# GT-STAR-Lab/MARBLER

Hardware: AMD Instinct MI355X
Metric: env agent-steps/sec (higher is better)
Workload: dtype f32

## Files before the change

include/robogym.h:

```cpp
#ifndef ROBOGYM_H
#define ROBOGYM_H

#include <stdint.h>

#ifdef __cplusplus
extern "C" {
#endif

#define RG_ABI_VERSION 7
#define RG_MAX_AGENTS 16
#define RG_MAX_PREY 64

enum {
    RG_SCN_PREDATOR_CAPTURE_PREY = 0,
    RG_SCN_WAREHOUSE = 1,
    RG_SCN_MATERIAL_TRANSPORT = 2,
    RG_SCN_SIMPLE = 3,
    RG_SCN_ARCTIC_TRANSPORT = 4
};
#define RG_ARCTIC_ROWS 8
#define RG_ARCTIC_COLS 12
enum { RG_COLLISION_CENTER = 0, RG_COLLISION_OFFSET = 1 };
enum { RG_VIOL_NONE = 0, RG_VIOL_COLLISION = 1, RG_VIOL_BOUNDARY = 2, RG_VIOL_COLLISION_BOUNDARY = 3 };
enum { RG_QP_EXACT = 0, RG_QP_CVXOPT = 1 };
#define RG_QP_CVXOPT_MAX_AGENTS 8

typedef struct rg_grid {
    int32_t nx, ny;
    float spacing, w2, h2, ox1, ox2, oy1, oy2;
} rg_grid;

typedef struct rg_scenario_params {
    int32_t scenario;
    int32_t n_agents;
    int32_t obs_dim;
    int32_t update_frequency;
    int32_t controller_period;
    int32_t max_episode_steps;
    int32_t penalize_violations;
    int32_t barrier_has_unsafe_gain;
    int32_t collision_variant;
    int32_t capability_aware;
    int32_t num_prey;
    int32_t num_neighbors;
    int32_t torque[RG_MAX_AGENTS];
    float time_step, bound_x0, bound_y0, bound_w, bound_h;
    float robot_diameter, wheel_radius, max_linear_velocity;
    float collision_offset, collision_diameter;
    float projection_distance, angular_velocity_limit, position_velocity_limit;
    float barrier_gain, unsafe_barrier_gain, safety_radius, barrier_magnitude_limit;
    float qp_rtol;
    int32_t qp_max_sweeps;
    float left, right, up, down;
    float agent_step[RG_MAX_AGENTS];
    float sensing_radius[RG_MAX_AGENTS];
    float capture_radius[RG_MAX_AGENTS];
    float time_penalty, sense_reward, capture_reward, violation_reward;
    float load_reward, unload_reward, goal_width;
    float unload_multiplier, load_multiplier, end_goal_width, zone1_radius;
    float reward_scaler;
    float arctic_normal_step, arctic_slow_step, arctic_fast_step;
    float not_reached_penalty, dist_multiplier;
    rg_grid agent_grid, prey_grid;
    int32_t keep_theta;
    int32_t shared_reward;
    float zone1_mean, zone1_std, zone2_mean, zone2_std;
    int32_t qp_mode;
    float ipm_abstol, ipm_reltol, ipm_feastol;
    int32_t ipm_maxiters;
} rg_scenario_params;

typedef struct rg_state {
    float *poses;
    float *carry_dist;
    int32_t *episode_steps;
    int32_t *reset_count;
    float *prey_loc;
    uint8_t *prey_sensed;
    uint8_t *prey_captured;
    uint8_t *loaded;
    int32_t *load;
    int32_t *zone_load;
    int32_t *messages;
    uint8_t *grid;
    int32_t *goal_col;
    uint8_t *pixel_type;
    uint8_t *reached_goal;
    float *ep_return;
    float *done_return_sum;
    int32_t *done_count;
    int32_t *done_steps_sum;
    float *next_init;
    int32_t *next_episode;
} rg_state;

typedef struct rg_step_io {
    float *obs;
    float *reward;
    uint8_t *done;
    float *dist_travelled;
    uint8_t *violation;
    int32_t *remaining;
    int32_t *qp_sweeps;
    int32_t *elapsed;
    uint8_t *truncated;
    uint8_t *ended;
    float *reward_sum;
    int32_t time_limit;
    int32_t zero_obs_on_end;
} rg_step_io;

typedef struct rg_handle rg_handle;

int rg_abi_version(void);
const char *rg_last_error(void);
int rg_sizeof_params(void);
int rg_sizeof_state(void);
int rg_sizeof_step_io(void);
int rg_next_init_stride(const rg_scenario_params *params);

rg_handle *rg_create(const rg_scenario_params *params, int32_t num_envs, int64_t env_offset, int32_t device,
                     void *hip_stream);
int rg_destroy(rg_handle *h);

int rg_bind_state(rg_handle *h, const rg_state *state);

#define RG_RESET_BOOK_EPISODE 1
int rg_reset(rg_handle *h, const uint8_t *mask, uint64_t seed, int32_t flags);

int rg_step(rg_handle *h, const int32_t *actions, const rg_step_io *io, int32_t auto_reset, uint64_t seed);

int rg_rollout(rg_handle *h, const int32_t *actions, int32_t num_steps, const rg_step_io *io, int32_t auto_reset,
               uint64_t seed);

int rg_set_stream(rg_handle *h, void *hip_stream);

int rg_get_obs(rg_handle *h, float *obs);

int rg_step_kernel(const rg_handle *h);

#define RG_LIDAR_MAX_RAYS 32
typedef struct rg_lidar_params {
    int32_t rays;
    int32_t offset;
    float range;
    float inv_range;
    float dir[RG_LIDAR_MAX_RAYS][2];
} rg_lidar_params;
int rg_sizeof_lidar_params(void);
int rg_set_lidar(rg_handle *h, const rg_lidar_params *lp);

#define RG_TEAM_MAX_SETS 64
#define RG_TEAM_EPISODE 0
#define RG_TEAM_FIXED 1
typedef struct rg_team_params {
    int32_t n_sets;
    int32_t mode;
    const float *agent_step;
    const float *sensing_radius;
    const float *capture_radius;
    const int32_t *torque;
    int32_t *team_index;
} rg_team_params;
int rg_sizeof_team_params(void);
int rg_set_teams(rg_handle *h, const rg_team_params *tp);

#define RG_DISTURB_MAX_SIGMA_XY 0.1f
#define RG_DISTURB_MAX_SIGMA_THETA 0.5f
typedef struct rg_disturbance_params {
    float sigma_xy;
    float sigma_theta;
    float reserved[2];
} rg_disturbance_params;
int rg_sizeof_disturbance_params(void);
int rg_set_disturbance(rg_handle *h, const rg_disturbance_params *dp);

typedef struct {
    const float *w1, *b1;
    const float *wih, *bih;
    const float *whh, *bhh;
    const float *w2, *b2;
    int32_t n_sets, input_dim, hidden_dim, n_actions, use_rnn;
    int32_t gru_packed;
} rg_actor_weights;

int rg_actor_forward(const rg_actor_weights *w, int32_t num_envs, int32_t n_agents, const float *obs,
                     int32_t obs_dim, int32_t append_agent_id, const uint8_t *restart, float *hidden, float *q,
                     int32_t *actions, void *hip_stream);
int rg_actor_forward_explore(const rg_actor_weights *w, int32_t num_envs, int32_t n_agents, const float *obs,
                             int32_t obs_dim, int32_t append_agent_id, const uint8_t *restart, float *hidden, float *q,
                             int32_t *actions, const float *explore_u, float epsilon, void *hip_stream);
int rg_actor_forward_sample(const rg_actor_weights *w, int32_t num_envs, int32_t n_agents, const float *obs,
                            int32_t obs_dim, int32_t append_agent_id, const uint8_t *restart, float *hidden, float *q,
                            int32_t *actions, const float *sample_u, float *prob, void *hip_stream);
int rg_actor_pack_gru(const float *src, int32_t n_sets, int32_t hidden_dim, float *dst, void *hip_stream);
int rg_actor_pack_gru_bf16x3(const float *src, int32_t n_sets, int32_t hidden_dim, void *dst, void *hip_stream);
int rg_actor_pack_gru_f16x2(const float *src, int32_t n_sets, int32_t hidden_dim, void *dst, void *hip_stream);
const char *rg_actor_last_error(void);

typedef struct rg_policy_io {
    float *hidden;
    const uint8_t *restart;
    int32_t append_agent_id;
    int32_t restart_on_done;
    const float *explore_u;
    float epsilon;
    int32_t *actions;
    float *obs;
    float *reward_sum;
    uint8_t *ended;
    float *dist_sum;
} rg_policy_io;
int rg_sizeof_policy_io(void);
int rg_policy_rollout(rg_handle *h, const rg_actor_weights *w, int32_t num_steps, const rg_policy_io *pio, const rg_step_io *io,
                      int32_t auto_reset, uint64_t seed);

typedef struct rg_policy_sample {
    const float *sample_u;
    float *prob;
} rg_policy_sample;
int rg_sizeof_policy_sample(void);
int rg_policy_rollout_sample(rg_handle *h, const rg_actor_weights *w, int32_t num_steps, const rg_policy_io *pio,
                             const rg_policy_sample *sample, const rg_step_io *io, int32_t auto_reset, uint64_t seed);

#ifdef __cplusplus
}
#endif
#endif
```

marbler_amd/_lib.py:

```python
import ctypes as C
import os

MAX_AGENTS, MAX_PREY = 16, 64
ABI_VERSION = 7
RESET_BOOK_EPISODE = 1

_HERE = os.path.dirname(os.path.abspath(__file__))
LIB_PATH = os.environ.get("ROBOGYM_LIB") or os.path.join(_HERE, "librobogym_hip.so")


class RgGrid(C.Structure):
    _fields_ = [("nx", C.c_int32), ("ny", C.c_int32), ("spacing", C.c_float), ("w2", C.c_float),
                ("h2", C.c_float), ("ox1", C.c_float), ("ox2", C.c_float), ("oy1", C.c_float),
                ("oy2", C.c_float)]


class RgScenarioParams(C.Structure):
    _fields_ = [
        ("scenario", C.c_int32), ("n_agents", C.c_int32), ("obs_dim", C.c_int32),
        ("update_frequency", C.c_int32), ("controller_period", C.c_int32),
        ("max_episode_steps", C.c_int32), ("penalize_violations", C.c_int32),
        ("barrier_has_unsafe_gain", C.c_int32), ("collision_variant", C.c_int32),
        ("capability_aware", C.c_int32), ("num_prey", C.c_int32), ("num_neighbors", C.c_int32),
        ("torque", C.c_int32 * MAX_AGENTS),
        ("time_step", C.c_float), ("bound_x0", C.c_float), ("bound_y0", C.c_float),
        ("bound_w", C.c_float), ("bound_h", C.c_float),
        ("robot_diameter", C.c_float), ("wheel_radius", C.c_float), ("max_linear_velocity", C.c_float),
        ("collision_offset", C.c_float), ("collision_diameter", C.c_float),
        ("projection_distance", C.c_float), ("angular_velocity_limit", C.c_float),
        ("position_velocity_limit", C.c_float),
        ("barrier_gain", C.c_float), ("unsafe_barrier_gain", C.c_float), ("safety_radius", C.c_float),
        ("barrier_magnitude_limit", C.c_float), ("qp_rtol", C.c_float), ("qp_max_sweeps", C.c_int32),
        ("left", C.c_float), ("right", C.c_float), ("up", C.c_float), ("down", C.c_float),
        ("agent_step", C.c_float * MAX_AGENTS), ("sensing_radius", C.c_float * MAX_AGENTS),
        ("capture_radius", C.c_float * MAX_AGENTS),
        ("time_penalty", C.c_float), ("sense_reward", C.c_float), ("capture_reward", C.c_float),
        ("violation_reward", C.c_float),
        ("load_reward", C.c_float), ("unload_reward", C.c_float), ("goal_width", C.c_float),
        ("unload_multiplier", C.c_float), ("load_multiplier", C.c_float), ("end_goal_width", C.c_float),
        ("zone1_radius", C.c_float), ("reward_scaler", C.c_float),
        ("arctic_normal_step", C.c_float), ("arctic_slow_step", C.c_float), ("arctic_fast_step", C.c_float),
        ("not_reached_penalty", C.c_float), ("dist_multiplier", C.c_float),
        ("agent_grid", RgGrid), ("prey_grid", RgGrid), ("keep_theta", C.c_int32), ("shared_reward", C.c_int32),
        ("zone1_mean", C.c_float), ("zone1_std", C.c_float), ("zone2_mean", C.c_float),
        ("zone2_std", C.c_float),
        ("qp_mode", C.c_int32), ("ipm_abstol", C.c_float), ("ipm_reltol", C.c_float), ("ipm_feastol", C.c_float), ("ipm_maxiters", C.c_int32),
    ]


class RgState(C.Structure):
    _fields_ = [("poses", C.c_void_p), ("carry_dist", C.c_void_p), ("episode_steps", C.c_void_p),
                ("reset_count", C.c_void_p), ("prey_loc", C.c_void_p), ("prey_sensed", C.c_void_p),
                ("prey_captured", C.c_void_p), ("loaded", C.c_void_p), ("load", C.c_void_p),
                ("zone_load", C.c_void_p), ("messages", C.c_void_p), ("grid", C.c_void_p),
                ("goal_col", C.c_void_p), ("pixel_type", C.c_void_p), ("reached_goal", C.c_void_p),
                ("ep_return", C.c_void_p),
                ("done_return_sum", C.c_void_p), ("done_count", C.c_void_p), ("done_steps_sum", C.c_void_p),
                ("next_init", C.c_void_p), ("next_episode", C.c_void_p)]


class RgStepIO(C.Structure):
    _fields_ = [("obs", C.c_void_p), ("reward", C.c_void_p), ("done", C.c_void_p),
                ("dist_travelled", C.c_void_p), ("violation", C.c_void_p), ("remaining", C.c_void_p),
                ("qp_sweeps", C.c_void_p),
                ("elapsed", C.c_void_p), ("truncated", C.c_void_p), ("ended", C.c_void_p), ("reward_sum", C.c_void_p),
                ("time_limit", C.c_int32), ("zero_obs_on_end", C.c_int32)]


class RgActorWeights(C.Structure):
    _fields_ = [("w1", C.c_void_p), ("b1", C.c_void_p), ("wih", C.c_void_p), ("bih", C.c_void_p),
                ("whh", C.c_void_p), ("bhh", C.c_void_p), ("w2", C.c_void_p), ("b2", C.c_void_p),
                ("n_sets", C.c_int32), ("input_dim", C.c_int32), ("hidden_dim", C.c_int32),
                ("n_actions", C.c_int32), ("use_rnn", C.c_int32), ("gru_packed", C.c_int32)]


class RgPolicyIO(C.Structure):
    _fields_ = [("hidden", C.c_void_p), ("restart", C.c_void_p), ("append_agent_id", C.c_int32), ("restart_on_done", C.c_int32),
                ("explore_u", C.c_void_p), ("epsilon", C.c_float), ("actions", C.c_void_p), ("obs", C.c_void_p),
                ("reward_sum", C.c_void_p), ("ended", C.c_void_p), ("dist_sum", C.c_void_p)]


class RgPolicySample(C.Structure):
    _fields_ = [("sample_u", C.c_void_p), ("prob", C.c_void_p)]


LIDAR_MAX_RAYS = 32


class RgLidarParams(C.Structure):
    _fields_ = [("rays", C.c_int32), ("offset", C.c_int32), ("range", C.c_float), ("inv_range", C.c_float),
                ("dir", (C.c_float * 2) * LIDAR_MAX_RAYS)]


TEAM_MAX_SETS = 64
TEAM_EPISODE, TEAM_FIXED = 0, 1


class RgTeamParams(C.Structure):
    _fields_ = [("n_sets", C.c_int32), ("mode", C.c_int32), ("agent_step", C.c_void_p), ("sensing_radius", C.c_void_p),
                ("capture_radius", C.c_void_p), ("torque", C.c_void_p), ("team_index", C.c_void_p)]


DISTURB_MAX_SIGMA_XY, DISTURB_MAX_SIGMA_THETA = 0.1, 0.5


class RgDisturbanceParams(C.Structure):
    _fields_ = [("sigma_xy", C.c_float), ("sigma_theta", C.c_float), ("reserved", C.c_float * 2)]


EXPORTS = ("rg_abi_version", "rg_last_error", "rg_sizeof_params", "rg_sizeof_state", "rg_sizeof_step_io", "rg_next_init_stride",
           "rg_create", "rg_destroy", "rg_bind_state", "rg_set_stream", "rg_reset", "rg_step", "rg_rollout", "rg_get_obs", "rg_step_kernel",
           "rg_actor_forward", "rg_actor_forward_explore", "rg_actor_pack_gru", "rg_actor_pack_gru_bf16x3", "rg_actor_pack_gru_f16x2", "rg_actor_last_error",
           "rg_sizeof_policy_io", "rg_policy_rollout", "rg_sizeof_lidar_params", "rg_set_lidar",
           "rg_sizeof_team_params", "rg_set_teams",
           "rg_actor_forward_sample", "rg_sizeof_policy_sample", "rg_policy_rollout_sample",
           "rg_sizeof_disturbance_params", "rg_set_disturbance")

_lib = None


class RobogymError(RuntimeError):
    pass


def load():
    global _lib
    if _lib is not None:
        return _lib
    if not os.path.exists(LIB_PATH):
        raise RobogymError(
            f"{LIB_PATH} not found: build it with `python -m marbler_amd.build` (hipcc, gfx950). "
            "marbler_amd has no CPU fallback.")
    lib = C.CDLL(LIB_PATH)
    for name in EXPORTS:
        if not hasattr(lib, name):
            raise RobogymError(f"{LIB_PATH} does not export {name}")
    lib.rg_abi_version.restype = C.c_int
    lib.rg_last_error.restype = C.c_char_p
    lib.rg_create.restype = C.c_void_p
    lib.rg_create.argtypes = [C.POINTER(RgScenarioParams), C.c_int32, C.c_int64, C.c_int32, C.c_void_p]
    lib.rg_next_init_stride.argtypes = [C.POINTER(RgScenarioParams)]
    lib.rg_next_init_stride.restype = C.c_int
    lib.rg_destroy.argtypes = [C.c_void_p]
    lib.rg_bind_state.argtypes = [C.c_void_p, C.POINTER(RgState)]
    lib.rg_set_stream.argtypes = [C.c_void_p, C.c_void_p]
    lib.rg_reset.argtypes = [C.c_void_p, C.c_void_p, C.c_uint64, C.c_int32]
    lib.rg_step.argtypes = [C.c_void_p, C.c_void_p, C.POINTER(RgStepIO), C.c_int32, C.c_uint64]
    lib.rg_rollout.argtypes = [C.c_void_p, C.c_void_p, C.c_int32, C.POINTER(RgStepIO), C.c_int32, C.c_uint64]
    lib.rg_get_obs.argtypes = [C.c_void_p, C.c_void_p]
    lib.rg_step_kernel.argtypes = [C.c_void_p]
    lib.rg_step_kernel.restype = C.c_int
    lib.rg_actor_forward.argtypes = [C.POINTER(RgActorWeights), C.c_int32, C.c_int32, C.c_void_p, C.c_int32, C.c_int32,
                                     C.c_void_p, C.c_void_p, C.c_void_p, C.c_void_p, C.c_void_p]
    lib.rg_actor_forward.restype = C.c_int
    lib.rg_actor_forward_explore.argtypes = [C.POINTER(RgActorWeights), C.c_int32, C.c_int32, C.c_void_p, C.c_int32, C.c_int32,
                                             C.c_void_p, C.c_void_p, C.c_void_p, C.c_void_p, C.c_void_p, C.c_float, C.c_void_p]
    lib.rg_actor_forward_explore.restype = C.c_int
    lib.rg_actor_forward_sample.argtypes = [C.POINTER(RgActorWeights), C.c_int32, C.c_int32, C.c_void_p, C.c_int32, C.c_int32,
                                            C.c_void_p, C.c_void_p, C.c_void_p, C.c_void_p, C.c_void_p, C.c_void_p, C.c_void_p]
    lib.rg_actor_forward_sample.restype = C.c_int
    lib.rg_actor_pack_gru.argtypes = [C.c_void_p, C.c_int32, C.c_int32, C.c_void_p, C.c_void_p]
    lib.rg_actor_pack_gru.restype = C.c_int
    lib.rg_actor_pack_gru_bf16x3.argtypes = [C.c_void_p, C.c_int32, C.c_int32, C.c_void_p, C.c_void_p]
    lib.rg_actor_pack_gru_bf16x3.restype = C.c_int
    lib.rg_actor_pack_gru_f16x2.argtypes = [C.c_void_p, C.c_int32, C.c_int32, C.c_void_p, C.c_void_p]
    lib.rg_actor_pack_gru_f16x2.restype = C.c_int
    lib.rg_actor_last_error.restype = C.c_char_p
    lib.rg_policy_rollout.argtypes = [C.c_void_p, C.POINTER(RgActorWeights), C.c_int32, C.POINTER(RgPolicyIO), C.POINTER(RgStepIO),
                                      C.c_int32, C.c_uint64]
    lib.rg_policy_rollout.restype = C.c_int
    lib.rg_sizeof_policy_io.restype = C.c_int
    lib.rg_policy_rollout_sample.argtypes = [C.c_void_p, C.POINTER(RgActorWeights), C.c_int32, C.POINTER(RgPolicyIO),
                                             C.POINTER(RgPolicySample), C.POINTER(RgStepIO), C.c_int32, C.c_uint64]
    lib.rg_policy_rollout_sample.restype = C.c_int
    lib.rg_sizeof_policy_sample.restype = C.c_int
    lib.rg_set_lidar.argtypes = [C.c_void_p, C.POINTER(RgLidarParams)]
    lib.rg_set_lidar.restype = C.c_int
    lib.rg_sizeof_lidar_params.restype = C.c_int
    lib.rg_set_teams.argtypes = [C.c_void_p, C.POINTER(RgTeamParams)]
    lib.rg_set_teams.restype = C.c_int
    lib.rg_sizeof_team_params.restype = C.c_int
    lib.rg_set_disturbance.argtypes = [C.c_void_p, C.POINTER(RgDisturbanceParams)]
    lib.rg_set_disturbance.restype = C.c_int
    lib.rg_sizeof_disturbance_params.restype = C.c_int
    for f in (lib.rg_destroy, lib.rg_bind_state, lib.rg_set_stream, lib.rg_reset, lib.rg_step, lib.rg_rollout, lib.rg_get_obs,
              lib.rg_sizeof_params, lib.rg_sizeof_state, lib.rg_sizeof_step_io):
        f.restype = C.c_int
    if lib.rg_abi_version() != ABI_VERSION:
        raise RobogymError(f"ABI version {lib.rg_abi_version()} != {ABI_VERSION}; rebuild the library")
    if (lib.rg_sizeof_params() != C.sizeof(RgScenarioParams) or lib.rg_sizeof_state() != C.sizeof(RgState)
            or lib.rg_sizeof_step_io() != C.sizeof(RgStepIO) or lib.rg_sizeof_policy_io() != C.sizeof(RgPolicyIO)
            or lib.rg_sizeof_policy_sample() != C.sizeof(RgPolicySample)
            or lib.rg_sizeof_lidar_params() != C.sizeof(RgLidarParams) or lib.rg_sizeof_team_params() != C.sizeof(RgTeamParams)
            or lib.rg_sizeof_disturbance_params() != C.sizeof(RgDisturbanceParams)):
        raise RobogymError("struct layout of the binding differs from the compiled library; rebuild")
    _lib = lib
    return lib


def check(rc, what):
    if rc != 0:
        raise RobogymError(f"{what} failed ({rc}): {load().rg_last_error().decode()}")
```

marbler_amd/build.py:

```python
import glob
import os
import shutil
import subprocess
import sys

HERE = os.path.dirname(os.path.abspath(__file__))
CSRC = os.path.join(HERE, "csrc")
LIB = os.path.join(HERE, "librobogym_hip.so")
SOURCES = ["robogym_kernels.hip", "robogym_resident.hip", "robogym_rollout_group.hip", "robogym_kernels_ipm.hip", "robogym_rollout_group_ipm.hip",
           "robogym_tpe.hip", "robogym_rollout_tpe.hip", "robogym_capi.hip", "actor_mfma.hip", "robogym_policy_h64.hip",
           "robogym_policy_h128.hip", "robogym_policy_sample_h64.hip", "robogym_policy_sample_h128.hip", "robogym_lidar.hip", "robogym_lidar_rollout.hip", "robogym_lidar_ipm.hip",
           "robogym_lidar_rollout_ipm.hip", "robogym_team.hip", "robogym_team_rollout.hip", "robogym_team_ipm.hip",
           "robogym_team_rollout_ipm.hip", "robogym_disturb.hip", "robogym_disturb_rollout.hip", "robogym_disturb_ipm.hip",
           "robogym_disturb_rollout_ipm.hip"]
HEADERS = sorted(glob.glob(os.path.join(CSRC, "*.h")) + glob.glob(os.path.join(CSRC, "*.inc")) + glob.glob(os.path.join(CSRC, "probes", "*.h"))) + \
          [os.path.join(HERE, "..", "include", "robogym.h")]
ARCH = "gfx950"
GROUP_SLP = ["-mllvm", "-slp-threshold=-60"]
IPM_SCHED = ["-mllvm", "-amdgpu-sched-strategy=max-ilp"]
RESIDENT_PRELOAD = ["-mllvm", "-amdgpu-kernarg-preload-count=16"]
FILE_FLAGS = {"robogym_tpe.hip": ["-fno-slp-vectorize"], "robogym_rollout_tpe.hip": ["-fno-slp-vectorize"],
              "robogym_kernels.hip": GROUP_SLP, "robogym_rollout_group.hip": GROUP_SLP,
              "robogym_resident.hip": GROUP_SLP + RESIDENT_PRELOAD,
              "robogym_kernels_ipm.hip": GROUP_SLP + IPM_SCHED, "robogym_rollout_group_ipm.hip": GROUP_SLP + IPM_SCHED,
              "robogym_policy_h64.hip": GROUP_SLP, "robogym_policy_h128.hip": GROUP_SLP,
              "robogym_policy_sample_h64.hip": GROUP_SLP, "robogym_policy_sample_h128.hip": GROUP_SLP,
              "robogym_lidar.hip": GROUP_SLP, "robogym_lidar_rollout.hip": GROUP_SLP,
              "robogym_lidar_ipm.hip": GROUP_SLP + IPM_SCHED, "robogym_lidar_rollout_ipm.hip": GROUP_SLP + IPM_SCHED,
              "robogym_team.hip": GROUP_SLP, "robogym_team_rollout.hip": GROUP_SLP,
              "robogym_team_ipm.hip": GROUP_SLP + IPM_SCHED, "robogym_team_rollout_ipm.hip": GROUP_SLP + IPM_SCHED,
              "robogym_disturb.hip": GROUP_SLP, "robogym_disturb_rollout.hip": GROUP_SLP,
              "robogym_disturb_ipm.hip": GROUP_SLP + IPM_SCHED, "robogym_disturb_rollout_ipm.hip": GROUP_SLP + IPM_SCHED}
BASE_FLAGS = [f"--offload-arch={ARCH}", "-O3", "-fPIC", "-std=c++17", "-ffp-contract=off", "-Wall", "-Wno-unused-function"]
STAMP = LIB + ".flags"


def hipcc_path():
    for c in (os.environ.get("HIPCC"), "/opt/rocm/bin/hipcc", shutil.which("hipcc")):
        if c and os.path.exists(c):
            return c
    raise RuntimeError("hipcc not found (ROCm 7.x expected under /opt/rocm)")


def flags_stamp(defines=(), extra=(), file_flags=True):
    per_file = sorted(FILE_FLAGS.items()) if file_flags else []
    return repr((BASE_FLAGS, sorted(defines), list(extra), per_file, SOURCES))


def needs_build():
    if not os.path.exists(LIB):
        return True
    t = os.path.getmtime(LIB)
    deps = [os.path.join(CSRC, s) for s in SOURCES] + HEADERS + [os.path.abspath(__file__)]
    if any(os.path.getmtime(d) > t for d in deps):
        return True
    try:
        with open(STAMP) as f:
            return f.read() != flags_stamp()
    except OSError:
        return True


def build(force=False, verbose=False, defines=(), out=None):
    extra = os.environ.get("RG_EXTRA_HIPCC_FLAGS", "").split()
    no_file_flags = bool(os.environ.get("RG_NO_FILE_FLAGS"))
    if out is None:
        if not force and not needs_build():
            return LIB
        if extra or no_file_flags:
            import warnings
            warnings.warn("RG_EXTRA_HIPCC_FLAGS / RG_NO_FILE_FLAGS are for diagnostic variants (build(out=...)) and are IGNORED for the "
                          "shipped library, whose flags are fixed in marbler_amd/build.py")
            extra, no_file_flags = [], False
    shipped = out is None
    out = out or LIB
    objdir = os.path.join(HERE, "build", os.path.splitext(os.path.basename(out))[0])
    os.makedirs(objdir, exist_ok=True)
    flags = BASE_FLAGS + [f"-D{d}" for d in defines] + extra
    objs, procs = [], []
    for src in SOURCES:
        obj = os.path.join(objdir, os.path.splitext(src)[0] + ".o")
        per_file = [] if no_file_flags else FILE_FLAGS.get(src, [])
        cmd = [hipcc_path()] + flags + per_file + ["-c", os.path.join(CSRC, src), "-o", obj]
        if verbose:
            print(" ".join(cmd))
        procs.append((cmd, subprocess.Popen(cmd)))
        objs.append(obj)
    for cmd, pr in procs:
        if pr.wait() != 0:
            raise subprocess.CalledProcessError(pr.returncode, cmd)
    link = [hipcc_path(), f"--offload-arch={ARCH}", "-shared", "-fPIC", "-o", out] + objs
    if verbose:
        print(" ".join(link))
    subprocess.check_call(link)
    with open(out + ".flags", "w") as f:
        f.write(flags_stamp(defines, extra, not no_file_flags) if not shipped else flags_stamp())
    return out


def build_host_sanitized(out=None):
    out = out or os.path.join(HERE, "build", "librobogym_capi_asan.so")
    os.makedirs(os.path.dirname(out), exist_ok=True)
    stubs = os.path.join(HERE, "..", "tests", "sanitize", "launch_stubs.cpp")
    stubs_sample = os.path.join(HERE, "..", "tests", "sanitize", "launch_stubs_sample.cpp")
    cmd = [hipcc_path(), "-x", "hip", "--offload-host-only", "-O1", "-g", "-fno-omit-frame-pointer",
           "-fsanitize=address,undefined", "-fno-sanitize-recover=undefined", "-fPIC", "-shared", "-std=c++17",
           "-I", CSRC, os.path.join(CSRC, "robogym_capi.hip"), stubs, stubs_sample, "-o", out]
    subprocess.check_call(cmd)
    return out


def asan_runtime():
    return subprocess.check_output([hipcc_path(), "-print-file-name=libclang_rt.asan-x86_64.so"], text=True).strip()


if __name__ == "__main__":
    print(build(force="--force" in sys.argv, verbose=True))
```

marbler_amd/csrc/kernel_args.h:

```cpp
#pragma once
#include <hip/hip_runtime.h>
#include <math.h>
#include <stddef.h>
#include <stdint.h>

#include <type_traits>

#include "../../include/robogym.h"

namespace rg {

struct Consts {
    float dt, pd, inv_pd, r2, wlim, vmax, wmax, pvl, bml;
    float xmin, xmax, ymin, ymax, coll_off, coll_lim2;
    float thr_pre;
    float lin_pre;
    float xc, xh, yc, yh;
};

constexpr float PRE_SLACK = 2e-6f;
inline float pre_margin(float max_abs_coordinate) {
    float spacing = 0.0009765625f;
    for (float lim = 2.0f; lim <= max_abs_coordinate && lim < 1024.0f; lim *= 2.0f) spacing *= 2.0f;
    return 1.05f * 1.41421356f * (2.0f * spacing + 6.103515625e-05f);
}

inline Consts make_consts(const rg_scenario_params &p) {
    Consts k;
    k.dt = p.time_step;
    k.pd = p.projection_distance;
    k.inv_pd = 1.0f / p.projection_distance;
    k.r2 = p.safety_radius * p.safety_radius;
    k.wlim = p.angular_velocity_limit;
    k.vmax = p.max_linear_velocity;
    k.wmax = 2.0f * (p.wheel_radius / p.robot_diameter) * (p.max_linear_velocity / p.wheel_radius);
    k.pvl = p.position_velocity_limit;
    k.bml = p.barrier_magnitude_limit;
    k.xmin = p.bound_x0;
    k.ymin = p.bound_y0;
    k.xmax = p.bound_x0 + p.bound_w;
    k.ymax = p.bound_y0 + p.bound_h;
    const bool off = p.collision_variant == RG_COLLISION_OFFSET;
    k.coll_off = off ? p.collision_offset : 0.0f;
    const float lim = off ? p.collision_diameter : p.robot_diameter;
    k.coll_lim2 = lim * lim;
    const float ax = fmaxf(fabsf(k.xmin), fabsf(k.xmax)), ay = fmaxf(fabsf(k.ymin), fabsf(k.ymax));
    const float lp = lim + pre_margin(fmaxf(ax, ay) + 0.25f);
    k.thr_pre = lp * lp * 1.00001f;
    k.lin_pre = lp;
    k.xc = 0.5f * (k.xmin + k.xmax);
    k.xh = 0.5f * (k.xmax - k.xmin);
    k.yc = 0.5f * (k.ymin + k.ymax);
    k.yh = 0.5f * (k.ymax - k.ymin);
    return k;
}

struct KernelArgs {
    rg_scenario_params p;
    Consts k;
    rg_state st;
    rg_step_io io;
    const int32_t *actions;
    const uint8_t *reset_mask;
    int32_t E;
    int32_t envs_per_wave;
    int32_t num_steps;
    int32_t auto_reset;
    int32_t reset_flags;
    int32_t next_stride;
    int64_t env_offset;
    uint64_t seed;
};

inline int next_init_stride(const rg_scenario_params &p) {
    int w = 3 * p.n_agents;
    if (p.scenario == RG_SCN_PREDATOR_CAPTURE_PREY || p.scenario == RG_SCN_SIMPLE) w += 2 * p.num_prey;
    else if (p.scenario == RG_SCN_MATERIAL_TRANSPORT) w += 2;
    else if (p.scenario == RG_SCN_ARCTIC_TRANSPORT) w += 25;
    return (w + 3) & ~3;
}

template <typename F>
inline hipError_t for_scenario(int scn, F &&f) {
    switch (scn) {
        case RG_SCN_PREDATOR_CAPTURE_PREY: return f(std::integral_constant<int, RG_SCN_PREDATOR_CAPTURE_PREY>());
        case RG_SCN_WAREHOUSE: return f(std::integral_constant<int, RG_SCN_WAREHOUSE>());
        case RG_SCN_MATERIAL_TRANSPORT: return f(std::integral_constant<int, RG_SCN_MATERIAL_TRANSPORT>());
        case RG_SCN_SIMPLE: return f(std::integral_constant<int, RG_SCN_SIMPLE>());
        case RG_SCN_ARCTIC_TRANSPORT: return f(std::integral_constant<int, RG_SCN_ARCTIC_TRANSPORT>());
        default: return hipErrorInvalidValue;
    }
}

hipError_t launch_reset(const KernelArgs &a, hipStream_t stream);

enum GroupFamily { GROUP_PLAIN, GROUP_LIDAR, GROUP_TEAM, GROUP_DISTURB };
enum GroupKind { GROUP_STEP, GROUP_ROLLOUT, GROUP_OBS, GROUP_STEP_RESIDENT };
#define RG_GROUP_ENTRIES(X)                                              \
    X(launch_step, GROUP_PLAIN, RG_QP_EXACT, GROUP_STEP)                 \
    X(launch_step_resident, GROUP_PLAIN, RG_QP_EXACT, GROUP_STEP_RESIDENT) \
    X(launch_obs, GROUP_PLAIN, RG_QP_EXACT, GROUP_OBS)                   \
    X(launch_rollout, GROUP_PLAIN, RG_QP_EXACT, GROUP_ROLLOUT)           \
    X(launch_step_ipm, GROUP_PLAIN, RG_QP_CVXOPT, GROUP_STEP)            \
    X(launch_rollout_ipm, GROUP_PLAIN, RG_QP_CVXOPT, GROUP_ROLLOUT)      \
    X(launch_lidar_step, GROUP_LIDAR, RG_QP_EXACT, GROUP_STEP)           \
    X(launch_lidar_obs, GROUP_LIDAR, RG_QP_EXACT, GROUP_OBS)             \
    X(launch_lidar_rollout, GROUP_LIDAR, RG_QP_EXACT, GROUP_ROLLOUT)     \
    X(launch_lidar_step_ipm, GROUP_LIDAR, RG_QP_CVXOPT, GROUP_STEP)      \
    X(launch_lidar_rollout_ipm, GROUP_LIDAR, RG_QP_CVXOPT, GROUP_ROLLOUT) \
    X(launch_team_step, GROUP_TEAM, RG_QP_EXACT, GROUP_STEP)             \
    X(launch_team_obs, GROUP_TEAM, RG_QP_EXACT, GROUP_OBS)               \
    X(launch_team_rollout, GROUP_TEAM, RG_QP_EXACT, GROUP_ROLLOUT)       \
    X(launch_team_step_ipm, GROUP_TEAM, RG_QP_CVXOPT, GROUP_STEP)        \
    X(launch_team_rollout_ipm, GROUP_TEAM, RG_QP_CVXOPT, GROUP_ROLLOUT)  \
    X(launch_disturb_step, GROUP_DISTURB, RG_QP_EXACT, GROUP_STEP)       \
    X(launch_disturb_rollout, GROUP_DISTURB, RG_QP_EXACT, GROUP_ROLLOUT) \
    X(launch_disturb_step_ipm, GROUP_DISTURB, RG_QP_CVXOPT, GROUP_STEP)  \
    X(launch_disturb_rollout_ipm, GROUP_DISTURB, RG_QP_CVXOPT, GROUP_ROLLOUT)
struct DisturbScale {
    float k_xy, k_theta;
};
inline float disturb_scale(float sigma) { return static_cast<float>(static_cast<double>(sigma) * sqrt(3.0 / 1048575.0)); }
struct GroupSide {
    const rg_lidar_params *lidar;
    const rg_team_params *teams;
    const DisturbScale *disturb;
    const struct KernelArgs *image;
};

struct ResidentCall {
    const KernelArgs *image;
    const int32_t *actions;
    uint64_t seed;
    int32_t auto_reset;
    int32_t grid;
    rg_step_io io;
};
static_assert(sizeof(ResidentCall) <= 256, "the per-call arguments fit one register of dwords (device_common.h load_arg_regs_resident)");
hipError_t resident_image(KernelArgs &a);
typedef hipError_t GroupLaunch(const KernelArgs &a, const GroupSide &side, hipStream_t stream);
#define RG_X(entry, family, mode, kind) GroupLaunch entry;
RG_GROUP_ENTRIES(RG_X)
#undef RG_X

struct StepView {
    const int32_t *actions;
    rg_step_io io;
    const int32_t *auto_reset;
    const uint64_t *seed;
    int32_t grid;
};
__host__ __device__ inline StepView step_view(const KernelArgs &a, int k, int n_agents, int obs_dim) {
    StepView v;
    const size_t e = static_cast<size_t>(a.E) * k, en = e * n_agents;
    v.actions = a.actions ? a.actions + en : nullptr;
    v.io.obs = a.io.obs ? a.io.obs + en * obs_dim : nullptr;
    v.io.reward = a.io.reward ? a.io.reward + en : nullptr;
    v.io.done = a.io.done ? a.io.done + e : nullptr;
    v.io.dist_travelled = a.io.dist_travelled ? a.io.dist_travelled + en : nullptr;
    v.io.violation = a.io.violation ? a.io.violation + e : nullptr;
    v.io.remaining = a.io.remaining ? a.io.remaining + e : nullptr;
    v.io.qp_sweeps = a.io.qp_sweeps ? a.io.qp_sweeps + e : nullptr;
    v.io.elapsed = a.io.elapsed;
    v.io.truncated = a.io.truncated ? a.io.truncated + e : nullptr;
    v.io.ended = a.io.ended ? a.io.ended + e : nullptr;
    v.io.reward_sum = a.io.reward_sum ? a.io.reward_sum + e : nullptr;
    v.io.time_limit = a.io.time_limit;
    v.io.zero_obs_on_end = a.io.zero_obs_on_end;
    v.auto_reset = &a.auto_reset;
    v.seed = &a.seed;
    v.grid = 0;
    return v;
}
bool tpe_supported(const rg_scenario_params &p);
hipError_t launch_step_tpe(const KernelArgs &a, hipStream_t stream);
hipError_t launch_rollout_tpe(const KernelArgs &a, hipStream_t stream);

}
```

marbler_amd/csrc/robogym_capi.hip:

```cpp
#include <hip/hip_runtime.h>
#include <stdint.h>
#include <stdio.h>
#include <stdlib.h>
#include <string.h>

#include <new>

#include "../../include/robogym.h"
#include "kernel_args.h"

struct rg_handle {
    rg_scenario_params params;
    rg::Consts consts;
    rg_state state;
    int32_t num_envs;
    int64_t env_offset;
    int32_t device;
    hipStream_t stream;
    bool bound;
    bool use_tpe;
    bool seed_seen;
    uint64_t last_seed;
    bool default_tpe;
    rg_lidar_params lidar;
    rg_team_params teams;
    bool disturbed;
    rg::DisturbScale disturb;
    bool span;
    bool resident;
    rg::KernelArgs *image_slots;
    int32_t images_used;
    const rg::KernelArgs *image;
    bool image_stale;
};
constexpr int RG_IMAGE_SLOTS = 8;
constexpr size_t RG_IMAGE_STRIDE = 1024;
static_assert(sizeof(rg::KernelArgs) <= RG_IMAGE_STRIDE, "an image slot holds the block");
static void write_image(rg_handle *h);
static void drop_image(rg_handle *h) {
    h->image = nullptr;
    h->image_stale = true;
}

static int32_t tpe_min_envs(const rg_scenario_params &p) {
    const bool mt = p.scenario == RG_SCN_MATERIAL_TRANSPORT, pcp = p.scenario == RG_SCN_PREDATOR_CAPTURE_PREY;
    if (p.qp_mode == RG_QP_CVXOPT) return p.n_agents == 5 ? 12288 : 20480;
    switch (p.n_agents) {
        case 2: return 65536;
        case 3: return pcp ? 98304 : 65536;
        case 4: return p.scenario == RG_SCN_SIMPLE ? 393216 : p.scenario == RG_SCN_ARCTIC_TRANSPORT ? 131072 : 196608;
        case 5: return mt ? 49152 : 65536;
        case 6: return mt ? 65536 : p.scenario == RG_SCN_WAREHOUSE ? 262144 : pcp ? 98304 : 131072;
        default: return INT32_MAX;
    }
}

static thread_local char g_err[512] = "";

struct DeviceGuard {
    int prev = -1;
    bool switched = false;
    hipError_t err;
    explicit DeviceGuard(int device) {
        err = hipGetDevice(&prev);
        if (err == hipSuccess && prev != device) {
            err = hipSetDevice(device);
            switched = (err == hipSuccess);
        }
    }
    ~DeviceGuard() {
        if (switched) (void)hipSetDevice(prev);
    }
    DeviceGuard(const DeviceGuard &) = delete;
    DeviceGuard &operator=(const DeviceGuard &) = delete;
};

static int fail(int code, const char *fmt, const char *detail = "") {
    snprintf(g_err, sizeof(g_err), fmt, detail);
    return code;
}

static int check_params(const rg_scenario_params *p) {
    if (!p) return fail(-1, "params is NULL");
    if (p->scenario < RG_SCN_PREDATOR_CAPTURE_PREY || p->scenario > RG_SCN_ARCTIC_TRANSPORT)
        return fail(-2, "unknown scenario id");
    if (p->n_agents < 1 || p->n_agents > RG_MAX_AGENTS) return fail(-3, "n_agents must be in 1..16");
    if (p->update_frequency < 1 || p->controller_period < 1) return fail(-4, "update_frequency / controller_period < 1");
    if (p->obs_dim < 1) return fail(-5, "obs_dim < 1");
    if (p->qp_max_sweeps < 1 || !(p->qp_rtol >= 0.0f)) return fail(-5, "qp_max_sweeps < 1 or qp_rtol < 0");
    if (p->qp_mode != RG_QP_EXACT && p->qp_mode != RG_QP_CVXOPT) return fail(-5, "unknown qp_mode");
    if (p->qp_mode == RG_QP_CVXOPT) {
        if (p->n_agents > RG_QP_CVXOPT_MAX_AGENTS) return fail(-3, "qp_mode RG_QP_CVXOPT is built for n_agents <= 8");
        if (p->ipm_maxiters < 0 || !(p->ipm_reltol >= 0.0f) || !(p->ipm_feastol > 0.0f) || !(p->ipm_abstol >= 0.0f))
            return fail(-5, "ipm_maxiters < 0, or a negative / zero cvxopt tolerance");
    }
    if (p->collision_variant != RG_COLLISION_CENTER && p->collision_variant != RG_COLLISION_OFFSET)
        return fail(-6, "unknown collision_variant");
    const rg_grid &g = p->agent_grid;
    if (g.nx < 1 || g.ny < 1 || g.nx * g.ny <= p->n_agents || g.nx * g.ny > 64)
        return fail(-7, "agent reset grid must have n_agents < nx*ny <= 64");
    if (p->scenario == RG_SCN_PREDATOR_CAPTURE_PREY) {
        if (p->num_prey < 1 || p->num_prey > RG_MAX_PREY) return fail(-8, "num_prey must be in 1..64");
        const rg_grid &q = p->prey_grid;
        if (q.nx < 1 || q.ny < 1 || q.nx * q.ny <= p->num_prey || q.nx * q.ny > 64)
            return fail(-9, "prey reset grid must have num_prey < nx*ny <= 64");
        const int od = p->capability_aware ? 6 : 4;
        const int nb = p->num_neighbors >= p->n_agents - 1 ? p->n_agents - 1 : p->num_neighbors;
        if (p->obs_dim < od * (nb + 1)) return fail(-10, "obs_dim too small for PredatorCapturePrey");
        if (od == 4 && (p->obs_dim & 3)) return fail(-10, "obs_dim must be a multiple of 4 for PredatorCapturePrey without capability_aware");
    } else if (p->scenario == RG_SCN_WAREHOUSE) {
        const int nb = p->num_neighbors >= p->n_agents - 1 ? p->n_agents - 1 : p->num_neighbors;
        if (p->obs_dim < 3 * (nb + 1)) return fail(-10, "obs_dim too small for Warehouse");
    } else if (p->scenario == RG_SCN_SIMPLE) {
        if (p->num_prey != 1) return fail(-8, "Simple has one goal (num_prey = 1)");
        const rg_grid &q = p->prey_grid;
        if (q.nx < 1 || q.ny < 1 || q.nx * q.ny <= 1 || q.nx * q.ny > 64) return fail(-9, "goal reset grid must have 1 < nx*ny <= 64");
        if (p->obs_dim < 2 * (p->n_agents + 1)) return fail(-10, "obs_dim too small for Simple");
    } else if (p->scenario == RG_SCN_ARCTIC_TRANSPORT) {
        if (p->n_agents != 4) return fail(-3, "ArcticTransport has exactly 4 agents");
        if (p->obs_dim < 30) return fail(-10, "obs_dim too small for ArcticTransport");
    } else {
        if (p->obs_dim < (p->capability_aware ? 11 : 9)) return fail(-10, "obs_dim too small for MaterialTransport");
    }
    return 0;
}

namespace rg {
hipError_t launch_policy_rollout_h64(const KernelArgs &, const rg_actor_weights &, const rg_policy_io &, int32_t, hipStream_t)
    __attribute__((weak));
hipError_t launch_policy_rollout_h128(const KernelArgs &, const rg_actor_weights &, const rg_policy_io &, int32_t, hipStream_t)
    __attribute__((weak));
hipError_t launch_policy_rollout_sample_h64(const KernelArgs &, const rg_actor_weights &, const rg_policy_io &, const rg_policy_sample &,
                                            int32_t, hipStream_t) __attribute__((weak));
hipError_t launch_policy_rollout_sample_h128(const KernelArgs &, const rg_actor_weights &, const rg_policy_io &, const rg_policy_sample &,
                                             int32_t, hipStream_t) __attribute__((weak));
#define RG_X(entry, family, mode, kind) GroupLaunch entry __attribute__((weak));
RG_GROUP_ENTRIES(RG_X)
#undef RG_X
hipError_t launch_team_index(const KernelArgs &, const rg_team_params &, hipStream_t) __attribute__((weak));
hipError_t resident_image(KernelArgs &) __attribute__((weak));
}

static int own_obs_width(const rg_scenario_params &p) {
    const int nb = p.num_neighbors >= p.n_agents - 1 ? p.n_agents - 1 : p.num_neighbors;
    switch (p.scenario) {
        case RG_SCN_PREDATOR_CAPTURE_PREY: return (p.capability_aware ? 6 : 4) * (nb + 1);
        case RG_SCN_WAREHOUSE: return 3 * (nb + 1);
        case RG_SCN_SIMPLE: return 2 * (p.n_agents + 1);
        case RG_SCN_ARCTIC_TRANSPORT: return 30;
        default: return p.capability_aware ? 11 : 9;
    }
}

static const struct GroupEntry {
    rg::GroupLaunch *launch;
    int family, mode, kind;
} g_group[] = {
#define RG_X(entry, family, mode, kind) {rg::entry, rg::family, mode, rg::kind},
    RG_GROUP_ENTRIES(RG_X)
#undef RG_X
};

static bool group_family_built(int family) {
    for (const GroupEntry &g : g_group)
        if (g.family == family && !g.launch) return false;
    return true;
}

extern "C" {

int rg_abi_version(void) { return RG_ABI_VERSION; }

const char *rg_last_error(void) { return g_err; }

int rg_sizeof_params(void) { return static_cast<int>(sizeof(rg_scenario_params)); }
int rg_sizeof_state(void) { return static_cast<int>(sizeof(rg_state)); }
int rg_sizeof_step_io(void) { return static_cast<int>(sizeof(rg_step_io)); }
int rg_sizeof_policy_io(void) { return static_cast<int>(sizeof(rg_policy_io)); }
int rg_sizeof_policy_sample(void) { return static_cast<int>(sizeof(rg_policy_sample)); }
int rg_sizeof_lidar_params(void) { return static_cast<int>(sizeof(rg_lidar_params)); }
int rg_sizeof_team_params(void) { return static_cast<int>(sizeof(rg_team_params)); }
int rg_sizeof_disturbance_params(void) { return static_cast<int>(sizeof(rg_disturbance_params)); }
int rg_next_init_stride(const rg_scenario_params *params) {
    if (check_params(params) != 0) return -1;
    return rg::next_init_stride(*params);
}

rg_handle *rg_create(const rg_scenario_params *params, int32_t num_envs, int64_t env_offset, int32_t device,
                     void *hip_stream) {
    if (check_params(params) != 0) return nullptr;
    if (num_envs < 1) {
        fail(-11, "num_envs < 1");
        return nullptr;
    }
    int count = 0;
    if (hipGetDeviceCount(&count) != hipSuccess || count < 1) {
        fail(-12, "no HIP device visible: librobogym_hip has no CPU fallback");
        return nullptr;
    }
    if (device < 0 || device >= count) {
        fail(-13, "device index out of range");
        return nullptr;
    }
    if (!group_family_built(rg::GROUP_PLAIN)) {
        fail(-100, "rg_create: this build has no lane-group step kernels");
        return nullptr;
    }
    rg_handle *h = new (std::nothrow) rg_handle();
    if (!h) {
        fail(-14, "out of host memory");
        return nullptr;
    }
    h->params = *params;
    h->consts = rg::make_consts(*params);
    memset(&h->state, 0, sizeof(h->state));
    h->num_envs = num_envs;
    h->env_offset = env_offset;
    h->device = device;
    h->stream = static_cast<hipStream_t>(hip_stream);
    h->bound = false;
    h->seed_seen = false;
    h->last_seed = 0;
    h->use_tpe = rg::tpe_supported(*params) && num_envs >= tpe_min_envs(*params);
    if (const char *force = getenv("RG_STEP_KERNEL")) {
        if (!strcmp(force, "group")) h->use_tpe = false;
        else if (!strcmp(force, "tpe") && rg::tpe_supported(*params)) h->use_tpe = true;
    }
    h->default_tpe = h->use_tpe;
    {
        const char *span = getenv("RG_STEP_SPAN");
        h->span = !(span && !strcmp(span, "0"));
    }
    {
        const char *res = getenv("RG_STEP_RESIDENT");
        h->resident = !(res && !strcmp(res, "0")) && rg::resident_image && rg::launch_step_resident;
    }
    h->image_slots = nullptr;
    h->images_used = 0;
    h->image = nullptr;
    h->image_stale = true;
    memset(&h->lidar, 0, sizeof(h->lidar));
    memset(&h->teams, 0, sizeof(h->teams));
    h->disturbed = false;
    h->disturb = rg::DisturbScale{0.0f, 0.0f};
    return h;
}

int rg_set_lidar(rg_handle *h, const rg_lidar_params *lp) {
    if (!h) return fail(-1, "handle is NULL");
    if (!lp || lp->rays == 0) {
        memset(&h->lidar, 0, sizeof(h->lidar));
        h->use_tpe = (h->teams.n_sets || h->disturbed) ? false : h->default_tpe;
        drop_image(h);
        return 0;
    }
    if (h->disturbed) return fail(-57, "rg_set_lidar: the handle has the pose disturbance on (rg_set_disturbance); the disturbance and the lidar do not combine");
    if (h->teams.n_sets) return fail(-54, "rg_set_lidar: the handle has a team pool (rg_set_teams); a pool and the lidar do not combine");
    if (lp->rays < 4 || lp->rays > RG_LIDAR_MAX_RAYS || (lp->rays & 3))
        return fail(-50, "rg_set_lidar: rays must be 0 or a multiple of 4 in 4..32");
    if (lp->offset + lp->rays != h->params.obs_dim)
        return fail(-51, "rg_set_lidar: offset + rays must equal obs_dim (the lidar block ends the observation row)");
    if (lp->offset < own_obs_width(h->params))
        return fail(-52, "rg_set_lidar: offset lies inside the scenario's own observation columns");
    if (!(lp->range > 0.0f && lp->range <= 3.402823466e38f)) return fail(-53, "rg_set_lidar: range must be positive and finite");
    if (!group_family_built(rg::GROUP_LIDAR)) return fail(-100, "rg_set_lidar: this build has no lidar kernels");
    h->lidar = *lp;
    h->use_tpe = false;
    drop_image(h);
    return 0;
}

int rg_set_disturbance(rg_handle *h, const rg_disturbance_params *dp) {
    if (!h) return fail(-1, "handle is NULL");
    if (!dp || (dp->sigma_xy == 0.0f && dp->sigma_theta == 0.0f)) {
        h->disturbed = false;
        h->disturb = rg::DisturbScale{0.0f, 0.0f};
        h->use_tpe = (h->lidar.rays || h->teams.n_sets) ? false : h->default_tpe;
        drop_image(h);
        return 0;
    }
    if (!(dp->sigma_xy >= 0.0f && dp->sigma_xy <= RG_DISTURB_MAX_SIGMA_XY))
        return fail(-70, "rg_set_disturbance: sigma_xy must be a finite number of metres in [0, 0.1]");
    if (!(dp->sigma_theta >= 0.0f && dp->sigma_theta <= RG_DISTURB_MAX_SIGMA_THETA))
        return fail(-71, "rg_set_disturbance: sigma_theta must be a finite number of radians in [0, 0.5]");
    if (h->lidar.rays) return fail(-72, "rg_set_disturbance: the handle has the lidar on (rg_set_lidar); the disturbance and the lidar do not combine");
    if (h->teams.n_sets) return fail(-73, "rg_set_disturbance: the handle has a team pool (rg_set_teams); the disturbance and a pool do not combine");
    if (!group_family_built(rg::GROUP_DISTURB)) return fail(-100, "rg_set_disturbance: this build has no disturbance kernels");
    h->disturb = rg::DisturbScale{rg::disturb_scale(dp->sigma_xy), rg::disturb_scale(dp->sigma_theta)};
    h->disturbed = true;
    h->use_tpe = false;
    drop_image(h);
    return 0;
}

int rg_destroy(rg_handle *h) {
    if (!h) return fail(-1, "handle is NULL");
    if (h->image_slots) {
        DeviceGuard guard(h->device);
        if (guard.err == hipSuccess) (void)hipFree(h->image_slots);
    }
    delete h;
    return 0;
}

int rg_set_stream(rg_handle *h, void *hip_stream) {
    if (!h) return fail(-1, "handle is NULL");
    h->stream = static_cast<hipStream_t>(hip_stream);
    return 0;
}

int rg_bind_state(rg_handle *h, const rg_state *st) {
    if (!h || !st) return fail(-1, "handle or state is NULL");
    if (!st->poses || !st->carry_dist || !st->episode_steps || !st->reset_count)
        return fail(-20, "poses, carry_dist, episode_steps and reset_count are required");
    switch (h->params.scenario) {
        case RG_SCN_PREDATOR_CAPTURE_PREY:
            if (!st->prey_loc || !st->prey_sensed || !st->prey_captured)
                return fail(-21, "PredatorCapturePrey needs prey_loc, prey_sensed, prey_captured");
            if (reinterpret_cast<uintptr_t>(st->prey_loc) & 7u) return fail(-26, "prey_loc must be 8-byte aligned");
            break;
        case RG_SCN_WAREHOUSE:
            if (!st->loaded) return fail(-21, "Warehouse needs loaded");
            break;
        case RG_SCN_SIMPLE:
            if (!st->prey_loc) return fail(-21, "Simple needs prey_loc (its goal)");
            break;
        case RG_SCN_ARCTIC_TRANSPORT:
            if (!st->grid || !st->goal_col || !st->pixel_type || !st->reached_goal)
                return fail(-21, "ArcticTransport needs grid, goal_col, pixel_type, reached_goal");
            if (reinterpret_cast<uintptr_t>(st->grid) & 3u) return fail(-26, "grid must be 4-byte aligned");
            break;
        default:
            if (!st->load || !st->zone_load || !st->messages)
                return fail(-21, "MaterialTransport needs load, zone_load, messages");
    }
    const int nstat = (st->ep_return != nullptr) + (st->done_return_sum != nullptr) + (st->done_count != nullptr) +
                      (st->done_steps_sum != nullptr);
    if (nstat != 0 && nstat != 4) return fail(-25, "rollout statistics arrays: set all four or none");
    if ((st->next_init != nullptr) != (st->next_episode != nullptr)) return fail(-25, "next_init / next_episode: set both or none");
    if (reinterpret_cast<uintptr_t>(st->next_init) & 15u) return fail(-26, "next_init must be 16-byte aligned");
    h->state = *st;
    h->bound = true;
    drop_image(h);
    write_image(h);
    h->seed_seen = false;
    return 0;
}

static int fill_args(rg_handle *h, rg::KernelArgs &a);
#define RG_ON_DEVICE(h)                                                                           \
    DeviceGuard guard_((h)->device);                                                              \
    if (guard_.err != hipSuccess) return fail(-31, "cannot select the handle's device: %s", hipGetErrorString(guard_.err))

static void write_image(rg_handle *h) {
    h->image = nullptr;
    if (!h->resident || !h->bound || h->use_tpe || !h->span || h->teams.n_sets || h->lidar.rays || h->disturbed ||
        h->params.qp_mode != RG_QP_EXACT) {
        h->image_stale = false;
        return;
    }
    if (h->images_used >= RG_IMAGE_SLOTS) {
        h->image_stale = false;
        return;
    }
    rg::KernelArgs a;
    if (fill_args(h, a) != 0 || rg::resident_image(a) != hipSuccess) {
        h->image_stale = false;
        return;
    }
    DeviceGuard guard(h->device);
    if (guard.err != hipSuccess) return;
    hipStreamCaptureStatus cap = hipStreamCaptureStatusNone;
    if (hipStreamIsCapturing(h->stream, &cap) != hipSuccess || cap != hipStreamCaptureStatusNone) {
        (void)hipGetLastError();
        return;
    }
    if (!h->image_slots) {
        void *mem = nullptr;
        if (hipMalloc(&mem, RG_IMAGE_SLOTS * RG_IMAGE_STRIDE) != hipSuccess) {
            (void)hipGetLastError();
            h->images_used = RG_IMAGE_SLOTS;
            h->image_stale = false;
            return;
        }
        h->image_slots = static_cast<rg::KernelArgs *>(mem);
    }
    rg::KernelArgs *slot = reinterpret_cast<rg::KernelArgs *>(reinterpret_cast<char *>(h->image_slots) + RG_IMAGE_STRIDE * h->images_used);
    h->images_used += 1;
    h->image_stale = false;
    if (hipMemcpy(slot, &a, sizeof(a), hipMemcpyHostToDevice) != hipSuccess) {
        (void)hipGetLastError();
        return;
    }
    h->image = slot;
}

static int fill_args(rg_handle *h, rg::KernelArgs &a) {
    if (!h) return fail(-1, "handle is NULL");
    if (!h->bound) return fail(-22, "rg_bind_state has not been called");
    memset(&a, 0, sizeof(a));
    a.p = h->params;
    a.k = h->consts;
    a.st = h->state;
    a.E = h->num_envs;
    a.num_steps = 1;
    a.env_offset = h->env_offset;
    a.next_stride = (!h->use_tpe && h->state.next_init) ? rg::next_init_stride(h->params) : 0;
    return 0;
}

static int sync_seed(rg_handle *h, uint64_t seed) {
    if (h->state.next_episode && (!h->seed_seen || h->last_seed != seed)) {
        const hipError_t err = hipMemsetAsync(h->state.next_episode, 0xFF, sizeof(int32_t) * static_cast<size_t>(h->num_envs), h->stream);
        if (err != hipSuccess) return fail(-30, "hipMemsetAsync(next_episode) failed: %s", hipGetErrorString(err));
        h->seed_seen = true;
        h->last_seed = seed;
    }
    return 0;
}

static int check_io(const rg_step_io *io) {
    if (!io->obs || !io->reward || !io->done || !io->dist_travelled || !io->violation || !io->remaining)
        return fail(-24, "every rg_step_io array except qp_sweeps and the gymma block is required");
    if (reinterpret_cast<uintptr_t>(io->obs) & 15u) return fail(-26, "obs must be 16-byte aligned");
    if (io->elapsed) {
        if (!io->truncated || !io->ended || !io->reward_sum) return fail(-24, "gymma block: elapsed needs truncated, ended and reward_sum");
        if (io->time_limit < 1) return fail(-29, "gymma block: time_limit must be > 0");
    }
    return 0;
}

static int launched(hipError_t err) {
    if (err != hipSuccess) return fail(-30, "kernel launch failed: %s", hipGetErrorString(err));
    return 0;
}

static int launch_group_entry(const rg_handle *h, const rg::KernelArgs &a, int kind, const rg::KernelArgs *image = nullptr) {
    const int family = h->teams.n_sets ? rg::GROUP_TEAM : h->lidar.rays ? rg::GROUP_LIDAR
                       : (h->disturbed && kind != rg::GROUP_OBS) ? rg::GROUP_DISTURB : rg::GROUP_PLAIN;
    const int mode = kind == rg::GROUP_OBS ? RG_QP_EXACT : h->params.qp_mode;
    const rg::GroupSide side = {&h->lidar, &h->teams, &h->disturb, family == rg::GROUP_PLAIN ? image : nullptr};
    for (const GroupEntry &g : g_group)
        if (g.family == family && g.mode == mode && g.kind == kind && g.launch) return launched(g.launch(a, side, h->stream));
    return fail(-100, "this build has no lane-group step kernels");
}

int rg_reset(rg_handle *h, const uint8_t *mask, uint64_t seed, int32_t flags) {
    rg::KernelArgs a;
    if (int rc = fill_args(h, a)) return rc;
    if (flags & ~RG_RESET_BOOK_EPISODE) return fail(-28, "unknown rg_reset flags");
    a.reset_mask = mask;
    a.seed = seed;
    a.reset_flags = flags;
    RG_ON_DEVICE(h);
    if (int rc = launched(rg::launch_reset(a, h->stream))) return rc;
    if (h->teams.n_sets) return launched(rg::launch_team_index(a, h->teams, h->stream));
    return 0;
}

int rg_step(rg_handle *h, const int32_t *actions, const rg_step_io *io, int32_t auto_reset, uint64_t seed) {
    rg::KernelArgs a;
    if (int rc = fill_args(h, a)) return rc;
    if (!actions || !io) return fail(-23, "actions or io is NULL");
    if (int rc = check_io(io)) return rc;
    a.actions = actions;
    a.io = *io;
    a.auto_reset = auto_reset;
    a.seed = seed;
    RG_ON_DEVICE(h);
    if (int rc = sync_seed(h, seed)) return rc;
    if (!h->span && !h->teams.n_sets && !h->lidar.rays && !h->disturbed) a.envs_per_wave = -1;
    if (h->use_tpe) return launched(rg::launch_step_tpe(a, h->stream));
    if (h->image_stale) write_image(h);
    return launch_group_entry(h, a, rg::GROUP_STEP, io->elapsed ? nullptr : h->image);
}

int rg_rollout(rg_handle *h, const int32_t *actions, int32_t num_steps, const rg_step_io *io, int32_t auto_reset,
               uint64_t seed) {
    rg::KernelArgs a;
    if (int rc = fill_args(h, a)) return rc;
    if (!actions || !io) return fail(-23, "actions or io is NULL");
    if (num_steps < 1) return fail(-27, "num_steps < 1");
    if (io->elapsed) return fail(-29, "the gymma block of rg_step_io belongs to rg_step (one launch per step)");
    if (int rc = check_io(io)) return rc;
    a.actions = actions;
    a.io = *io;
    a.num_steps = num_steps;
    a.auto_reset = auto_reset;
    a.seed = seed;
    RG_ON_DEVICE(h);
    if (int rc = sync_seed(h, seed)) return rc;
    if (!h->use_tpe) return launch_group_entry(h, a, rg::GROUP_ROLLOUT);
    if (h->num_envs <= 65536) return launched(rg::launch_rollout_tpe(a, h->stream));
    a.num_steps = 1;
    for (int32_t k = 0; k < num_steps; ++k) {
        const rg::StepView v = rg::step_view(a, k, h->params.n_agents, h->params.obs_dim);
        rg::KernelArgs ak = a;
        ak.actions = v.actions;
        ak.io = v.io;
        if (int rc = launched(rg::launch_step_tpe(ak, h->stream))) return rc;
    }
    return 0;
}

static int policy_rollout(rg_handle *h, const rg_actor_weights *w, int32_t num_steps, const rg_policy_io *pio,
                          const rg_policy_sample *sample, bool sampling, const rg_step_io *io, int32_t auto_reset, uint64_t seed) {
    rg::KernelArgs a;
    if (int rc = fill_args(h, a)) return rc;
    if (!w || !pio || !io) return fail(-23, "weights, policy io or step io is NULL");
    if (num_steps < 1) return fail(-27, "num_steps < 1");
    if (h->params.qp_mode == RG_QP_CVXOPT) return fail(-40, "rg_policy_rollout: the interior-point mode (barrier_solver: cvxopt) is not supported");
    if (h->lidar.rays) return fail(-49, "rg_policy_rollout: a handle with the lidar observation on (rg_set_lidar) is not supported");
    if (h->teams.n_sets) return fail(-39, "rg_policy_rollout: a handle with a team pool (rg_set_teams) is not supported");
    if (h->disturbed) return fail(-38, "rg_policy_rollout: a handle with the pose disturbance on (rg_set_disturbance) is not supported");
    if (!w->use_rnn || w->gru_packed != 3)
        return fail(-41, "rg_policy_rollout: the actor must be a GRU with gru_packed == 3 (two binary16 planes, pack_gru='f16x2')");
    if (w->hidden_dim != 64 && w->hidden_dim != 128) return fail(-42, "rg_policy_rollout: hidden_dim must be 64 or 128");
    const int N = h->params.n_agents;
    if (w->n_sets != 1 && w->n_sets != N) return fail(-43, "rg_policy_rollout: n_sets must be 1 (shared) or n_agents");
    if (w->input_dim != h->params.obs_dim + (pio->append_agent_id ? N : 0))
        return fail(-44, "rg_policy_rollout: the actor's input_dim != obs_dim (+ n_agents with append_agent_id)");
    if (w->input_dim > 64) return fail(-44, "rg_policy_rollout: input_dim above 64 is not supported");
    if (w->n_actions < 1 || w->n_actions > 32) return fail(-45, "rg_policy_rollout: n_actions must be in 1..32");
    if (!w->w1 || !w->b1 || !w->wih || !w->bih || !w->whh || !w->bhh || !w->w2 || !w->b2) return fail(-46, "rg_policy_rollout: a weight array is NULL");
    if (!pio->hidden || !pio->actions) return fail(-47, "rg_policy_rollout: hidden and actions are required");
    if ((reinterpret_cast<uintptr_t>(pio->hidden) | reinterpret_cast<uintptr_t>(pio->obs) | reinterpret_cast<uintptr_t>(w->w1) |
         reinterpret_cast<uintptr_t>(w->wih) | reinterpret_cast<uintptr_t>(w->whh) | reinterpret_cast<uintptr_t>(w->w2)) & 15u)
        return fail(-26, "rg_policy_rollout: hidden, obs, w1, wih, whh and w2 must be 16-byte aligned");
    if (pio->explore_u && !(pio->epsilon >= 1e-6f && pio->epsilon <= 1.0f)) return fail(-48, "rg_policy_rollout: epsilon must be in [1e-6, 1] with explore_u");
    if (!io->elapsed) return fail(-29, "rg_policy_rollout: the step io must carry the gymma block (elapsed, truncated, ended, reward_sum)");
    if (int rc = check_io(io)) return rc;
    auto launch = w->hidden_dim == 64 ? rg::launch_policy_rollout_h64 : rg::launch_policy_rollout_h128;
    auto launch_sample = w->hidden_dim == 64 ? rg::launch_policy_rollout_sample_h64 : rg::launch_policy_rollout_sample_h128;
    if (sampling ? !launch_sample : !launch) return fail(-100, "rg_policy_rollout: this build has no device code");
    a.io = *io;
    a.auto_reset = auto_reset;
    a.seed = seed;
    a.next_stride = 0;
    RG_ON_DEVICE(h);
    if (int rc = sync_seed(h, seed)) return rc;
    if (sampling) return launched(launch_sample(a, *w, *pio, *sample, num_steps, h->stream));
    return launched(launch(a, *w, *pio, num_steps, h->stream));
}

int rg_policy_rollout(rg_handle *h, const rg_actor_weights *w, int32_t num_steps, const rg_policy_io *pio, const rg_step_io *io,
                      int32_t auto_reset, uint64_t seed) {
    return policy_rollout(h, w, num_steps, pio, nullptr, false, io, auto_reset, seed);
}

int rg_policy_rollout_sample(rg_handle *h, const rg_actor_weights *w, int32_t num_steps, const rg_policy_io *pio,
                             const rg_policy_sample *sample, const rg_step_io *io, int32_t auto_reset, uint64_t seed) {
    if (!sample || !sample->sample_u) return fail(-55, "rg_policy_rollout_sample: sample or its sample_u is NULL");
    if (pio && pio->explore_u) return fail(-56, "rg_policy_rollout_sample: sample_u and explore_u do not combine (explore_u must be NULL)");
    return policy_rollout(h, w, num_steps, pio, sample, true, io, auto_reset, seed);
}

int rg_set_teams(rg_handle *h, const rg_team_params *tp) {
    if (!h) return fail(-1, "handle is NULL");
    if (!tp || tp->n_sets == 0) {
        memset(&h->teams, 0, sizeof(h->teams));
        h->use_tpe = (h->lidar.rays || h->disturbed) ? false : h->default_tpe;
        drop_image(h);
        return 0;
    }
    if (h->disturbed) return fail(-65, "rg_set_teams: the handle has the pose disturbance on (rg_set_disturbance); the disturbance and a pool do not combine");
    if (tp->n_sets < 1 || tp->n_sets > RG_TEAM_MAX_SETS) return fail(-60, "rg_set_teams: n_sets must be 0 or in 1..64");
    if (tp->mode != RG_TEAM_EPISODE && tp->mode != RG_TEAM_FIXED)
        return fail(-61, "rg_set_teams: unknown mode (RG_TEAM_EPISODE or RG_TEAM_FIXED)");
    if (h->params.scenario == RG_SCN_ARCTIC_TRANSPORT)
        return fail(-62, "rg_set_teams: ArcticTransport's agent types are fixed by the scenario; it takes no team pool");
    if (h->lidar.rays) return fail(-63, "rg_set_teams: the handle has the lidar on (rg_set_lidar); a pool and the lidar do not combine");
    const int sc = h->params.scenario;
    if (!tp->team_index || !tp->agent_step || (sc == RG_SCN_PREDATOR_CAPTURE_PREY && (!tp->sensing_radius || !tp->capture_radius)) ||
        (sc == RG_SCN_MATERIAL_TRANSPORT && !tp->torque))
        return fail(-64, "rg_set_teams: team_index, agent_step and the scenario's other tables (PredatorCapturePrey: sensing_radius, "
                         "capture_radius; MaterialTransport: torque) are required");
    if (!group_family_built(rg::GROUP_TEAM) || !rg::launch_team_index) return fail(-100, "rg_set_teams: this build has no team kernels");
    if (tp->mode == RG_TEAM_FIXED) {
        rg::KernelArgs a;
        if (int rc = fill_args(h, a)) return rc;
        RG_ON_DEVICE(h);
        if (int rc = launched(rg::launch_team_index(a, *tp, h->stream))) return rc;
    }
    h->teams = *tp;
    h->use_tpe = false;
    drop_image(h);
    return 0;
}

int rg_step_kernel(const rg_handle *h) {
    if (!h) return fail(-1, "handle is NULL");
    return h->use_tpe ? 1 : 0;
}

int rg_get_obs(rg_handle *h, float *obs) {
    rg::KernelArgs a;
    if (int rc = fill_args(h, a)) return rc;
    if (!obs) return fail(-23, "obs is NULL");
    if (reinterpret_cast<uintptr_t>(obs) & 15u) return fail(-26, "obs must be 16-byte aligned");
    a.io.obs = obs;
    RG_ON_DEVICE(h);
    return launch_group_entry(h, a, rg::GROUP_OBS);
}

}
```

marbler_amd/csrc/step_group.h:

```cpp
#pragma once
#include <hip/hip_runtime.h>
#include <stdint.h>

#include <type_traits>

#include "device_common.h"
#include "ipm_qp.h"
#include "lidar.h"
#include "team.h"
#include "disturb.h"
#include "probes/diag.h"

namespace rg {

__device__ __forceinline__ void out_store4(float *p, float a, float b, float c, float d) {
    *reinterpret_cast<float4 *>(p) = make_float4(a, b, c, d);
}
__device__ __forceinline__ void out_store1(float *p, float a) {
    *p = a;
}

constexpr int CHUNK = RG_CHUNK;
static_assert(CHUNK >= 1 && CHUNK <= 5, "the sparse collision pre-test covers sub-steps 0..2 and 3..4 of a chunk: longer chunks would go untested");

template <int GW, int QPM = 0, typename QpLds = void, bool SPAN = false>
__device__ __forceinline__ int controller(const rg_scenario_params &p, const Consts &k, int N, int ag, bool lane_ok,
                                          bool upd, float x, float y, float c, float s, float gx, float gy, float &v,
                                          float &w, QpLds *qp RG_CTRL_TICKS_PARAM) {
    RG_CTRL_BEGIN(x, y, c, s)
    const float xix = x + k.pd * c, xiy = y + k.pd * s;
    float ux = gx - xix, uy = gy - xiy;
    {
        const float nrm = norm2_spec(ux, uy);
        const float sc = k.pvl / nrm;
        const bool clip = nrm > k.pvl;
        ux = clip ? ux * sc : ux;
        uy = clip ? uy * sc : uy;
    }
    if constexpr (QPM == RG_QP_CVXOPT) {
        {
            const float n2u = ux * ux + uy * uy;
            const bool clip = n2u > k.bml * k.bml;
            if (__any(clip)) {
                const float sc = k.bml / __builtin_sqrtf(n2u);
                ux = clip ? ux * sc : ux;
                uy = clip ? uy * sc : uy;
            }
        }
        const int lane_ = threadIdx.x;
        qp->rec[lane_] = make_float4(xix, xiy, ux, uy);
        __syncthreads();
        int iters = 0;
        if (upd) iters = ipm::solve_qp_n<GW>(N, ipm::make_consts(p), qp->rec + (lane_ & ~(GW - 1)), qp->ws[lane_ / GW], ag);
        __syncthreads();
        const float4 r = qp->rec[lane_];
        ux = r.z;
        uy = r.w;
        RG_CTRL_TICK(1);
        float vv = c * ux + s * uy;
        float ww = k.inv_pd * (-s * ux + c * uy);
        ww = ww > k.wlim ? k.wlim : ww;
        ww = ww < -k.wlim ? -k.wlim : ww;
        vv = vv > k.vmax ? k.vmax : vv;
        vv = vv < -k.vmax ? -k.vmax : vv;
        ww = ww > k.wmax ? k.wmax : ww;
        ww = ww < -k.wmax ? -k.wmax : ww;
        v = upd ? vv : v;
        w = upd ? ww : w;
        RG_CTRL_TICK(2);
        return iters;
    }
    const float bgain = p.barrier_gain, ugain = p.unsafe_barrier_gain, qp_rtol = p.qp_rtol;
    const int qp_cap = p.qp_max_sweeps;
    const bool has_unsafe = p.barrier_has_unsafe_gain != 0;
    float ex[GW - 1], ey[GW - 1], fx[GW - 1], fy[GW - 1], bp[GW - 1], emax[GW - 1];
    float mu[GW - 1], dmu[GW - 1];
    auto pair_consts = [&](float pxi, float pyi, int K, int i) {
        const float dx = xix - pxi, dy = xiy - pyi;
        const float ee = dx * dx + dy * dy;
        const float h = ee - k.r2;
        const float gain = ((h >= 0.0f) | !has_unsafe) ? bgain : ugain;
        const float b = gain * ((h * h) * h);
        const float n2 = 2.0f * ee;
        const bool ok = lane_ok & ((ag ^ K) < N) & (n2 > 0.0f);
        const float rn2 = ok ? 1.0f / n2 : 0.0f;
        ex[i] = dx;
        ey[i] = dy;
        fx[i] = dx * rn2;
        fy[i] = dy * rn2;
        bp[i] = (0.5f * b) * rn2;
        emax[i] = ok ? fmaxf(__builtin_fabsf(dx), __builtin_fabsf(dy)) : 0.0f;
    };
    const bool helper = SPAN && (threadIdx.x & GW) != 0;
    if constexpr (SPAN) {
        static_assert(GW == 8, "16-lane rows of two 8-lane halves");
        const float mx = mirror_upper_half(xix), my = mirror_upper_half(xiy);
        static_for<0, 4>([&](auto SS) {
            constexpr int S = decltype(SS)::value;
            const int K = helper ? S ^ 7 : S;
            if constexpr (S == 0) pair_consts(mx, my, K, 6);
            else pair_consts(xor_lane<S>(mx), xor_lane<S>(my), K, (S ^ 7) - 1);
        });
        static_for<1, 4>([&](auto SS) {
            constexpr int S = decltype(SS)::value, J = (S ^ 7) - 1;
            ex[S - 1] = ex[J];
            ey[S - 1] = ey[J];
            fx[S - 1] = fx[J];
            fy[S - 1] = fy[J];
            bp[S - 1] = bp[J];
            emax[S - 1] = emax[J];
        });
        static_for<3, 7>([&](auto JJ) {
            constexpr int J = decltype(JJ)::value;
            auto cross = [](float v) { return RG_ROW_SWAP_HALVES ? swap_halves(v) : to_lower_half(v); };
            ex[J] = cross(ex[J]);
            ey[J] = cross(ey[J]);
            fx[J] = cross(fx[J]);
            fy[J] = cross(fy[J]);
            bp[J] = cross(bp[J]);
            emax[J] = cross(emax[J]);
        });
    } else {
        static_for<1, GW>([&](auto KK) {
            constexpr int K = decltype(KK)::value;
            pair_consts(xor_lane<K>(xix), xor_lane<K>(xiy), K, K - 1);
        });
    }
    static_for<0, GW - 1>([&](auto KK) { mu[decltype(KK)::value] = dmu[decltype(KK)::value] = 0.0f; });
    RG_CTRL_PIN_ROUNDS(GW, fx, bp, emax)
    RG_CTRL_TICK(0);
    {
        const float n2u = ux * ux + uy * uy;
        const bool clip = n2u > k.bml * k.bml;
        if (__any(clip)) {
            const float sc = k.bml / __builtin_sqrtf(n2u);
            ux = clip ? ux * sc : ux;
            uy = clip ? uy * sc : uy;
        }
    }
    const float uhx = ux, uhy = uy;
    bool active = upd & !helper;
    int sweeps = 0, my_sweeps = 0;
    auto sweep = [&](auto PH) {
        constexpr int PHASE = decltype(PH)::value;
        ++sweeps;
        if (active) {
            float chg = 0.0f, pa = 0.0f, pb = 0.0f;
            static_for<1, GW>([&](auto KK) {
                constexpr int K = decltype(KK)::value;
                const float pux = xor_lane<K>(ux), puy = xor_lane<K>(uy);
                const float c0 = mu[K - 1] - bp[K - 1];
                const float t = __builtin_fmaf(fy[K - 1], puy - uy, c0);
                float mn = __builtin_fmaf(fx[K - 1], pux - ux, t);
                mn = (mn > 0.0f) ? mn : 0.0f;
                const float delta = mn - mu[K - 1];
                mu[K - 1] = mn;
                ux = __builtin_fmaf(delta, ex[K - 1], ux);
                uy = __builtin_fmaf(delta, ey[K - 1], uy);
                chg = fmaxf(chg, __builtin_fabsf(delta) * emax[K - 1]);
                if constexpr (PHASE == 2) dmu[K - 1] = delta;
                if constexpr (PHASE == 3) {
                    const float dd = delta - dmu[K - 1];
                    pa = __builtin_fmaf(dd, delta, pa);
                    pb = __builtin_fmaf(dd, dd, pb);
                    dmu[K - 1] = delta;
                }
            });
            my_sweeps = sweeps;
            const float um = lane_ok ? fmaxf(__builtin_fabsf(ux), __builtin_fabsf(uy)) : 0.0f;
            const float gchg = group_max_nonneg<GW>(chg);
            const float gum = fmaxf(k.bml, group_max_nonneg<GW>(um));
            active = (gchg > qp_rtol * gum) & (sweeps < qp_cap);
            if constexpr (PHASE == 3) {
                if (active) {
                    const float ga = group_sum<GW>(pa), gb = group_sum<GW>(pb);
                    const bool ok = (gb > 0.0f) & (ga < 0.0f) & (-ga < 32.0f * gb);
                    const float gam = ok ? ga / gb : 0.0f;
                    float sx = uhx, sy = uhy;
                    static_for<1, GW>([&](auto KK) {
                        constexpr int K = decltype(KK)::value;
                        float m = __builtin_fmaf(-gam, dmu[K - 1], mu[K - 1]);
                        m = (m > 0.0f) ? m : 0.0f;
                        mu[K - 1] = m;
                        sx = __builtin_fmaf(m, ex[K - 1], sx);
                        sy = __builtin_fmaf(m, ey[K - 1], sy);
                    });
                    ux = sx;
                    uy = sy;
                }
            }
        }
    };
    if constexpr (SPAN) {
        while (active) {
            sweep(std::integral_constant<int, 1>{});
            if (!active) break;
            sweep(std::integral_constant<int, 2>{});
            if (!active) break;
            sweep(std::integral_constant<int, 3>{});
            if (!active) break;
            sweep(std::integral_constant<int, 0>{});
        }
    } else {
        while (__any(active)) {
            sweep(std::integral_constant<int, 1>{});
            if (!__any(active)) break;
            sweep(std::integral_constant<int, 2>{});
            if (!__any(active)) break;
            sweep(std::integral_constant<int, 3>{});
            if (!__any(active)) break;
            sweep(std::integral_constant<int, 0>{});
        }
    }
    if constexpr (SPAN) {
        ux = to_upper_half(ux);
        uy = to_upper_half(uy);
    }
    RG_CTRL_PIN2(ux, uy);
    RG_CTRL_TICK(1);
    float vv = c * ux + s * uy;
    float ww = k.inv_pd * (-s * ux + c * uy);
    ww = ww > k.wlim ? k.wlim : ww;
    ww = ww < -k.wlim ? -k.wlim : ww;
    vv = vv > k.vmax ? k.vmax : vv;
    vv = vv < -k.vmax ? -k.vmax : vv;
    ww = ww > k.wmax ? k.wmax : ww;
    ww = ww < -k.wmax ? -k.wmax : ww;
    v = upd ? vv : v;
    w = upd ? ww : w;
    RG_CTRL_PIN2(v, w);
    RG_CTRL_COUNT_SWEEPS(sweeps);
    RG_CTRL_TICK(2);
    return my_sweeps;
}

template <int GW, int OD, int NT, bool SPAN = false>
__device__ __forceinline__ void write_neighbour_obs(Lds<GW> &lds, int N, int Knb, int ag, int gbase, bool lane_ok,
                                                    float x, float y, float *obs_row) {
    constexpr int M = NT > 0 ? NT - 1 : GW - 1;
    constexpr int S = SPAN ? (M + 1) / 2 : M;
    const int r0 = SPAN && (threadIdx.x & GW) != 0 ? S : 0;
    unsigned long long key[S > 0 ? S : 1], okey[S > 0 ? S : 1];
    bool ok[S > 0 ? S : 1];
    int rank[S > 0 ? S : 1], who[S > 0 ? S : 1];
    static_for<0, S>([&](auto RR) {
        constexpr int l = decltype(RR)::value;
        const int r = r0 + l;
        int j = ag + r + 1;
        j = j >= N ? j - N : j;
        j = j & (GW - 1);
        who[l] = j;
        const float2 pxy = *reinterpret_cast<const float2 *>(&lds.own[gbase + j][0]);
        const float dx = pxy.x - x, dy = pxy.y - y;
        const float d2 = dx * dx + dy * dy;
        ok[l] = lane_ok & (r + 1 < N);
        if constexpr (SPAN) ok[l] &= r < M;
        const unsigned int hi = ok[l] ? __builtin_bit_cast(unsigned int, d2) : 0xFFFFFFFFu;
        key[l] = (static_cast<unsigned long long>(hi) << 32) | static_cast<unsigned int>(j);
        if constexpr (SPAN) {
            const unsigned int ohi = static_cast<unsigned int>(xor_lane_i<8>(static_cast<int>(hi)));
            okey[l] = (static_cast<unsigned long long>(ohi) << 32) | static_cast<unsigned int>(xor_lane_i<8>(j));
        }
        rank[l] = S - 1 - l;
    });
    const bool all_others = Knb >= N - 1;
    static_for<1, S>([&](auto KK) {
        constexpr int k = decltype(KK)::value;
        static_for<0, k>([&](auto QQ) {
            constexpr int q = decltype(QQ)::value;
            const int q_first = key[q] < key[k] ? 1 : 0;
            rank[k] += q_first;
            rank[q] -= q_first;
        });
    });
    if constexpr (SPAN) {
        static_for<0, S>([&](auto LL) {
            constexpr int l = decltype(LL)::value;
            static_for<0, S>([&](auto QQ) { rank[l] += okey[decltype(QQ)::value] < key[l] ? 1 : 0; });
        });
    }
    float row[S > 0 ? S : 1][OD];
    static_for<0, S>([&](auto RR) {
        constexpr int r = decltype(RR)::value;
        const float *src = &lds.own[gbase + who[r]][0];
        if constexpr (OD == 4) {
            const float4 v = *reinterpret_cast<const float4 *>(src);
            row[r][0] = v.x;
            row[r][1] = v.y;
            row[r][2] = v.z;
            row[r][3] = v.w;
        } else {
#pragma unroll
            for (int c = 0; c < OD; ++c) row[r][c] = src[c];
        }
    });
    static_for<0, S>([&](auto RR) {
        constexpr int r = decltype(RR)::value;
        const int j = who[r];
        const int slot = all_others ? (j < ag ? j : j - 1) : rank[r];
        if (ok[r] & (all_others | (slot < Knb))) {
            float *o = obs_row + (slot + 1) * OD;
            if constexpr (OD == 4) {
                out_store4(o, row[r][0], row[r][1], row[r][2], row[r][3]);
            } else {
#pragma unroll
                for (int c = 0; c < OD; ++c) o[c] = row[r][c];
            }
        }
    });
}

template <int SCN, int GW, bool OBS_ONLY, int NT, bool AHEAD, bool GYM, int QPM = 0, typename QpLds = void, typename Sync = WgSync,
          bool LIDAR = false, bool TEAM = false, bool SPAN = false, bool NOISE = false, bool RES = false>
__device__ __forceinline__ void step_once(const KernelArgs &a, Lds<GW> &lds, const StepView &sv, QpLds *qp_lds = nullptr,
                                          const rg_lidar_params *lid = nullptr, const rg_team_params *tm = nullptr,
                                          const DisturbScale *nz = nullptr) {
    static_assert(!SPAN || (GW == 8 && QPM == 0 && !GYM && !LIDAR && !TEAM && !NOISE), "the 16-lane rows: exact mode, GW = 8, no side blocks");
    static_assert(!NOISE || !OBS_ONLY, "an observation-only launch displaces nothing");
    static_assert(!RES || (SPAN && RG_ROW_ARG_REGS != 0), "the resident form: the 16-lane rows, arguments in vector registers");
    constexpr int RW = SPAN ? 2 * GW : GW;
    constexpr int EPW = WAVE / RW;
    RG_STAMPS_BEGIN()
    const rg_scenario_params &p = a.p;
    const Consts &k = a.k;
    constexpr bool ARGV = SPAN && RG_ROW_ARG_REGS != 0;
    int av[ARG_REGS] = {0, 0, 0, 0, 0};
    if constexpr (RES) load_arg_regs_resident(a, threadIdx.x, av);
    else if constexpr (ARGV) load_arg_regs(a, threadIdx.x, av);
#define RG_ARG_BLOCK_OFF(f) static_cast<unsigned>(reinterpret_cast<const char *>(&(f)) - reinterpret_cast<const char *>(&a))
#define RG_ARG_OFF(f) (RES ? resident_arg_off(RG_ARG_BLOCK_OFF(f)) : RG_ARG_BLOCK_OFF(f))
#define RG_ARG(f) (ARGV ? arg_reg<std::decay_t<decltype(f)>>(av, RG_ARG_OFF(f)) : (f))
#define RG_ARG_OR(f, q) (ARGV ? arg_reg<std::decay_t<decltype(q)>>(av, RG_ARG_OFF(f)) : (q))
#define RG_OUT(m) (ARGV ? arg_reg<std::decay_t<decltype(sv.io.m)>>(av, RG_ARG_OFF(a.io.m)) : (sv.io.m))
    auto arg_elem = [&](const auto &array, int i) {
        const unsigned off = static_cast<unsigned>(reinterpret_cast<const char *>(&array) - reinterpret_cast<const char *>(&a));
        return __builtin_amdgcn_readlane(av[off >> 8], static_cast<int>((off >> 2) & 63) + i);
    };
    static_assert(offsetof(KernelArgs, p.torque) / 256 == (offsetof(KernelArgs, p.torque) + sizeof(rg_scenario_params::torque) - 1) / 256,
                  "arg_elem(p.torque, j): the table lies in one of the argument registers");
#define RG_IMG(ptr) (RES ? as_global(ptr) : (ptr))
#define RG_SAMPLER_ARGS (RES ? reopened_image(a) : (a))
    const float *q_poses = RG_IMG(a.st.poses), *q_carry = RG_IMG(a.st.carry_dist), *q_ret = RG_IMG(a.st.ep_return), *q_sum = RG_IMG(a.st.done_return_sum);
    const int32_t *q_steps = RG_IMG(a.st.episode_steps), *q_act = sv.actions, *q_cnt = RG_IMG(a.st.done_count), *q_stp = RG_IMG(a.st.done_steps_sum);
    int32_t *q_el = GYM ? sv.io.elapsed : nullptr;
    const int q_tl = GYM ? sv.io.time_limit : 0;
    const int32_t *q_rc = RG_IMG(a.st.reset_count), *q_nep = AHEAD ? RG_IMG(a.st.next_episode) : nullptr;
    const float *q_nin = AHEAD ? RG_IMG(a.st.next_init) : nullptr;
    const int q_nst = AHEAD ? a.next_stride : 0;
    const int q_E = a.E, q_epw = a.envs_per_wave, q_P = p.num_prey, q_N = p.n_agents, q_G = RES ? sv.grid : gridDim.x;
    asm volatile("" ::"s"(q_poses), "s"(q_carry), "s"(q_ret), "s"(q_sum), "s"(q_steps), "s"(q_act), "s"(q_cnt), "s"(q_stp),
                 "s"(q_E), "s"(q_epw), "s"(q_P), "s"(q_N), "s"(q_G), "s"(q_rc));
    if constexpr (GYM) asm volatile("" ::"s"(q_el), "s"(q_tl));
    if constexpr (AHEAD) asm volatile("" ::"s"(q_nep), "s"(q_nin), "s"(q_nst));
    const float *q_prey = RG_IMG(a.st.prey_loc);
    const uint8_t *q_sen = RG_IMG(a.st.prey_sensed), *q_cap = RG_IMG(a.st.prey_captured), *q_loaded = RG_IMG(a.st.loaded), *q_grid = RG_IMG(a.st.grid);
    const uint8_t *q_pix = RG_IMG(a.st.pixel_type), *q_reached = RG_IMG(a.st.reached_goal);
    const int32_t *q_gcol = RG_IMG(a.st.goal_col), *q_msg = RG_IMG(a.st.messages), *q_zone = RG_IMG(a.st.zone_load), *q_load = RG_IMG(a.st.load);
    if constexpr (SCN == RG_SCN_PREDATOR_CAPTURE_PREY) asm volatile("" ::"s"(q_prey), "s"(q_sen), "s"(q_cap));
    else if constexpr (SCN == RG_SCN_WAREHOUSE) asm volatile("" ::"s"(q_loaded));
    else if constexpr (SCN == RG_SCN_SIMPLE) asm volatile("" ::"s"(q_prey));
    else if constexpr (SCN == RG_SCN_ARCTIC_TRANSPORT) asm volatile("" ::"s"(q_grid), "s"(q_pix), "s"(q_reached), "s"(q_gcol));
    else asm volatile("" ::"s"(q_msg), "s"(q_zone), "s"(q_load));
    int32_t *q_tidx = TEAM ? tm->team_index : nullptr;
    const float *q_tstep = TEAM ? tm->agent_step : nullptr, *q_tsr = TEAM ? tm->sensing_radius : nullptr;
    const float *q_tcr = TEAM ? tm->capture_radius : nullptr;
    const int32_t *q_ttq = TEAM ? tm->torque : nullptr;
    const int q_tC = TEAM ? tm->n_sets : 1;
    if constexpr (TEAM) {
        asm volatile("" ::"s"(q_tidx), "s"(q_tstep), "s"(q_tC));
        if constexpr (SCN == RG_SCN_PREDATOR_CAPTURE_PREY) asm volatile("" ::"s"(q_tsr), "s"(q_tcr));
        else if constexpr (SCN == RG_SCN_MATERIAL_TRANSPORT) asm volatile("" ::"s"(q_ttq));
    }

    const uint64_t q_seed = NOISE ? a.seed : 0;
    const int64_t q_off = NOISE ? a.env_offset : 0;
    const float q_kxy = NOISE ? nz->k_xy : 0.0f, q_kth = NOISE ? nz->k_theta : 0.0f;
    if constexpr (NOISE) asm volatile("" ::"s"(q_seed), "s"(q_off), "s"(q_kxy), "s"(q_kth));

    const int N = NT > 0 ? NT : q_N;
    const int lane = threadIdx.x;
    const int ag = lane & (GW - 1);
    const int g = lane / RW;
    const int gbase = lane & ~(RW - 1);
    const bool helper = SPAN && (lane & GW) != 0;
    const int epw = q_epw > 0 ? q_epw : EPW;
    const int chunk = xcd_chunk(q_G);
    const int e = chunk * epw + g;
    const bool env_ok = (g < epw) & (e < q_E);
    const bool lane_ok = env_ok && ag < N;
    const bool env_st = env_ok & !helper, lane_st = lane_ok & !helper;
    const bool lane_nb = SPAN ? lane_ok : lane_st;
    const size_t eN = static_cast<size_t>(e) * N;

#define RG_LATE(v) asm volatile("" : "+v"(v))
    float x = 0.0f, y = 0.0f, th = 0.0f, carry = 0.0f;
    int act = 4;
    int steps_raw = 0;
    float agent_step = 0.0f, sr = 0.0f, cr = 0.0f;
    float st_ret = 0.0f, st_sum = 0.0f;
    int st_cnt = 0, st_steps = 0;
    const bool stats = (!OBS_ONLY) && q_ret != nullptr;
    int pix = 0, reached = 0;
    int team_raw = 0, tq_raw = 0;
    if constexpr (TEAM) {
        if (env_ok) team_raw = q_tidx[e];
    }
    int nz_rc = 0, nz_steps = 0;
    if constexpr (NOISE) {
        if (env_ok) {
            nz_rc = q_rc[e];
            nz_steps = q_steps[e];
        }
    }
    if (lane_ok) {
        const float *X = q_poses + eN * 3;
        x = X[ag];
        y = X[N + ag];
        th = X[2 * N + ag];
        if constexpr (!OBS_ONLY) act = q_act[eN + ag];
        if constexpr (SCN == RG_SCN_ARCTIC_TRANSPORT) pix = q_pix[eN + ag];
        if constexpr (!TEAM) {
        agent_step = p.agent_step[ag];
        if constexpr (SCN == RG_SCN_PREDATOR_CAPTURE_PREY) {
            sr = p.sensing_radius[ag];
            cr = p.capture_radius[ag];
        }
        }
        if constexpr (!OBS_ONLY) carry = q_carry[eN + ag];
        if constexpr (TEAM) {
            const size_t ti = static_cast<size_t>(team_clamp(team_raw, q_tC)) * N + ag;
            agent_step = q_tstep[ti];
            if constexpr (SCN == RG_SCN_PREDATOR_CAPTURE_PREY) {
                sr = q_tsr[ti];
                cr = q_tcr[ti];
            }
            if constexpr (SCN == RG_SCN_MATERIAL_TRANSPORT) tq_raw = q_ttq[ti];
        }
    }
    int rc_raw = -1;
    const bool ahead = AHEAD && (!OBS_ONLY) && q_nst > 0 && *sv.auto_reset;
    int nx_tag = -2;
    float nx_pose[3] = {0.0f, 0.0f, 0.0f};
    float nx_a = 0.0f, nx_b = 0.0f;
    uint32_t nx_grid[7] = {0, 0, 0, 0, 0, 0, 0};
    auto load_next = [&](bool want) {
        if (want) {
            const auto nb = RG_ARG_OR(a.st.next_init, q_nin) + static_cast<size_t>(e) * RG_ARG_OR(a.next_stride, q_nst);
            if (ag < N) {
                nx_pose[0] = nb[ag];
                nx_pose[1] = nb[N + ag];
                nx_pose[2] = nb[2 * N + ag];
            }
            if constexpr (SCN == RG_SCN_PREDATOR_CAPTURE_PREY || SCN == RG_SCN_SIMPLE) {
                if (ag < RG_ARG_OR(p.num_prey, q_P)) {
                    nx_a = nb[3 * N + 2 * ag];
                    nx_b = nb[3 * N + 2 * ag + 1];
                }
            } else if constexpr (SCN == RG_SCN_MATERIAL_TRANSPORT) {
                if (ag < 2) nx_a = nb[3 * N + ag];
            } else if constexpr (SCN == RG_SCN_ARCTIC_TRANSPORT) {
                const uint32_t *gb = reinterpret_cast<const uint32_t *>(nb + 3 * N);
#pragma unroll
                for (int t = 0; t < 6; ++t) nx_grid[t] = gb[ag * 6 + t];
                nx_grid[6] = gb[24];
            }
        }
    };
    int el_raw = 0;
    if (env_ok) {
        steps_raw = q_steps[e];
        if (!OBS_ONLY && *sv.auto_reset) rc_raw = q_rc[e];
        if constexpr (GYM) el_raw = q_el[e];
        if (ahead) nx_tag = q_nep[e];
        if (stats && ag == 0) {
            st_ret = q_ret[e];
            st_sum = q_sum[e];
            st_cnt = q_cnt[e];
            st_steps = q_stp[e];
        }
    }
    uint32_t sen_lo = 0, sen_hi = 0, cap_lo = 0, cap_hi = 0;
    int flag_raw[4] = {0, 0, 0, 0};
    int loaded = 0;
    float goal_x = 0.0f, goal_y = 0.0f;
    uint32_t grid_pre[6] = {0, 0, 0, 0, 0, 0};
    int goal_col = 1;
    int load = 0, zone0 = 0, zone1 = 0;
    int msg[4] = {0, 0, 0, 0};
    float2 prey_r[8];
#pragma unroll
    for (int t = 0; t < 8; ++t) prey_r[t] = make_float2(0.0f, 0.0f);
    static_assert(SCN != RG_SCN_ARCTIC_TRANSPORT || GW == 4, "ArcticTransport is a 4-agent scenario");
    if constexpr (SCN == RG_SCN_PREDATOR_CAPTURE_PREY) {
        const int P = q_P;
        if (P <= 8) {
            if (env_ok) {
                const float2 *src = reinterpret_cast<const float2 *>(q_prey) + static_cast<size_t>(e) * P;
                if constexpr (SPAN) {
                    const int t0 = helper ? 4 : 0;
#pragma unroll
                    for (int t = 0; t < 4; ++t) prey_r[t] = src[t0 + t < P ? t0 + t : P - 1];
                } else {
#pragma unroll
                for (int t = 0; t < 8; ++t) prey_r[t] = src[t < P ? t : P - 1];
                }
                if (ag < P) {
                    flag_raw[0] = q_sen[static_cast<size_t>(e) * P + ag];
                    flag_raw[1] = q_cap[static_cast<size_t>(e) * P + ag];
                }
                if constexpr (GW < 8)
                    if (ag + GW < P) {
                        flag_raw[2] = q_sen[static_cast<size_t>(e) * P + ag + GW];
                        flag_raw[3] = q_cap[static_cast<size_t>(e) * P + ag + GW];
                    }
            }
        } else {
            if (env_ok) {
                for (int i = ag; i < 2 * P; i += GW) lds.prey[g][i] = q_prey[static_cast<size_t>(e) * 2 * P + i];
                for (int i = ag; i < P; i += GW) {
                    const uint32_t sb = q_sen[static_cast<size_t>(e) * P + i] != 0;
                    const uint32_t cb = q_cap[static_cast<size_t>(e) * P + i] != 0;
                    if (i < 32) {
                        sen_lo |= sb << i;
                        cap_lo |= cb << i;
                    } else {
                        sen_hi |= sb << (i - 32);
                        cap_hi |= cb << (i - 32);
                    }
                }
            }
            sen_lo = group_or<GW>(sen_lo);
            cap_lo = group_or<GW>(cap_lo);
            if (P > 32) {
                sen_hi = group_or<GW>(sen_hi);
                cap_hi = group_or<GW>(cap_hi);
            }
        }
    } else if constexpr (SCN == RG_SCN_WAREHOUSE) {
        if (lane_ok) loaded = q_loaded[eN + ag];
    } else if constexpr (SCN == RG_SCN_SIMPLE) {
        if (env_ok) {
            goal_x = q_prey[static_cast<size_t>(e) * 2];
            goal_y = q_prey[static_cast<size_t>(e) * 2 + 1];
        }
    } else if constexpr (SCN == RG_SCN_ARCTIC_TRANSPORT) {
        if (env_ok) {
            const uint32_t *gsrc = reinterpret_cast<const uint32_t *>(q_grid + static_cast<size_t>(e) * 96);
#pragma unroll
            for (int t = 0; t < 6; ++t) grid_pre[t] = gsrc[ag * 6 + t];
            goal_col = q_gcol[e];
        }
        if (lane_ok) reached = q_reached[eN + ag];
    } else {
        if (env_ok) {
#pragma unroll
            for (int i = 0; i < 4; ++i) {
                if (OBS_ONLY || i >= N) msg[i] = q_msg[4 * e + i];
                else msg[i] = q_act[eN + i];
            }
            zone0 = q_zone[2 * e];
            zone1 = q_zone[2 * e + 1];
        }
        if (lane_ok) load = q_load[eN + ag];
    }

    if constexpr (NOISE) {
        RG_LATE(nz_rc);
        RG_LATE(nz_steps);
        int nz_c[3];
        disturb_draw(static_cast<uint64_t>(q_off + e), nz_rc - 1, nz_steps, ag, q_seed, nz_c);
        float dx = x, dy = y, dth = th;
        disturb_pose(q_kxy, q_kth, nz_c, dx, dy, dth);
        x = lane_ok ? dx : x;
        y = lane_ok ? dy : y;
        th = lane_ok ? dth : th;
    }

    int viol = 0, max_sweeps = 0;
    bool replayed = false;
    float dist = 0.0f;
    if constexpr (!OBS_ONLY) {
        RG_PIN5(x, y, th, carry, act);
        RG_STAMP(0);
        float gx = x, gy = y;
        {
            const int mv = (SCN == RG_SCN_MATERIAL_TRANSPORT) ? act / 4 : act;
            float sd = agent_step;
            if constexpr (SCN == RG_SCN_ARCTIC_TRANSPORT) {
                const float nrm_s = p.arctic_normal_step, slow_s = p.arctic_slow_step, fast_s = p.arctic_fast_step;
                const float water = pix == 1 ? slow_s : pix == 2 ? fast_s : nrm_s;
                const float ice = pix == 1 ? fast_s : pix == 2 ? slow_s : nrm_s;
                sd = ag < 2 ? fast_s : ag == 3 ? water : ice;
            }
            const float cgx = clamp_spec(gx, p.left, p.right), cgy = clamp_spec(gy, p.up, p.down);
            const float lft = (gx - sd) > p.left ? (gx - sd) : p.left;
            const float rgt = (gx + sd) < p.right ? (gx + sd) : p.right;
            const float upw = (gy - sd) > p.up ? (gy - sd) : p.up;
            const float dwn = (gy + sd) < p.down ? (gy + sd) : p.down;
            gx = mv == 0 ? lft : mv == 1 ? rgt : cgx;
            gy = mv == 2 ? upw : mv == 3 ? dwn : cgy;
        }
        const int thr_pre = __builtin_bit_cast(int, k.thr_pre);
        const int ghost_q = __builtin_bit_cast(int, __builtin_amdgcn_cvt_pkrtz(1000.0f + 32.0f * ag, -1000.0f));
        float v = 0.0f, w = 0.0f, s = 0.0f, c = 1.0f;
        RG_CHUNK_LOCALS()
        RG_CTRL_LOCALS()
        float acc = carry, last = 0.0f;
        bool dead = false;
        float fin_x = 0.0f, fin_y = 0.0f;
        float bx = x, by = y, ox = 0.0f, oy = 0.0f;
        const bool penalize = p.penalize_violations != 0;
        const int U = p.update_frequency, period = p.controller_period;
        for (int it0 = 0; it0 < U; it0 += period) {
            const int n = (U - it0) < period ? (U - it0) : period;
            RG_HEADING_SINCOS(th, s, c);
            const int sw = controller<GW, QPM, QpLds, SPAN>(p, k, N, ag, lane_ok, env_ok & !dead, x, y, c, s, gx, gy, v, w, qp_lds RG_CTRL_TICKS_ARG);
            max_sweeps = sw > max_sweeps ? sw : max_sweeps;
            const float dtv = k.dt * v, dtw = k.dt * w;
            float sd, cd;
            sincos_small_spec(dtw, sd, cd);
            if (__any(__builtin_fabsf(dtw) > 0.25f)) {
                float sd2, cd2;
                sincos_spec(dtw, sd2, cd2);
                const bool big = __builtin_fabsf(dtw) > 0.25f;
                sd = big ? sd2 : sd;
                cd = big ? cd2 : cd;
            }
            if (it0 == 0) RG_STAMP(1);
            const float mrg = __builtin_fmaf((CHUNK - 1) * 1.000001f, __builtin_fabsf(dtv), PRE_SLACK);
            int n_exec = n;
            bool died_now = false;
            const float mstep = lane_ok ? __builtin_fmaf(__builtin_fabsf(k.coll_off), __builtin_fabsf(dtw), __builtin_fabsf(dtv)) * 1.00001f : 0.0f;
            const float M2 = 2.0f * group_max_nonneg<GW>(mstep);
            auto thr_span = [&](int span) {
                const float t = (k.lin_pre + PRE_SLACK) + static_cast<float>(span) * M2;
                return __builtin_bit_cast(int, (t * t) * 1.00002f);
            };
            const int thr_s1 = thr_span(1), thr_s2 = thr_span(2);
            const bool sparse_ok = (k.lin_pre + 2.0f * M2) < 0.24f;

            auto run_chunk = [&](auto CC, int j0) {
                constexpr int C = decltype(CC)::value;
                const float x0 = x, y0 = y, ox0 = ox, oy0 = oy, c0 = c, s0 = s;
                const bool live = lane_ok & !dead;
                int q[C];
                const bool bnd_any = live & ((__builtin_fabsf(x - k.xc) + mrg > k.xh) | (__builtin_fabsf(y - k.yc) + mrg > k.yh));
                static_for<0, C>([&](auto UU) {
                    constexpr int u = decltype(UU)::value;
                    const float fx = __builtin_fmaf(k.coll_off, c, x), fy = __builtin_fmaf(k.coll_off, s, y);
                    const int qr = __builtin_bit_cast(int, __builtin_amdgcn_cvt_pkrtz(fx, fy));
                    q[u] = live ? qr : ghost_q;
                    ox = __builtin_fmaf(c, dtv, ox);
                    oy = __builtin_fmaf(s, dtv, oy);
                    x = bx + ox;
                    y = by + oy;
                    const float cn = __builtin_fmaf(c, cd, -(s * sd));
                    const float sn = __builtin_fmaf(s, cd, c * sd);
                    c = cn;
                    s = sn;
                });
                auto pair_min = [&](int qv) {
                    constexpr bool QUAD_COVER = GW == 8 && NT >= 5 && NT <= 7;
                    constexpr int R = QUAD_COVER ? NT - 1 : GW - 1;
                    int d[R];
                    auto diff = [&](int partner_q) {
                        return __builtin_bit_cast(int, __builtin_bit_cast(half2v, qv) - __builtin_bit_cast(half2v, partner_q));
                    };
                    if constexpr (QUAD_COVER) {
                        static_for<1, 4>([&](auto KK) { d[decltype(KK)::value - 1] = diff(xor_lane_i<decltype(KK)::value>(qv)); });
                        static_for<0, NT - 4>([&](auto MM) { d[3 + decltype(MM)::value] = diff(cross_lane_i<decltype(MM)::value>(qv)); });
                    } else {
                        static_for<1, GW>([&](auto KK) { d[decltype(KK)::value - 1] = diff(xor_lane_i<decltype(KK)::value>(qv)); });
                    }
                    int dm = 0x7FFFFFFF;
                    dot2_batch<R>(d);
#pragma unroll
                    for (int r = 0; r < R; ++r) dm = d[r] < dm ? d[r] : dm;
                    return dm;
                };
                int dmin_u[C];
                bool sparse_hit = live & !sparse_ok;
                {
                    constexpr int SPAN0 = C - 1 < 2 ? C - 1 : 2;
                    const int t0 = SPAN0 == 0 ? thr_pre : SPAN0 == 1 ? thr_s1 : thr_s2;
                    if constexpr (SPAN && C >= 4) {
                        const int t3 = C == 4 ? thr_pre : thr_s1;
                        const int dm = pair_min(helper ? q[3] : q[0]);
                        sparse_hit = sparse_hit | (dm <= (helper ? t3 : t0));
                        dmin_u[0] = dmin_u[3] = dm;
                    } else {
                        dmin_u[0] = pair_min(q[0]);
                        sparse_hit = sparse_hit | (dmin_u[0] <= t0);
                        if constexpr (C >= 4) {
                            const int t3 = C == 4 ? thr_pre : thr_s1;
                            dmin_u[3] = pair_min(q[3]);
                            sparse_hit = sparse_hit | (dmin_u[3] <= t3);
                        }
                    }
                }
                if (penalize && __any(sparse_hit | bnd_any)) {
                RG_CHUNK_DENSE_BEGIN()
                if constexpr (SPAN && C >= 4) {
                    const int mine = dmin_u[0], other = xor_lane_i<8>(mine);
                    dmin_u[0] = helper ? other : mine;
                    dmin_u[3] = helper ? mine : other;
                }
                if constexpr (SPAN && C >= 3) {
                    const int mine = pair_min(helper ? q[2] : q[1]), other = xor_lane_i<8>(mine);
                    if constexpr (C == 5) dmin_u[4] = pair_min(q[4]);
                    dmin_u[1] = helper ? other : mine;
                    dmin_u[2] = helper ? mine : other;
                } else {
                    static_for<1, C>([&](auto UU) {
                        constexpr int u = decltype(UU)::value;
                        if constexpr (u != 3) dmin_u[u] = pair_min(q[u]);
                    });
                }
                int dmin = dmin_u[0];
                static_for<1, C>([&](auto UU) { dmin = dmin_u[decltype(UU)::value] < dmin ? dmin_u[decltype(UU)::value] : dmin; });
                RG_CHUNK_DENSE_END(dmin)
                if (__any((dmin <= thr_pre) | bnd_any)) {
                    replayed = true;
                    float rx = x0, ry = y0, rox = ox0, roy = oy0, rc = c0, rs = s0;
                    static_for<0, C>([&](auto UU) {
                        constexpr int u = decltype(UU)::value;
                        const bool bnd = lane_ok & !dead & ((rx < k.xmin) | (rx > k.xmax) | (ry < k.ymin) | (ry > k.ymax));
                        const float fx = __builtin_fmaf(k.coll_off, rc, rx), fy = __builtin_fmaf(k.coll_off, rs, ry);
                        bool col = false;
                        if (!__any(dmin_u[u] <= thr_pre)) {
                        } else if constexpr (GW == 8 && NT >= 5 && NT <= 7) {
                            static_for<1, 4>([&](auto KK) {
                                constexpr int K = decltype(KK)::value;
                                const float dx = fx - xor_lane<K>(fx), dy = fy - xor_lane<K>(fy);
                                col = col | (((ag ^ K) < N) & (dx * dx + dy * dy <= k.coll_lim2));
                            });
                            static_for<0, NT - 4>([&](auto MM) {
                                constexpr int M = decltype(MM)::value;
                                const float dx = fx - cross_lane<M>(fx), dy = fy - cross_lane<M>(fy);
                                col = col | (dx * dx + dy * dy <= k.coll_lim2);
                            });
                        } else {
                            static_for<1, GW>([&](auto KK) {
                                constexpr int K = decltype(KK)::value;
                                const float dx = fx - xor_lane<K>(fx), dy = fy - xor_lane<K>(fy);
                                col = col | (((ag ^ K) < N) & (dx * dx + dy * dy <= k.coll_lim2));
                            });
                        }
                        col = col & lane_ok & !dead;
                        const int code = (group_any<GW>(col, gbase) ? 1 : 0) | (group_any<GW>(bnd, gbase) ? 2 : 0);
                        rox = __builtin_fmaf(rc, dtv, rox);
                        roy = __builtin_fmaf(rs, dtv, roy);
                        rx = bx + rox;
                        ry = by + roy;
                        if (env_ok & !dead & (code != 0)) {
                            viol = code;
                            n_exec = j0 + u + 1;
                            died_now = true;
                            dead = true;
                            fin_x = rx;
                            fin_y = ry;
                        }
                        const float cn = __builtin_fmaf(rc, cd, -(rs * sd));
                        const float sn = __builtin_fmaf(rs, cd, rc * sd);
                        rc = cn;
                        rs = sn;
                    });
                    RG_CHUNK_REPLAY_END(rx, ry)
                }
                }
            };
            int j = 0;
            for (; j + CHUNK <= n; j += CHUNK) run_chunk(std::integral_constant<int, CHUNK>{}, j);
            static_for<1, CHUNK>([&](auto RR) {
                if (n - j == decltype(RR)::value) run_chunk(RR, j);
            });

            const bool upd = env_ok & (!dead | died_now);
            const float ne = static_cast<float>(n_exec);
            const float adv = __builtin_fabsf(dtv);
            th = upd ? wrap_spec(__builtin_fmaf(ne, dtw, th)) : th;
            acc = upd ? __builtin_fmaf(ne, adv, acc) : acc;
            last = upd ? adv : last;
            {
                const float tx = x - bx, ty = y - by;
                ox = (bx - (x - tx)) + (ox - tx);
                oy = (by - (y - ty)) + (oy - ty);
                bx = x;
                by = y;
            }
            if (it0 == 0) RG_STAMP(2);
            if (!__any(env_ok & !dead)) break;
        }
        if (dead) {
            x = fin_x;
            y = fin_y;
        }
        dist = viol ? acc : acc - last;
        carry = last;
        RG_STAMP(3);
        RG_CTRL_REPORT()
        RG_CHUNK_REPORT()
    }

    const int D = RG_ARG(p.obs_dim);
    const auto obs_row = RG_OUT(obs) + (eN + ag) * D;
    const bool ahead_e = ARGV ? AHEAD && (!OBS_ONLY) && RG_ARG(a.next_stride) > 0 && RG_ARG(a.auto_reset) : ahead;
    const bool stats_e = ARGV ? (!OBS_ONLY) && RG_ARG(a.st.ep_return) != nullptr : stats;
    bool done = false;
    int remaining = -1;
    float reward = 0.0f;
    RG_LATE(steps_raw);
    const int steps = steps_raw + (OBS_ONLY ? 0 : 1);
    RG_LATE(rc_raw);
    RG_LATE(nx_tag);
    const bool have_next = ahead_e & (nx_tag == rc_raw);
    const bool next_early = env_ok & have_next & ((viol != 0) | (steps > RG_ARG(p.max_episode_steps)));
    if constexpr (AHEAD) load_next(next_early & !helper);

    if constexpr (SCN == RG_SCN_PREDATOR_CAPTURE_PREY) {
        const int P = RG_ARG_OR(p.num_prey, q_P);
        if constexpr (TEAM) {
            RG_LATE(sr);
            RG_LATE(cr);
        }
        const float sr2 = sr * sr, cr2 = cr * cr;
        if (P > 8) Sync::sync();
        if (P <= 8) {
            RG_LATE(flag_raw[0]);
            RG_LATE(flag_raw[1]);
            uint32_t sb = (flag_raw[0] != 0 ? 1u : 0u) << ag, cb = (flag_raw[1] != 0 ? 1u : 0u) << ag;
            if constexpr (GW < 8) {
                RG_LATE(flag_raw[2]);
                RG_LATE(flag_raw[3]);
                sb |= (flag_raw[2] != 0 ? 1u : 0u) << (ag + GW);
                cb |= (flag_raw[3] != 0 ? 1u : 0u) << (ag + GW);
            }
            sen_lo = group_or<GW>(sb);
            cap_lo = group_or<GW>(cb);
        }
        uint32_t nsen_lo = sen_lo, nsen_hi = sen_hi, ncap_lo = cap_lo, ncap_hi = cap_hi;
        auto scan = [&](int lo, int hi, auto &&f) {
            for (int i0 = lo; i0 < hi; i0 += 4) {
                float2 pl[4];
#pragma unroll
                for (int t = 0; t < 4; ++t) {
                    const int i = (i0 + t) < hi ? (i0 + t) : (hi - 1);
                    pl[t] = *reinterpret_cast<const float2 *>(&lds.prey[g][2 * i]);
                }
#pragma unroll
                for (int t = 0; t < 4; ++t) {
                    const float dx = x - pl[t].x, dy = y - pl[t].y;
                    f(i0 + t, (i0 + t) < hi, pl[t].x, pl[t].y, dx * dx + dy * dy);
                }
            }
        };
        float closest = -1.0f, qx = -5.0f, qy = -5.0f;
        if (SPAN && P <= 8) {
            const float2 (&pl)[8] = prey_r;
            const int t0 = helper ? 4 : 0;
            const bool acts = lane_ok & (act == 4);
            const float sr2e = lane_ok ? sr2 : -1.0f, cr2e = acts ? cr2 : -1.0f;
            float d2[4];
            uint32_t m = 0;
#pragma unroll
            for (int t = 0; t < 4; ++t) {
                const float dx = x - pl[t].x, dy = y - pl[t].y;
                d2[t] = dx * dx + dy * dy;
                m |= (d2[t] <= sr2e ? 1u : 0u) << t;
                m |= (d2[t] <= cr2e ? 1u : 0u) << (8 + t);
            }
            m <<= t0;
            m = group_or<GW>(m);
            m |= static_cast<uint32_t>(xor_lane_i<8>(static_cast<int>(m)));
            const uint32_t in_p = (1u << P) - 1u;
            if constexpr (!OBS_ONLY) {
                const uint32_t s_b = m & in_p, c_b = (m >> 8) & in_p;
                nsen_lo = sen_lo | (s_b & ~cap_lo);
                ncap_lo = cap_lo | (nsen_lo & c_b & ~cap_lo);
                if (env_st && ag < P) {
                    RG_ARG(a.st.prey_sensed)[static_cast<size_t>(e) * P + ag] = (nsen_lo >> ag) & 1u;
                    RG_ARG(a.st.prey_captured)[static_cast<size_t>(e) * P + ag] = (ncap_lo >> ag) & 1u;
                }
            }
            const uint32_t cap_l = (ncap_lo | ~in_p) >> t0;
#pragma unroll
            for (int t = 0; t < 4; ++t) {
                const bool cap = ((cap_l >> t) & 1u) != 0;
                const bool take = !cap & (d2[t] <= sr2) & ((d2[t] < closest) | (closest == -1.0f));
                qx = take ? pl[t].x : qx;
                qy = take ? pl[t].y : qy;
                closest = take ? d2[t] : closest;
            }
            const float o_closest = xor_lane<8>(closest), o_qx = xor_lane<8>(qx), o_qy = xor_lane<8>(qy);
            const bool other = (o_closest != -1.0f) & ((closest == -1.0f) | (o_closest < closest));
            qx = other ? o_qx : qx;
            qy = other ? o_qy : qy;
        } else if (P <= 8) {
            const float2 (&pl)[8] = prey_r;
            float d2[8];
            uint32_t s_b = 0, c_b = 0;
            const bool acts = lane_ok & (act == 4);
#pragma unroll
            for (int t = 0; t < 8; ++t) {
                const float dx = x - pl[t].x, dy = y - pl[t].y;
                d2[t] = dx * dx + dy * dy;
                const bool in = t < P;
                s_b |= ((in & lane_ok & (d2[t] <= sr2)) ? 1u : 0u) << t;
                c_b |= ((in & acts & (d2[t] <= cr2)) ? 1u : 0u) << t;
            }
            if constexpr (!OBS_ONLY) {
                s_b = group_or<GW>(s_b);
                c_b = group_or<GW>(c_b);
                nsen_lo = sen_lo | (s_b & ~cap_lo);
                ncap_lo = cap_lo | (nsen_lo & c_b & ~cap_lo);
                if (env_st && ag < P) {
                    a.st.prey_sensed[static_cast<size_t>(e) * P + ag] = (nsen_lo >> ag) & 1u;
                    a.st.prey_captured[static_cast<size_t>(e) * P + ag] = (ncap_lo >> ag) & 1u;
                }
                if constexpr (GW < 8)
                    if (env_ok && ag + GW < P) {
                        a.st.prey_sensed[static_cast<size_t>(e) * P + ag + GW] = (nsen_lo >> (ag + GW)) & 1u;
                        a.st.prey_captured[static_cast<size_t>(e) * P + ag + GW] = (ncap_lo >> (ag + GW)) & 1u;
                    }
            }
#pragma unroll
            for (int t = 0; t < 8; ++t) {
                const bool cap = ((ncap_lo >> t) & 1u) != 0;
                const bool take = (t < P) & !cap & (d2[t] <= sr2) & ((d2[t] < closest) | (closest == -1.0f));
                qx = take ? pl[t].x : qx;
                qy = take ? pl[t].y : qy;
                closest = take ? d2[t] : closest;
            }
        } else {
        if constexpr (!OBS_ONLY) {
            uint32_t s_lo = 0, s_hi = 0, c_lo = 0, c_hi = 0;
            const bool acts = lane_ok & (act == 4);
            const int P32 = P < 32 ? P : 32;
            scan(0, P32, [&](int i, bool in, float, float, float d2) {
                s_lo |= ((in & lane_ok & (d2 <= sr2)) ? 1u : 0u) << (i & 31);
                c_lo |= ((in & acts & (d2 <= cr2)) ? 1u : 0u) << (i & 31);
            });
            s_lo = group_or<GW>(s_lo);
            c_lo = group_or<GW>(c_lo);
            nsen_lo = sen_lo | (s_lo & ~cap_lo);
            ncap_lo = cap_lo | (nsen_lo & c_lo & ~cap_lo);
            if (P > 32) {
                scan(32, P, [&](int i, bool in, float, float, float d2) {
                    s_hi |= ((in & lane_ok & (d2 <= sr2)) ? 1u : 0u) << ((i - 32) & 31);
                    c_hi |= ((in & acts & (d2 <= cr2)) ? 1u : 0u) << ((i - 32) & 31);
                });
                s_hi = group_or<GW>(s_hi);
                c_hi = group_or<GW>(c_hi);
                nsen_hi = sen_hi | (s_hi & ~cap_hi);
                ncap_hi = cap_hi | (nsen_hi & c_hi & ~cap_hi);
            }
            if (env_st) {
                for (int i = ag; i < P; i += GW) {
                    const uint32_t sw_ = i < 32 ? nsen_lo >> i : nsen_hi >> (i - 32);
                    const uint32_t cw_ = i < 32 ? ncap_lo >> i : ncap_hi >> (i - 32);
                    RG_ARG(a.st.prey_sensed)[static_cast<size_t>(e) * P + i] = sw_ & 1u;
                    RG_ARG(a.st.prey_captured)[static_cast<size_t>(e) * P + i] = cw_ & 1u;
                }
            }
        }
        {
            auto nearest = [&](uint32_t capmask, int base) {
                return [&, capmask, base](int i, bool in, float px, float py, float d2) {
                    const bool cap = ((capmask >> ((i - base) & 31)) & 1u) != 0;
                    const bool take = in & !cap & (d2 <= sr2) & ((d2 < closest) | (closest == -1.0f));
                    qx = take ? px : qx;
                    qy = take ? py : qy;
                    closest = take ? d2 : closest;
                };
            };
            scan(0, P < 32 ? P : 32, nearest(ncap_lo, 0));
            if (P > 32) scan(32, P, nearest(ncap_hi, 32));
        }
        }
        RG_STAMP_E(0);
        const int od = RG_ARG(p.capability_aware) ? 6 : 4;
        lds.own[lane][0] = x;
        lds.own[lane][1] = y;
        lds.own[lane][2] = qx;
        lds.own[lane][3] = qy;
        lds.own[lane][4] = sr;
        lds.own[lane][5] = cr;
        Sync::sync();
        if (od == 6) {
            if (lane_st) {
#pragma unroll
                for (int cc = 0; cc < 6; ++cc) obs_row[cc] = lds.own[lane][cc];
            }
            write_neighbour_obs<GW, 6, NT, SPAN>(lds, N, RG_ARG(p.num_neighbors), ag, gbase, lane_nb, x, y, obs_row);
        } else {
            if (lane_st) out_store4(obs_row, x, y, qx, qy);
            write_neighbour_obs<GW, 4, NT, SPAN>(lds, N, RG_ARG(p.num_neighbors), ag, gbase, lane_nb, x, y, obs_row);
        }
        RG_STAMP_E(1);
        if constexpr (!OBS_ONLY) {
            const int unseen0 = P - __builtin_popcount(sen_lo) - __builtin_popcount(sen_hi);
            const int left0 = P - __builtin_popcount(cap_lo) - __builtin_popcount(cap_hi);
            const int unseen1 = P - __builtin_popcount(nsen_lo) - __builtin_popcount(nsen_hi);
            const int left1 = P - __builtin_popcount(ncap_lo) - __builtin_popcount(ncap_hi);
            if (viol) {
                reward = RG_ARG(p.violation_reward);
                done = true;
            } else {
                reward = 0.0f;
                reward = reward + static_cast<float>(unseen0 - unseen1) * RG_ARG(p.sense_reward);
                reward = reward + static_cast<float>(left0 - left1) * RG_ARG(p.capture_reward);
                reward = reward + RG_ARG(p.time_penalty);
                if (steps > RG_ARG(p.max_episode_steps) || left1 == 0) {
                    done = true;
                    remaining = left1;
                }
            }
        }
    } else if constexpr (SCN == RG_SCN_WAREHOUSE) {
        lds.own[lane][0] = x;
        lds.own[lane][1] = y;
        lds.own[lane][2] = loaded ? 1.0f : 0.0f;
        Sync::sync();
        if (lane_st) {
            obs_row[0] = x;
            obs_row[1] = y;
            obs_row[2] = loaded ? 1.0f : 0.0f;
        }
        write_neighbour_obs<GW, 3, NT, SPAN>(lds, N, RG_ARG(p.num_neighbors), ag, gbase, lane_nb, x, y, obs_row);
        if constexpr (!OBS_ONLY) {
            if (viol) {
                reward = RG_ARG(p.violation_reward);
                done = true;
            } else {
                const bool green = (ag % 2) == 0;
                if (loaded) {
                    if (x < -1.5f + RG_ARG(p.goal_width) && ((green && y > 0.0f) || (!green && y <= 0.0f))) {
                        reward = RG_ARG(p.unload_reward);
                        loaded = 0;
                    }
                } else {
                    if (x > 1.5f - RG_ARG(p.goal_width) && ((!green && y > 0.0f) || (green && y <= 0.0f))) {
                        reward = RG_ARG(p.load_reward);
                        loaded = 1;
                    }
                }
                done = steps > RG_ARG(p.max_episode_steps);
                if (lane_st) RG_ARG(a.st.loaded)[eN + ag] = static_cast<uint8_t>(loaded);
            }
        }
    } else if constexpr (SCN == RG_SCN_SIMPLE) {
        lds.own[lane][0] = x;
        lds.own[lane][1] = y;
        Sync::sync();
        if (lane_st) {
            obs_row[0] = x;
            obs_row[1] = y;
            obs_row[2 * N] = goal_x;
            obs_row[2 * N + 1] = goal_y;
        }
        write_neighbour_obs<GW, 2, NT, SPAN>(lds, N, N - 1, ag, gbase, lane_nb, x, y, obs_row);
        if constexpr (!OBS_ONLY) {
            if (viol) {
                reward = RG_ARG(p.violation_reward);
                done = true;
            } else {
                const float dx = x - goal_x, dy = y - goal_y;
                const float r = -(dx * dx + dy * dy);
                reward = r * RG_ARG(p.reward_scaler);
                done = steps > RG_ARG(p.max_episode_steps);
            }
        }
    } else if constexpr (SCN == RG_SCN_ARCTIC_TRANSPORT) {
        {
            uint32_t *gdst = reinterpret_cast<uint32_t *>(&lds.grid[g][0]);
#pragma unroll
            for (int t = 0; t < 6; ++t) gdst[ag * 6 + t] = grid_pre[t];
        }
        Sync::sync();
        const uint8_t *grid = &lds.grid[g][0];
        int row = -static_cast<int>((y - 1.0f) / 0.25f), col = static_cast<int>((x + 1.5f) / 0.25f);
        row = row < 0 ? 0 : row > 7 ? 7 : row;
        col = col < 0 ? 0 : col > 11 ? 11 : col;
        if constexpr (!OBS_ONLY) {
            pix = grid[row * 12 + col];
            reached = reached | (pix == 3 ? 1 : 0);
        }
        const int here = grid[row * 12 + col];
        lds.own[lane][0] = x;
        lds.own[lane][1] = y;
        lds.own[lane][2] = static_cast<float>(here);
        lds.aload[lane] = row * 16 + col;
        Sync::sync();
        const float goalx = static_cast<float>(goal_col) * 0.25f - 1.5f, goaly = -1.0f * 0.25f + 0.75f;
        if (lane_ok) {
            obs_row[0] = x;
            obs_row[1] = y;
            obs_row[2] = static_cast<float>(here);
            const int o0 = ag == 0 ? 1 : ag == 1 ? 0 : ag == 2 ? 3 : 2;
            const int o1 = ag < 2 ? 2 : 0, o2 = ag < 2 ? 3 : 1;
            const int oth[3] = {o0, o1, o2};
#pragma unroll
            for (int m = 0; m < 3; ++m) {
                obs_row[3 + 3 * m + 0] = lds.own[gbase + oth[m]][0];
                obs_row[3 + 3 * m + 1] = lds.own[gbase + oth[m]][1];
                obs_row[3 + 3 * m + 2] = lds.own[gbase + oth[m]][2];
            }
            obs_row[12] = goalx;
            obs_row[13] = goaly;
#pragma unroll
            for (int i = 0; i < 2; ++i) {
                const int rc = lds.aload[gbase + i];
                const int r_ = rc >> 4, c_ = rc & 15;
                const int left = c_ > 0 ? c_ - 1 : c_, right = c_ < 11 ? c_ + 1 : c_;
                const int up = r_ > 0 ? r_ - 1 : r_, down = r_ < 7 ? r_ + 1 : r_;
                float *o = obs_row + 14 + 8 * i;
                o[0] = static_cast<float>(grid[up * 12 + left]);
                o[1] = static_cast<float>(grid[r_ * 12 + left]);
                o[2] = static_cast<float>(grid[down * 12 + left]);
                o[3] = static_cast<float>(grid[up * 12 + c_]);
                o[4] = static_cast<float>(grid[down * 12 + c_]);
                o[5] = static_cast<float>(grid[up * 12 + right]);
                o[6] = static_cast<float>(grid[r_ * 12 + right]);
                o[7] = static_cast<float>(grid[down * 12 + right]);
            }
        }
        if constexpr (LIDAR) write_lidar<SCN, GW, OBS_ONLY, Sync>(*lid, a, lds, lane, gbase, N, ag, lane_ok, x, y, th, obs_row);
        if constexpr (!OBS_ONLY) {
            const float dx = x - goalx, dy = y - goaly;
            lds.ax[lane] = dx * dx + dy * dy;
            lds.ay[lane] = static_cast<float>(pix * 2 + reached);
            Sync::sync();
            if (viol) {
                reward = p.violation_reward;
                done = true;
            } else {
                reward = 0.0f;
                bool all_reached = true;
#pragma unroll
                for (int j = 2; j < 4; ++j) {
                    const int pr = static_cast<int>(lds.ay[gbase + j]);
                    const bool rj = (pr & 1) != 0;
                    if (!rj) reward = reward + p.not_reached_penalty;
                    if ((pr >> 1) != 3) reward = reward + p.dist_multiplier * lds.ax[gbase + j];
                    all_reached = all_reached && rj;
                }
                done = steps > p.max_episode_steps;
                if (!done) done = all_reached;
            }
            if (lane_ok) {
                a.st.pixel_type[eN + ag] = static_cast<uint8_t>(pix);
                a.st.reached_goal[eN + ag] = static_cast<uint8_t>(reached);
            }
        }
    } else {
#pragma unroll
        for (int i = 0; i < 4; ++i) {
            RG_LATE(msg[i]);
            if (!OBS_ONLY && i < N) msg[i] = msg[i] % 4;
        }
        if constexpr (TEAM) RG_LATE(tq_raw);
        if (lane_st) {
            obs_row[0] = x;
            obs_row[1] = y;
            obs_row[2] = static_cast<float>(load);
            obs_row[3] = static_cast<float>(zone0);
            obs_row[4] = static_cast<float>(zone1);
#pragma unroll
            for (int i = 0; i < 4; ++i) obs_row[5 + i] = static_cast<float>(msg[i]);
            if (RG_ARG(p.capability_aware)) {
                if constexpr (TEAM) obs_row[9] = static_cast<float>(tq_raw);
                else obs_row[9] = static_cast<float>(p.torque[ag]);
                obs_row[10] = agent_step;
            }
        }
        if constexpr (!OBS_ONLY) {
            lds.ax[lane] = x;
            lds.ay[lane] = y;
            lds.aload[lane] = load;
            if constexpr (TEAM) team_lds<SCN, GW>().torque[lane] = tq_raw;
            Sync::sync();
            if (viol) {
                reward = RG_ARG(p.violation_reward);
                done = true;
            } else {
                reward = RG_ARG(p.time_penalty);
                const float egw = RG_ARG(p.end_goal_width);
                const float zr2 = RG_ARG(p.zone1_radius) * RG_ARG(p.zone1_radius);
                bool any_load = false;
                for (int j = 0; j < N; ++j) {
                    const float jx = lds.ax[gbase + j], jy = lds.ay[gbase + j];
                    int jl = lds.aload[gbase + j];
                    int tq;
                    if constexpr (TEAM) tq = team_lds<SCN, GW>().torque[gbase + j];
                    else if constexpr (ARGV) tq = arg_elem(p.torque, j);
                    else tq = p.torque[j];
                    if (jl > 0) {
                        if (jx < -1.5f + egw) {
                            reward = reward + static_cast<float>(jl) * RG_ARG(p.unload_multiplier);
                            jl = 0;
                        }
                    } else {
                        if (jx > 1.5f - egw) {
                            if (zone1 > tq) {
                                jl = tq;
                                zone1 -= tq;
                            } else {
                                jl = zone1;
                                zone1 = 0;
                            }
                            reward = reward + static_cast<float>(jl) * RG_ARG(p.load_multiplier);
                        } else if (jx * jx + jy * jy <= zr2) {
                            if (zone0 > tq) {
                                jl = tq;
                                zone0 -= tq;
                            } else {
                                jl = zone0;
                                zone0 = 0;
                            }
                            reward = reward + static_cast<float>(jl) * RG_ARG(p.load_multiplier);
                        }
                    }
                    if (j == ag) load = jl;
                    any_load = any_load || (jl != 0);
                }
                done = steps > RG_ARG(p.max_episode_steps);
                if (!done) done = (zone0 == 0 && zone1 == 0 && !any_load);
            }
            int total = 0;
            {
                lds.aload[lane] = lane_ok ? load : 0;
                Sync::sync();
                for (int j = 0; j < N; ++j) total += lds.aload[gbase + j];
            }
            if (done) remaining = zone0 + zone1 + total;
            if (lane_st) RG_ARG(a.st.load)[eN + ag] = load;
            if (lane_st && ag == 0) {
                RG_ARG(a.st.zone_load)[2 * e] = zone0;
                RG_ARG(a.st.zone_load)[2 * e + 1] = zone1;
            }
            if (lane_st && ag < 4) RG_ARG(a.st.messages)[4 * e + ag] = msg[ag == 0 ? 0 : ag == 1 ? 1 : ag == 2 ? 2 : 3];
        }
    }

    if constexpr (LIDAR && SCN != RG_SCN_ARCTIC_TRANSPORT) write_lidar<SCN, GW, OBS_ONLY, Sync>(*lid, a, lds, lane, gbase, N, ag, lane_ok, x, y, th, obs_row);
    RG_STAMP(4);
    if constexpr (!OBS_ONLY) {
        constexpr bool gym = GYM;
        bool trunc = false;
        if (gym) {
            RG_LATE(el_raw);
            trunc = env_ok & !done & (el_raw + 1 >= q_tl);
        }
        const bool ended = done | trunc;
        float rsum = 0.0f;
        if ((stats_e && !RG_ARG(p.shared_reward)) || gym) {
            Sync::sync();
            lds.ax[lane] = lane_ok ? reward : 0.0f;
            Sync::sync();
            for (int j = 0; j < N; ++j) rsum = rsum + lds.ax[gbase + j];
        }
        if (lane_st) {
            const auto X = RG_ARG(a.st.poses) + eN * 3;
            X[ag] = x;
            X[N + ag] = y;
            X[2 * N + ag] = th;
            RG_ARG(a.st.carry_dist)[eN + ag] = carry;
            out_store1(RG_OUT(reward) + eN + ag, reward);
            out_store1(RG_OUT(dist_travelled) + eN + ag, dist);
            if (ag == 0) {
                RG_ARG(a.st.episode_steps)[e] = steps;
                if (stats_e) {
                    RG_LATE(st_ret);
                    RG_LATE(st_sum);
                    RG_LATE(st_cnt);
                    RG_LATE(st_steps);
                    float ret = st_ret + (RG_ARG(p.shared_reward) ? reward : rsum);
                    if (ended) {
                        RG_ARG(a.st.done_return_sum)[e] = st_sum + ret;
                        RG_ARG(a.st.done_count)[e] = st_cnt + 1;
                        RG_ARG(a.st.done_steps_sum)[e] = st_steps + steps;
                        ret = 0.0f;
                    }
                    RG_ARG(a.st.ep_return)[e] = ret;
                }
                RG_OUT(done)[e] = done ? 1 : 0;
                if (gym) {
                    q_el[e] = ended ? 0 : el_raw + 1;
                    sv.io.truncated[e] = trunc ? 1 : 0;
                    sv.io.ended[e] = ended ? 1 : 0;
                    sv.io.reward_sum[e] = rsum;
                }
                RG_OUT(violation)[e] = static_cast<uint8_t>(viol);
                RG_OUT(remaining)[e] = remaining;
                if (RG_OUT(qp_sweeps)) RG_OUT(qp_sweeps)[e] = max_sweeps;
            }
            if constexpr (GYM) {
                if (sv.io.zero_obs_on_end && ended) {
                    for (int c = 0; c < D; ++c) obs_row[c] = 0.0f;
                }
            }
        }
        RG_STAMP(5);
        if (RG_ARG(a.auto_reset) && __any(env_ok & ended)) {
            Sync::sync();
            if constexpr (AHEAD) load_next(env_st & ended & have_next & !next_early);
            if (__any(env_ok & ended & !have_next)) reset_group<SCN, GW, Sync>(RG_SAMPLER_ARGS, lds, e, g, ag, env_st & ended & !have_next, rc_raw, sv.seed);
            if (env_st & ended & have_next) {
                if (ag < N) {
                    const auto X = RG_ARG(a.st.poses) + eN * 3;
                    X[ag] = nx_pose[0];
                    X[N + ag] = nx_pose[1];
                    X[2 * N + ag] = nx_pose[2];
                    RG_ARG(a.st.carry_dist)[eN + ag] = 0.0f;
                    if constexpr (SCN == RG_SCN_WAREHOUSE) RG_ARG(a.st.loaded)[eN + ag] = 0;
                    if constexpr (SCN == RG_SCN_MATERIAL_TRANSPORT) {
                        RG_ARG(a.st.load)[eN + ag] = 0;
                        if (ag < 4) RG_ARG(a.st.messages)[4 * e + ag] = 0;
                    }
                    if constexpr (SCN == RG_SCN_ARCTIC_TRANSPORT) {
                        a.st.pixel_type[eN + ag] = 0;
                        a.st.reached_goal[eN + ag] = 0;
                    }
                }
                if constexpr (SCN == RG_SCN_PREDATOR_CAPTURE_PREY || SCN == RG_SCN_SIMPLE) {
                    const int P = RG_ARG_OR(p.num_prey, q_P);
                    const auto nb = RG_ARG_OR(a.st.next_init, q_nin) + static_cast<size_t>(e) * RG_ARG_OR(a.next_stride, q_nst) + 3 * N;
                    for (int i = ag; i < P; i += GW) {
                        const auto pl = RG_ARG(a.st.prey_loc) + (static_cast<size_t>(e) * P + i) * 2;
                        pl[0] = i == ag ? nx_a : nb[2 * i];
                        pl[1] = i == ag ? nx_b : nb[2 * i + 1];
                        if constexpr (SCN == RG_SCN_PREDATOR_CAPTURE_PREY) {
                            RG_ARG(a.st.prey_sensed)[static_cast<size_t>(e) * P + i] = 0;
                            RG_ARG(a.st.prey_captured)[static_cast<size_t>(e) * P + i] = 0;
                        }
                    }
                } else if constexpr (SCN == RG_SCN_MATERIAL_TRANSPORT) {
                    if (ag < 2) RG_ARG(a.st.zone_load)[2 * e + ag] = __builtin_bit_cast(int32_t, nx_a);
                } else if constexpr (SCN == RG_SCN_ARCTIC_TRANSPORT) {
                    uint32_t *gd = reinterpret_cast<uint32_t *>(a.st.grid + static_cast<size_t>(e) * 96);
#pragma unroll
                    for (int t = 0; t < 6; ++t) gd[ag * 6 + t] = nx_grid[t];
                    if (ag == 0) a.st.goal_col[e] = static_cast<int32_t>(nx_grid[6]);
                }
                if (ag == 0) {
                    RG_ARG(a.st.reset_count)[e] = rc_raw + 1;
                    RG_ARG(a.st.episode_steps)[e] = 0;
                }
            }
            if constexpr (TEAM) {
                if (env_ok & ended & (ag == 0)) q_tidx[e] = team_draw(*tm, static_cast<uint64_t>(a.env_offset + e), rc_raw, a.seed);
            }
        }
        if (AHEAD && ahead_e && !(replayed | __any(max_sweeps > 2)) && __any(env_ok & !ended & !have_next)) {
            const bool need = env_st & !ended & !have_next;
            Sync::sync();
            reset_group<SCN, GW, Sync>(RG_SAMPLER_ARGS, lds, e, g, ag, need, rc_raw, reset_dst_next(RG_SAMPLER_ARGS, e), sv.seed);
            if (need && ag == 0) RG_ARG(a.st.next_episode)[e] = rc_raw;
        }
        RG_STAMP(6);
        RG_STAMPS_WRITE(lane, sv.io.qp_sweeps, chunk * EPW, a.E, max_sweeps)
    }
}

#undef RG_ARG
#undef RG_ARG_BLOCK_OFF
#undef RG_IMG
#undef RG_SAMPLER_ARGS
#undef RG_ARG_OFF
#undef RG_ARG_OR
#undef RG_OUT

struct PlainFamily {
    using Args = KernelArgs;
    static constexpr bool LIDAR = false, TEAM = false, NOISE = false, READDRESS = false;
    static Args args(const KernelArgs &a, const GroupSide &) { return a; }
    __device__ __forceinline__ static const KernelArgs &kernel_args(const Args &x) { return x; }
    __device__ __forceinline__ static const rg_lidar_params *lidar(const Args &) { return nullptr; }
    __device__ __forceinline__ static const rg_team_params *teams(const Args &) { return nullptr; }
    __device__ __forceinline__ static const DisturbScale *disturb(const Args &) { return nullptr; }
};
struct LidarFamily {
    using Args = LidarArgs;
    static constexpr bool LIDAR = true, TEAM = false, NOISE = false, READDRESS = true;
    static Args args(const KernelArgs &a, const GroupSide &side) { return Args{a, *side.lidar}; }
    __device__ __forceinline__ static const KernelArgs &kernel_args(const Args &x) { return x.k; }
    __device__ __forceinline__ static const rg_lidar_params *lidar(const Args &x) { return &x.lid; }
    __device__ __forceinline__ static const rg_team_params *teams(const Args &) { return nullptr; }
    __device__ __forceinline__ static const DisturbScale *disturb(const Args &) { return nullptr; }
};
struct TeamFamily {
    using Args = TeamArgs;
    static constexpr bool LIDAR = false, TEAM = true, NOISE = false, READDRESS = true;
    static Args args(const KernelArgs &a, const GroupSide &side) { return Args{a, *side.teams}; }
    __device__ __forceinline__ static const KernelArgs &kernel_args(const Args &x) { return x.k; }
    __device__ __forceinline__ static const rg_lidar_params *lidar(const Args &) { return nullptr; }
    __device__ __forceinline__ static const rg_team_params *teams(const Args &x) { return &x.tp; }
    __device__ __forceinline__ static const DisturbScale *disturb(const Args &) { return nullptr; }
};
struct DisturbFamily {
    using Args = DisturbArgs;
    static constexpr bool LIDAR = false, TEAM = false, NOISE = true, READDRESS = true;
    static Args args(const KernelArgs &a, const GroupSide &side) { return Args{a, *side.disturb}; }
    __device__ __forceinline__ static const KernelArgs &kernel_args(const Args &x) { return x.k; }
    __device__ __forceinline__ static const rg_lidar_params *lidar(const Args &) { return nullptr; }
    __device__ __forceinline__ static const rg_team_params *teams(const Args &) { return nullptr; }
    __device__ __forceinline__ static const DisturbScale *disturb(const Args &x) { return &x.ds; }
};

template <class F>
__device__ __forceinline__ const typename F::Args &rollout_step_args(const typename F::Args &args) {
    if constexpr (F::READDRESS) return *(const typename F::Args *)kernarg_block<typename F::Args>();
    else return args;
}

template <class F, int SCN, int GW, bool OBS_ONLY, int NT, bool ROLLOUT, bool GYM, int QPM, bool SPAN = false>
__device__ __forceinline__ void step_kernel_body(const typename F::Args &args) {
    constexpr bool IPM = QPM == RG_QP_CVXOPT;
    static_assert(!IPM || GW == 4 || GW == 8, "the interior-point mode admits n_agents <= 8");
    static_assert(!IPM || !OBS_ONLY, "an observation-only launch runs no controller");
    static_assert(!SPAN || (!ROLLOUT && !OBS_ONLY), "the 16-lane rows: the single-step launch");
    __shared__ Lds<GW> lds;
    using Q = std::conditional_t<IPM, ipm::GroupLds<GW>, void>;
    Q *qp_lds = nullptr;
    if constexpr (IPM) {
        __shared__ Q qp_block;
        qp_lds = &qp_block;
    }
    const KernelArgs &a = F::kernel_args(args);
    const int N = NT > 0 ? NT : a.p.n_agents;
    if constexpr (!ROLLOUT) {
        step_once<SCN, GW, OBS_ONLY, NT, true, GYM, QPM, Q, WgSync, F::LIDAR, F::TEAM, SPAN, F::NOISE>(a, lds, step_view(a, 0, N, a.p.obs_dim), qp_lds,
                                                                                                     F::lidar(args), F::teams(args), F::disturb(args));
    } else {
        for (int t = 0; t < a.num_steps; ++t) {
            if (t) __syncthreads();
            const typename F::Args &now = rollout_step_args<F>(args);
            const KernelArgs &at = F::kernel_args(now);
            step_once<SCN, GW, OBS_ONLY, NT, false, false, QPM, Q, WgSync, F::LIDAR, F::TEAM, false, F::NOISE>(at, lds, step_view(at, t, N, at.p.obs_dim), qp_lds,
                                                                                                            F::lidar(now), F::teams(now), F::disturb(now));
        }
    }
}

template <int SCN, int GW, bool OBS_ONLY, int NT, bool ROLLOUT, bool GYM = false, int QPM = 0>
__global__ __launch_bounds__(WAVE) void step_kernel(const KernelArgs a) {
    step_kernel_body<PlainFamily, SCN, GW, OBS_ONLY, NT, ROLLOUT, GYM, QPM>(a);
}
template <int SCN, int GW, bool OBS_ONLY, int NT, bool ROLLOUT, int ROW, std::enable_if_t<ROW == 16, int> = 0>
__global__ __launch_bounds__(WAVE) void step_kernel(const KernelArgs a) {
    step_kernel_body<PlainFamily, SCN, GW, OBS_ONLY, NT, ROLLOUT, false, 0, true>(a);
}
#ifndef RG_HOST_SIM
template <int SCN, int GW, bool OBS_ONLY, int NT, bool ROLLOUT, int ROW, bool RESIDENT, std::enable_if_t<ROW == 16 && RESIDENT, int> = 0>
__global__ __launch_bounds__(WAVE) void step_kernel(const KernelArgs *image, const int32_t *actions, const uint64_t seed, const int32_t auto_reset,
                                                    const int32_t grid, const rg_step_io io) {
    static_assert(GW == 8 && !OBS_ONLY && !ROLLOUT, "the 16-lane rows: the single-step launch at GW 8");
    typedef const __attribute__((address_space(4))) KernelArgs *ConstImage;
    ConstImage ci = (ConstImage)image;
    asm volatile("" : "+s"(ci));
    const KernelArgs &a = *(const KernelArgs *)ci;
    __shared__ Lds<GW> lds;
    const StepView sv = {actions, io, &auto_reset, &seed, grid};
    step_once<SCN, GW, false, NT, true, false, 0, void, WgSync, false, false, true, false, true>(a, lds, sv);
}
#endif
template <int SCN, int GW, bool OBS_ONLY, bool ROLLOUT, bool GYM, int QPM>
__global__ __launch_bounds__(WAVE) void lidar_step_kernel(const LidarArgs la) {
    step_kernel_body<LidarFamily, SCN, GW, OBS_ONLY, 0, ROLLOUT, GYM, QPM>(la);
}
template <int SCN, int GW, bool OBS_ONLY, int NT, bool ROLLOUT, bool GYM, int QPM>
__global__ __launch_bounds__(WAVE) void team_step_kernel(const TeamArgs ta) {
    step_kernel_body<TeamFamily, SCN, GW, OBS_ONLY, NT, ROLLOUT, GYM, QPM>(ta);
}

template <int SCN, int GW, bool ROLLOUT, bool GYM, int QPM>
__global__ __launch_bounds__(WAVE) void disturb_step_kernel(const DisturbArgs da) {
    step_kernel_body<DisturbFamily, SCN, GW, false, 0, ROLLOUT, GYM, QPM>(da);
}

template <int SCN, int GW>
__global__ __launch_bounds__(WAVE) void reset_kernel(const KernelArgs a) {
    constexpr int EPW = WAVE / GW;
    __shared__ Lds<GW> lds;
    const int lane = threadIdx.x;
    const int ag = lane & (GW - 1);
    const int g = lane / GW;
    const int e = blockIdx.x * EPW + g;
    const bool env_ok = e < a.E;
    const bool want = env_ok && (a.reset_mask == nullptr || a.reset_mask[e] != 0);
    if (!__any(want)) return;
    const bool stats = want && ag == 0 && a.st.ep_return != nullptr;
    const int steps_before = stats ? a.st.episode_steps[e] : 0;
    reset_group<SCN, GW>(a, lds, e, g, ag, want);
    if (stats) {
        if ((a.reset_flags & RG_RESET_BOOK_EPISODE) && steps_before > 0) {
            a.st.done_return_sum[e] = a.st.done_return_sum[e] + a.st.ep_return[e];
            a.st.done_count[e] = a.st.done_count[e] + 1;
            a.st.done_steps_sum[e] = a.st.done_steps_sum[e] + steps_before;
        }
        a.st.ep_return[e] = 0.0f;
    }
}

}


namespace rg {

inline int group_width(int N) { return N <= 4 ? 4 : N <= 8 ? 8 : 16; }

struct WaveFill {
    int epw, grid;
};
inline WaveFill wave_fill(int E, int gw) {
    int epw = WAVE / gw;
    if constexpr (!kStampsBuild) {
        while (epw >= 2 && (E + epw / 2 - 1) / (epw / 2) <= RG_MAX_WAVES) epw /= 2;
    }
    return {epw, (E + epw - 1) / epw};
}

template <class F, int SCN, int GW, bool OBS_ONLY, int NT, bool ROLLOUT, bool GYM, int QPM, bool ROWS = false>
static void launch_kernel(const typename F::Args &args, int grid, hipStream_t stream) {
    if constexpr (ROWS) hipLaunchKernelGGL((step_kernel<SCN, GW, OBS_ONLY, NT, ROLLOUT, 16>), dim3(grid), dim3(WAVE), 0, stream, args);
    else if constexpr (F::LIDAR) hipLaunchKernelGGL((lidar_step_kernel<SCN, GW, OBS_ONLY, ROLLOUT, GYM, QPM>), dim3(grid), dim3(WAVE), 0, stream, args);
    else if constexpr (F::TEAM) hipLaunchKernelGGL((team_step_kernel<SCN, GW, OBS_ONLY, NT, ROLLOUT, GYM, QPM>), dim3(grid), dim3(WAVE), 0, stream, args);
    else if constexpr (F::NOISE) hipLaunchKernelGGL((disturb_step_kernel<SCN, GW, ROLLOUT, GYM, QPM>), dim3(grid), dim3(WAVE), 0, stream, args);
    else hipLaunchKernelGGL((step_kernel<SCN, GW, OBS_ONLY, NT, ROLLOUT, GYM, QPM>), dim3(grid), dim3(WAVE), 0, stream, args);
}

template <class F, int SCN, bool OBS_ONLY, bool ROLLOUT, bool GYM, int QPM>
static hipError_t launch_gw(const typename F::Args &args, const GroupSide &side, int gw, int n, bool rows, int grid, hipStream_t stream) {
    constexpr bool EXACT = QPM == RG_QP_EXACT;
    constexpr bool BY_N = EXACT && !OBS_ONLY && !GYM && !F::LIDAR && !F::NOISE;
    constexpr bool ROWS = BY_N && !ROLLOUT && !F::TEAM && !kStampsBuild;
    if (gw == 4) {
        launch_kernel<F, SCN, 4, OBS_ONLY, 0, ROLLOUT, GYM, QPM>(args, grid, stream);
    } else if constexpr (SCN == RG_SCN_ARCTIC_TRANSPORT) {
        return hipErrorInvalidValue;
    } else if (gw == 16) {
        if constexpr (EXACT) launch_kernel<F, SCN, 16, OBS_ONLY, 0, ROLLOUT, GYM, QPM>(args, grid, stream);
        else return hipErrorInvalidValue;
    } else if constexpr (BY_N) {
        auto by_n = [&](auto rows_c) {
            constexpr bool R = decltype(rows_c)::value;
            switch (n) {
                case 5: launch_kernel<F, SCN, 8, false, 5, ROLLOUT, false, QPM, R>(args, grid, stream); break;
                case 6: launch_kernel<F, SCN, 8, false, 6, ROLLOUT, false, QPM, R>(args, grid, stream); break;
                case 7: launch_kernel<F, SCN, 8, false, 7, ROLLOUT, false, QPM, R>(args, grid, stream); break;
                default: launch_kernel<F, SCN, 8, false, 8, ROLLOUT, false, QPM, R>(args, grid, stream); break;
            }
        };
        if constexpr (ROWS) {
            if (rows && side.image) return launch_step_resident(args, side, stream);
        }
        if (ROWS && rows) by_n(std::integral_constant<bool, ROWS>());
        else by_n(std::false_type());
    } else {
        launch_kernel<F, SCN, 8, OBS_ONLY, 0, ROLLOUT, GYM, QPM>(args, grid, stream);
    }
    return hipGetLastError();
}

template <class F, bool OBS_ONLY, bool ROLLOUT, int QPM>
static hipError_t launch_group(const KernelArgs &a_in, const GroupSide &side, hipStream_t stream) {
    static_assert(!OBS_ONLY || (!ROLLOUT && QPM == RG_QP_EXACT), "rg_get_obs is a single launch of the exact mode's kernel");
    static_assert(!OBS_ONLY || !F::NOISE, "rg_get_obs of a disturbed handle is the plain family's launch");
    return for_scenario(a_in.p.scenario, [&](auto scn) -> hipError_t {
        constexpr int SCN = decltype(scn)::value;
        constexpr bool ARCTIC = SCN == RG_SCN_ARCTIC_TRANSPORT;
        if constexpr (ARCTIC && F::TEAM) {
            return hipErrorInvalidValue;
        } else {
            KernelArgs a = a_in;
            int gw = 4;
            WaveFill wf = {WAVE / 4, (a.E + 15) / 16};
            if constexpr (!ARCTIC) {
                gw = group_width(a.p.n_agents);
                wf = wave_fill(a.E, gw);
                if constexpr (!kStampsBuild) a.envs_per_wave = wf.epw;
            }
            const typename F::Args args = F::args(a, side);
            if constexpr (!OBS_ONLY && !ROLLOUT) {
                if (a.io.elapsed)
                    return launch_gw<F, SCN, false, false, true, QPM>(args, side, gw, a.p.n_agents, false, wf.grid, stream);
            }
            const bool rows = a_in.envs_per_wave >= 0 && wf.epw <= 4;
            return launch_gw<F, SCN, OBS_ONLY, ROLLOUT, false, QPM>(args, side, gw, a.p.n_agents, rows, wf.grid, stream);
        }
    });
}

}
```

marbler_amd/vec_env.py:

```python
import ctypes as C

import torch

from . import _lib
from .params import TeamPool, disturbance_params, lidar_params, load_config, make_params, team_pool

VIOLATION_MESSAGES = ("", "collision", "boundary", "collision_boundary")


class VecRobotariumEnv(object):
    def __init__(self, scenario, num_envs, config_path=None, overrides=None, device="cuda:0", seed=0,
                 env_offset=0, auto_reset=True, reference_reset_obs=True, params=None, collect_qp_stats=False, lidar=None,
                 teams=None, disturbance=None):
        self.lib = _lib.load()
        self.scenario = scenario
        self.cfg = None
        if params is None:
            self.cfg = load_config(scenario, config_path, overrides)
            params = make_params(scenario, self.cfg)
            if lidar is None:
                lidar = lidar_params(scenario, self.cfg, params)
            if teams is None:
                teams = team_pool(scenario, self.cfg, params)
            if disturbance is None:
                disturbance = disturbance_params(scenario, self.cfg, params)
        if lidar is not None and int(lidar.rays) == 0:
            lidar = None
        if teams is not None and not isinstance(teams, TeamPool):
            teams = team_pool(scenario, {"teams": teams}, params)
        if teams is not None:
            if teams.n_agents != int(params.n_agents):
                raise ValueError(f"teams: the pool is built for {teams.n_agents} agents, the scenario has {int(params.n_agents)}")
            if lidar is not None:
                raise ValueError("teams: a team pool does not combine with the lidar (lidar_rays > 0)")
        if disturbance is not None and float(disturbance.sigma_xy) == 0.0 and float(disturbance.sigma_theta) == 0.0:
            disturbance = None
        if disturbance is not None and lidar is not None:
            raise ValueError("disturbance: the pose disturbance does not combine with the lidar (lidar_rays > 0)")
        if disturbance is not None and teams is not None:
            raise ValueError("disturbance: the pose disturbance does not combine with a team pool (teams)")
        self.params = params
        self.disturbance = disturbance
        self.teams = teams
        self.lidar = lidar
        self.device = torch.device(device)
        if self.device.type != "cuda":
            raise _lib.RobogymError("VecRobotariumEnv runs on an AMD GPU only (device='cuda:N'); no CPU path exists")
        if not torch.cuda.is_available():
            raise _lib.RobogymError("no HIP device visible to torch; marbler_amd has no CPU fallback")
        self.E = int(num_envs)
        self.N = int(params.n_agents)
        self.D = int(params.obs_dim)
        self.P = int(params.num_prey)
        if seed is None:
            import os
            seed = int.from_bytes(os.urandom(8), "little")
        self.seed = int(seed) & 0xFFFFFFFFFFFFFFFF
        self.env_offset = int(env_offset)
        self.auto_reset = bool(auto_reset)
        self.reference_reset_obs = bool(reference_reset_obs)
        E, N, D, P = self.E, self.N, self.D, max(self.P, 1)
        dev = self.device
        f32, i32, u8 = torch.float32, torch.int32, torch.uint8
        zeros = self._alloc
        self.poses = zeros((E, 3, N,), f32)
        self.carry_dist = zeros((E, N,), f32)
        self.episode_steps = zeros((E,), i32)
        self.reset_count = zeros((E,), i32)
        self.prey_loc = zeros((E, P, 2,), f32)
        self.prey_sensed = zeros((E, P,), u8)
        self.prey_captured = zeros((E, P,), u8)
        self.loaded = zeros((E, N,), u8)
        self.load = zeros((E, N,), i32)
        self.zone_load = zeros((E, 2,), i32)
        self.messages = zeros((E, 4,), i32)
        self.grid = zeros((E, 96,), u8)
        self.goal_col = zeros((E,), i32, fill=1)
        self.pixel_type = zeros((E, N,), u8)
        self.reached_goal = zeros((E, N,), u8)
        self.ep_return = zeros((E,), f32)
        self.done_return_sum = zeros((E,), f32)
        self.done_count = zeros((E,), i32)
        self.done_steps_sum = zeros((E,), i32)
        self.next_init = self.next_episode = None
        if E <= 65536:
            stride = self.lib.rg_next_init_stride(C.byref(params))
            if stride <= 0:
                raise _lib.RobogymError("rg_next_init_stride failed: " + self.lib.rg_last_error().decode())
            self.next_init = zeros((E, stride,), f32)
            self.next_episode = zeros((E,), i32, fill=-1)
        self._alloc_outputs()
        self.qp_sweeps = zeros((E,), i32) if collect_qp_stats else None
        self.team_index = self.team_table = None
        if teams is not None:
            self.team_index = zeros((E,), i32)
            self.team_table = {}
            for k in TeamPool.TABLES:
                v = getattr(teams, k)
                self.team_table[k] = zeros(v.shape, i32 if k == "torque" else f32)
                self.team_table[k].copy_(torch.as_tensor(v))

        if dev.index is None:
            self.device = dev = torch.device("cuda", torch.cuda.current_device())
        self._stream = torch.cuda.current_stream(dev)
        self._stream_ptr = self._stream.cuda_stream
        self._h = self.lib.rg_create(C.byref(params), self.E, self.env_offset, dev.index,
                                     C.c_void_p(self._stream_ptr))
        if not self._h:
            raise _lib.RobogymError("rg_create failed: " + self.lib.rg_last_error().decode())
        st = _lib.RgState(*(t.data_ptr() for t in (
            self.poses, self.carry_dist, self.episode_steps, self.reset_count, self.prey_loc, self.prey_sensed,
            self.prey_captured, self.loaded, self.load, self.zone_load, self.messages, self.grid, self.goal_col,
            self.pixel_type, self.reached_goal, self.ep_return,
            self.done_return_sum, self.done_count, self.done_steps_sum)),
            self.next_init.data_ptr() if self.next_init is not None else None,
            self.next_episode.data_ptr() if self.next_episode is not None else None)
        _lib.check(self.lib.rg_bind_state(self._h, C.byref(st)), "rg_bind_state")
        if self.lidar is not None:
            rc = self.lib.rg_set_lidar(self._h, C.byref(self.lidar))
            if rc != 0:
                msg = "rg_set_lidar failed (%d): %s" % (rc, self.lib.rg_last_error().decode())
                self.lib.rg_destroy(self._h)
                self._h = None
                raise (ValueError if -60 < rc <= -50 else _lib.RobogymError)(msg)
        if self.teams is not None:
            tt = self.team_table
            self._team_params = _lib.RgTeamParams(self.teams.n_sets, self.teams.mode, tt["agent_step"].data_ptr(),
                                                  tt["sensing_radius"].data_ptr(), tt["capture_radius"].data_ptr(),
                                                  tt["torque"].data_ptr(), self.team_index.data_ptr())
            rc = self.lib.rg_set_teams(self._h, C.byref(self._team_params))
            if rc != 0:
                msg = "rg_set_teams failed (%d): %s" % (rc, self.lib.rg_last_error().decode())
                self.lib.rg_destroy(self._h)
                self._h = None
                raise (ValueError if -70 < rc <= -60 else _lib.RobogymError)(msg)
        if self.disturbance is not None:
            rc = self.lib.rg_set_disturbance(self._h, C.byref(self.disturbance))
            if rc != 0:
                msg = "rg_set_disturbance failed (%d): %s" % (rc, self.lib.rg_last_error().decode())
                self.lib.rg_destroy(self._h)
                self._h = None
                raise (ValueError if -80 < rc <= -70 else _lib.RobogymError)(msg)
        self._io = _lib.RgStepIO(self.obs.data_ptr(), self.reward.data_ptr(), self.done_u8.data_ptr(),
                                 self.dist_travelled.data_ptr(), self.violation.data_ptr(),
                                 self.remaining.data_ptr(),
                                 self.qp_sweeps.data_ptr() if self.qp_sweeps is not None else None)
        self._io_ref = C.byref(self._io)
        self._actions_i32 = zeros((E, N), i32)
        self.time_limit = 0
        self.elapsed = self.truncated = self.ended = self.reward_sum = None

    def _alloc_outputs(self):
        E, N, D = self.E, self.N, self.D
        f32, i32, u8 = torch.float32, torch.int32, torch.uint8
        sizes = [("obs", E * N * D * 4), ("reward", E * N * 4), ("dist_travelled", E * N * 4), ("remaining", E * 4),
                 ("done_u8", E), ("violation", E)]
        offs, total = {}, 0
        for name, nbytes in sizes:
            offs[name] = total
            total += (nbytes + 15) // 16 * 16
        self._out_arena = self._alloc((total,), u8)
        self._out_offsets = offs

        def view(name, nbytes, dtype, shape):
            return self._out_arena[offs[name]:offs[name] + nbytes].view(dtype).view(shape)

        self.obs = view("obs", E * N * D * 4, f32, (E, N, D))
        self.reward = view("reward", E * N * 4, f32, (E, N))
        self.dist_travelled = view("dist_travelled", E * N * 4, f32, (E, N))
        self.remaining = view("remaining", E * 4, i32, (E,))
        self.remaining.fill_(-1)
        self.done_u8 = view("done_u8", E, u8, (E,))
        self.done = self.done_u8.view(torch.bool)
        self.violation = view("violation", E, u8, (E,))

    def _alloc(self, shape, dtype, fill=0):
        if fill == 0:
            return torch.zeros(*shape, dtype=dtype, device=self.device)
        return torch.full(tuple(shape), fill, dtype=dtype, device=self.device)

    @property
    def n_agents(self):
        return self.N

    @property
    def num_envs(self):
        return self.E

    def _sync_stream(self):
        ptr = torch.cuda.current_stream(self.device).cuda_stream
        if ptr != self._stream_ptr:
            _lib.check(self.lib.rg_set_stream(self._h, C.c_void_p(ptr)), "rg_set_stream")
            self._stream_ptr = ptr

    def reset(self, mask=None, book_episode=False, reference_rng=None, py_random=None):
        self._sync_stream()
        mptr = None
        if mask is not None:
            mask = mask.to(device=self.device, dtype=torch.uint8).contiguous()
            mptr = mask.data_ptr()
        _lib.check(self.lib.rg_reset(self._h, mptr, self.seed, _lib.RESET_BOOK_EPISODE if book_episode else 0), "rg_reset")
        if self.elapsed is not None:
            if mask is None:
                self.elapsed.zero_()
            else:
                self.elapsed.masked_fill_(mask.bool(), 0)
        if reference_rng is not None:
            self._upload_reference_reset(mask, reference_rng, py_random)
        if self.reference_reset_obs:
            if mask is None:
                self.obs.zero_()
            else:
                self.obs.masked_fill_(mask.bool()[:, None, None], 0.0)
            return self.obs
        return self.get_obs()

    def _upload_reference_reset(self, mask, rng, py_random):
        import numpy as np
        from .reference_reset import draw_reset
        if self.cfg is None:
            raise ValueError("reference_rng needs the scenario config (construct the env from a config, not from params)")
        idx = list(range(self.E)) if mask is None else [int(i) for i in torch.nonzero(mask).flatten().cpu()]
        if not idx:
            return
        draws = [draw_reset(self.scenario, self.cfg, rng, py_random) for _ in idx]
        ix = torch.as_tensor(idx, device=self.device)

        def put(dst, key, dtype):
            arr = np.stack([np.asarray(d[key]) for d in draws]).astype(dtype)
            dst[ix] = torch.as_tensor(arr, device=self.device).reshape((len(idx),) + tuple(dst.shape[1:]))

        put(self.poses, "poses", np.float32)
        if "prey_loc" in draws[0]:
            put(self.prey_loc, "prey_loc", np.float32)
        if "zone_load" in draws[0]:
            put(self.zone_load, "zone_load", np.int32)
        if "grid" in draws[0]:
            put(self.grid, "grid", np.uint8)
            self.goal_col[ix] = torch.as_tensor([d["goal_col"] for d in draws], dtype=torch.int32, device=self.device)

    def enable_time_limit(self, time_limit):
        E, dev = self.E, self.device
        self.time_limit = int(time_limit)
        if self.time_limit < 1:
            raise ValueError("time_limit must be > 0")
        self.elapsed = self._alloc((E,), torch.int32)
        pad = (E + 15) // 16 * 16
        self._gymma_arena = self._alloc((4 * pad + 2 * pad,), torch.uint8)
        self._gymma_pad = pad
        self.reward_sum, self._ended_u8, self._trunc_u8 = self._gymma_views(self._gymma_arena)
        self.truncated, self.ended = self._trunc_u8.view(torch.bool), self._ended_u8.view(torch.bool)
        self._io.elapsed, self._io.truncated = self.elapsed.data_ptr(), self._trunc_u8.data_ptr()
        self._io.ended, self._io.reward_sum = self._ended_u8.data_ptr(), self.reward_sum.data_ptr()
        self._io.time_limit = self.time_limit
        self._io_into = _lib.RgStepIO.from_buffer_copy(self._io)
        self._io_into.zero_obs_on_end = 1
        self._io_into_ref = C.byref(self._io_into)

    def _gymma_views(self, arena):
        E, pad = self.E, self._gymma_pad
        return arena[:4 * E].view(torch.float32), arena[4 * pad:4 * pad + E], arena[5 * pad:5 * pad + E]

    def step_into(self, actions_ptr, obs_ptr, reward_sum_ptr, ended_ptr):
        io = self._io_into
        io.obs, io.reward_sum, io.ended = obs_ptr, reward_sum_ptr, ended_ptr
        return self.lib.rg_step(self._h, actions_ptr, self._io_into_ref, 1 if self.auto_reset else 0, self.seed)

    def gymma_outputs_copy(self):
        r, e, t = self._gymma_views(self._gymma_arena.clone())
        return r, e.view(torch.bool), t.view(torch.bool)

    def step(self, actions):
        self._sync_stream()
        if actions.dtype != torch.int32 or not actions.is_contiguous() or actions.device != self.device:
            self._actions_i32.copy_(actions.reshape(self.E, self.N))
            actions = self._actions_i32
        rc = self.lib.rg_step(self._h, actions.data_ptr(), self._io_ref, 1 if self.auto_reset else 0, self.seed)
        if rc != 0:
            _lib.check(rc, "rg_step")
        return self.obs, self.reward, self.done, self.info

    @property
    def info(self):
        return {"dist_travelled": self.dist_travelled, "violation": self.violation, "remaining": self.remaining}

    def host_step(self, actions):
        if self.E != 1:
            raise ValueError("host_step is the single-env path (num_envs == 1)")
        import numpy as np
        self._sync_stream()
        if getattr(self, "_hs", None) is None:
            o, N, D = self._out_offsets, self.N, self.D
            host = torch.zeros_like(self._out_arena, device="cpu").pin_memory()
            n = host.numpy()
            self._hs = {"act_host": torch.zeros(1, N, dtype=torch.int32).pin_memory(),
                        "act_dev": torch.zeros(1, N, dtype=torch.int32, device=self.device), "host": host,
                        "obs": n[o["obs"]:o["obs"] + N * D * 4].view(np.float32).reshape(N, D),
                        "reward": n[o["reward"]:o["reward"] + N * 4].view(np.float32),
                        "dist": n[o["dist_travelled"]:o["dist_travelled"] + N * 4].view(np.float32),
                        "remaining": n[o["remaining"]:o["remaining"] + 4].view(np.int32),
                        "done": n[o["done_u8"]:o["done_u8"] + 1], "viol": n[o["violation"]:o["violation"] + 1]}
        hs = self._hs
        hs["act_host"].numpy()[0, :] = np.asarray(actions, dtype=np.int32).reshape(self.N)
        hs["act_dev"].copy_(hs["act_host"], non_blocking=True)
        rc = self.step_raw(hs["act_dev"].data_ptr())
        if rc != 0:
            _lib.check(rc, "rg_step")
        hs["host"].copy_(self._out_arena, non_blocking=True)
        torch.cuda.current_stream(self.device).synchronize()
        return hs["obs"], hs["reward"], bool(hs["done"][0]), int(hs["viol"][0]), int(hs["remaining"][0]), hs["dist"]

    @property
    def step_kernel(self):
        return "tpe" if self.lib.rg_step_kernel(self._h) == 1 else "group"

    def step_raw(self, actions_ptr):
        return self.lib.rg_step(self._h, actions_ptr, self._io_ref, 1 if self.auto_reset else 0, self.seed)

    def set_stream(self, stream=None):
        stream = torch.cuda.current_stream(self.device) if stream is None else stream
        _lib.check(self.lib.rg_set_stream(self._h, C.c_void_p(stream.cuda_stream)), "rg_set_stream")
        self._stream = stream
        self._stream_ptr = stream.cuda_stream

    def rollout(self, actions, out=None):
        if actions.dtype != torch.int32 or not actions.is_contiguous() or actions.device != self.device:
            actions = actions.to(device=self.device, dtype=torch.int32).contiguous()
        self._sync_stream()
        K = int(actions.shape[0])
        if tuple(actions.shape) != (K, self.E, self.N):
            raise ValueError(f"actions must be [K,{self.E},{self.N}], got {tuple(actions.shape)}")
        if out is None or out["obs"].shape[0] != K:
            f32, new = torch.float32, self._alloc
            out = {"obs": new((K, self.E, self.N, self.D), f32),
                   "reward": new((K, self.E, self.N), f32),
                   "done": new((K, self.E), torch.uint8),
                   "dist_travelled": new((K, self.E, self.N), f32),
                   "violation": new((K, self.E), torch.uint8),
                   "remaining": new((K, self.E), torch.int32)}
            if self.qp_sweeps is not None:
                out["qp_sweeps"] = new((K, self.E), torch.int32)
            out["_io"] = _lib.RgStepIO(out["obs"].data_ptr(), out["reward"].data_ptr(), out["done"].data_ptr(),
                                       out["dist_travelled"].data_ptr(), out["violation"].data_ptr(),
                                       out["remaining"].data_ptr(),
                                       out["qp_sweeps"].data_ptr() if "qp_sweeps" in out else None)
        rc = self.lib.rg_rollout(self._h, actions.data_ptr(), K, C.byref(out["_io"]), 1 if self.auto_reset else 0,
                                 self.seed)
        if rc != 0:
            _lib.check(rc, "rg_rollout")
        return out

    def get_obs(self, out=None):
        self._sync_stream()
        out = self.obs if out is None else out
        _lib.check(self.lib.rg_get_obs(self._h, out.data_ptr()), "rg_get_obs")
        return out

    STATE_KEYS = ("poses", "carry_dist", "episode_steps", "reset_count", "prey_loc", "prey_sensed", "prey_captured",
                  "loaded", "load", "zone_load", "messages", "grid", "goal_col", "pixel_type", "reached_goal",
                  "ep_return", "done_return_sum", "done_count", "done_steps_sum")

    def state_dict(self):
        sd = {k: getattr(self, k).clone() for k in self.STATE_KEYS}
        if self.team_index is not None:
            sd["team_index"] = self.team_index.clone()
        if self.elapsed is not None:
            sd["elapsed"] = self.elapsed.clone()
        sd["seed"] = torch.tensor([self.seed & 0xFFFFFFFF, self.seed >> 32], dtype=torch.int64)
        return sd

    def load_state_dict(self, sd):
        if self.elapsed is not None and "elapsed" not in sd:
            raise KeyError("snapshot has no 'elapsed' (gym TimeLimit counter) but this env has a time limit: take the "
                           "snapshot from a time-limited env, or add sd['elapsed'] (zeros = every episode just started)")
        if self.elapsed is None and "elapsed" in sd:
            raise KeyError("snapshot carries 'elapsed' (gym TimeLimit counter) but this env has no time limit: call "
                           "enable_time_limit() first, or drop the key")
        if self.team_index is None and "team_index" in sd:
            raise KeyError("snapshot carries 'team_index' (team pool) but this env has no team pool")
        unknown = [k for k in sd if k not in ("seed", "elapsed", "team_index") and k not in self.STATE_KEYS]
        if unknown:
            raise KeyError(f"unknown snapshot keys {unknown}")
        if self.next_episode is not None:
            self.next_episode.fill_(-1)
        for k, v in sd.items():
            if k == "seed":
                self.seed = int(v[0]) | (int(v[1]) << 32)
                continue
            getattr(self, k).copy_(torch.as_tensor(v).to(getattr(self, k).dtype).reshape(getattr(self, k).shape))

    def episode_stats(self):
        return self.done_return_sum.sum(), self.done_count.sum(), self.done_steps_sum.sum()

    def close(self):
        if getattr(self, "_h", None):
            self.lib.rg_destroy(self._h)
            self._h = None

    def __del__(self):
        try:
            self.close()
        except Exception:
            pass
```

Before: 1.865 billion.

## Specialize resident step kernel on compile-time reference scenario shapes

Adds a table of reference scenario shapes (prey count, obs dim, neighbours, capability flag, update frequency, controller period, penalty flag). When the handle's parameters match one, it launches a resident step kernel instantiated with those values as template constants. This lets the compiler fold loop bounds and branches and drop scalar argument reads. It adds more kernel instantiations and binary size, and introduces a query API for which step form ran.

Result: faster. 1.964 billion, median of 6 (+5.3%).

```diff
diff --git a/include/robogym.h b/include/robogym.h
--- a/include/robogym.h
+++ b/include/robogym.h
@@ -139,6 +139,14 @@
 
 int rg_step_kernel(const rg_handle *h);
 
+#define RG_FORM_NONE 0
+#define RG_FORM_BY_VALUE 1
+#define RG_FORM_RESIDENT 2
+#define RG_FORM_SHAPE 16
+int rg_step_form(const rg_handle *h);
+int rg_shape_match(const rg_scenario_params *params);
+int rg_shape_info(int32_t shape, int32_t *row);
+
 #define RG_LIDAR_MAX_RAYS 32
 typedef struct rg_lidar_params {
     int32_t rays;
diff --git a/marbler_amd/_lib.py b/marbler_amd/_lib.py
--- a/marbler_amd/_lib.py
+++ b/marbler_amd/_lib.py
@@ -108,13 +108,27 @@
     _fields_ = [("sigma_xy", C.c_float), ("sigma_theta", C.c_float), ("reserved", C.c_float * 2)]
 
 
+FORM_NONE, FORM_BY_VALUE, FORM_RESIDENT, FORM_SHAPE = 0, 1, 2, 16
+
+
+def reference_shapes():
+    lib = load()
+    names = ("id", "scenario", "n_agents", "num_prey", "obs_dim", "num_neighbors", "capability_aware", "update_frequency",
+             "controller_period", "penalize_violations")
+    out, row = [], (C.c_int32 * 10)()
+    while lib.rg_shape_info(len(out) + 1, C.byref(row)) == 0:
+        out.append(dict(zip(names, list(row))))
+    return out
+
+
 EXPORTS = ("rg_abi_version", "rg_last_error", "rg_sizeof_params", "rg_sizeof_state", "rg_sizeof_step_io", "rg_next_init_stride",
            "rg_create", "rg_destroy", "rg_bind_state", "rg_set_stream", "rg_reset", "rg_step", "rg_rollout", "rg_get_obs", "rg_step_kernel",
            "rg_actor_forward", "rg_actor_forward_explore", "rg_actor_pack_gru", "rg_actor_pack_gru_bf16x3", "rg_actor_pack_gru_f16x2", "rg_actor_last_error",
            "rg_sizeof_policy_io", "rg_policy_rollout", "rg_sizeof_lidar_params", "rg_set_lidar",
            "rg_sizeof_team_params", "rg_set_teams",
            "rg_actor_forward_sample", "rg_sizeof_policy_sample", "rg_policy_rollout_sample",
-           "rg_sizeof_disturbance_params", "rg_set_disturbance")
+           "rg_sizeof_disturbance_params", "rg_set_disturbance", "rg_step_form", "rg_shape_match", "rg_shape_info")
+LATE_QUERIES = ("rg_step_form", "rg_shape_match", "rg_shape_info")
 
 _lib = None
 
@@ -134,6 +148,8 @@
     lib = C.CDLL(LIB_PATH)
     for name in EXPORTS:
         if not hasattr(lib, name):
+            if name in LATE_QUERIES and os.environ.get("ROBOGYM_LIB"):
+                continue
             raise RobogymError(f"{LIB_PATH} does not export {name}")
     lib.rg_abi_version.restype = C.c_int
     lib.rg_last_error.restype = C.c_char_p
@@ -150,6 +166,13 @@
     lib.rg_get_obs.argtypes = [C.c_void_p, C.c_void_p]
     lib.rg_step_kernel.argtypes = [C.c_void_p]
     lib.rg_step_kernel.restype = C.c_int
+    if hasattr(lib, "rg_step_form"):
+        lib.rg_step_form.argtypes = [C.c_void_p]
+        lib.rg_step_form.restype = C.c_int
+        lib.rg_shape_match.argtypes = [C.POINTER(RgScenarioParams)]
+        lib.rg_shape_match.restype = C.c_int
+        lib.rg_shape_info.argtypes = [C.c_int32, C.POINTER(C.c_int32 * 10)]
+        lib.rg_shape_info.restype = C.c_int
     lib.rg_actor_forward.argtypes = [C.POINTER(RgActorWeights), C.c_int32, C.c_int32, C.c_void_p, C.c_int32, C.c_int32,
                                      C.c_void_p, C.c_void_p, C.c_void_p, C.c_void_p, C.c_void_p]
     lib.rg_actor_forward.restype = C.c_int
diff --git a/marbler_amd/build.py b/marbler_amd/build.py
--- a/marbler_amd/build.py
+++ b/marbler_amd/build.py
@@ -7,7 +7,7 @@
 HERE = os.path.dirname(os.path.abspath(__file__))
 CSRC = os.path.join(HERE, "csrc")
 LIB = os.path.join(HERE, "librobogym_hip.so")
-SOURCES = ["robogym_kernels.hip", "robogym_resident.hip", "robogym_rollout_group.hip", "robogym_kernels_ipm.hip", "robogym_rollout_group_ipm.hip",
+SOURCES = ["robogym_kernels.hip", "robogym_resident.hip", "robogym_resident_shapes.hip", "robogym_rollout_group.hip", "robogym_kernels_ipm.hip", "robogym_rollout_group_ipm.hip",
            "robogym_tpe.hip", "robogym_rollout_tpe.hip", "robogym_capi.hip", "actor_mfma.hip", "robogym_policy_h64.hip",
            "robogym_policy_h128.hip", "robogym_policy_sample_h64.hip", "robogym_policy_sample_h128.hip", "robogym_lidar.hip", "robogym_lidar_rollout.hip", "robogym_lidar_ipm.hip",
            "robogym_lidar_rollout_ipm.hip", "robogym_team.hip", "robogym_team_rollout.hip", "robogym_team_ipm.hip",
@@ -22,6 +22,7 @@
 FILE_FLAGS = {"robogym_tpe.hip": ["-fno-slp-vectorize"], "robogym_rollout_tpe.hip": ["-fno-slp-vectorize"],
               "robogym_kernels.hip": GROUP_SLP, "robogym_rollout_group.hip": GROUP_SLP,
               "robogym_resident.hip": GROUP_SLP + RESIDENT_PRELOAD,
+              "robogym_resident_shapes.hip": GROUP_SLP + RESIDENT_PRELOAD,
               "robogym_kernels_ipm.hip": GROUP_SLP + IPM_SCHED, "robogym_rollout_group_ipm.hip": GROUP_SLP + IPM_SCHED,
               "robogym_policy_h64.hip": GROUP_SLP, "robogym_policy_h128.hip": GROUP_SLP,
               "robogym_policy_sample_h64.hip": GROUP_SLP, "robogym_policy_sample_h128.hip": GROUP_SLP,
diff --git a/marbler_amd/csrc/kernel_args.h b/marbler_amd/csrc/kernel_args.h
--- a/marbler_amd/csrc/kernel_args.h
+++ b/marbler_amd/csrc/kernel_args.h
@@ -95,10 +95,11 @@
 hipError_t launch_reset(const KernelArgs &a, hipStream_t stream);
 
 enum GroupFamily { GROUP_PLAIN, GROUP_LIDAR, GROUP_TEAM, GROUP_DISTURB };
-enum GroupKind { GROUP_STEP, GROUP_ROLLOUT, GROUP_OBS, GROUP_STEP_RESIDENT };
+enum GroupKind { GROUP_STEP, GROUP_ROLLOUT, GROUP_OBS, GROUP_STEP_RESIDENT, GROUP_STEP_SHAPE };
 #define RG_GROUP_ENTRIES(X)                                              \
     X(launch_step, GROUP_PLAIN, RG_QP_EXACT, GROUP_STEP)                 \
     X(launch_step_resident, GROUP_PLAIN, RG_QP_EXACT, GROUP_STEP_RESIDENT) \
+    X(launch_step_shape, GROUP_PLAIN, RG_QP_EXACT, GROUP_STEP_SHAPE)     \
     X(launch_obs, GROUP_PLAIN, RG_QP_EXACT, GROUP_OBS)                   \
     X(launch_rollout, GROUP_PLAIN, RG_QP_EXACT, GROUP_ROLLOUT)           \
     X(launch_step_ipm, GROUP_PLAIN, RG_QP_CVXOPT, GROUP_STEP)            \
@@ -126,6 +127,7 @@
     const rg_team_params *teams;
     const DisturbScale *disturb;
     const struct KernelArgs *image;
+    int shape;
 };
 
 struct ResidentCall {
@@ -138,6 +140,42 @@
 };
 static_assert(sizeof(ResidentCall) <= 256, "the per-call arguments fit one register of dwords (device_common.h load_arg_regs_resident)");
 hipError_t resident_image(KernelArgs &a);
+
+template <int P_, int D_, int M_, int CA_, int U_, int PERIOD_, int PENALIZE_>
+struct Shape {
+    static constexpr int P = P_, D = D_, M = M_, CA = CA_, U = U_, PERIOD = PERIOD_, PENALIZE = PENALIZE_;
+};
+using NoShape = Shape<-1, -1, -1, -1, -1, -1, -1>;
+#ifndef RG_SHAPE_FIELDS
+#define RG_SHAPE_FIELDS 127
+#endif
+#define RG_SF(bit, v) ((RG_SHAPE_FIELDS >> (bit)) & 1 ? (v) : -1)
+#define RG_REF_SHAPES(X)                                                                                                      \
+    X(1, RG_SCN_PREDATOR_CAPTURE_PREY, 5, RG_SF(0, 6), RG_SF(1, 16), RG_SF(2, 3), RG_SF(3, 0), RG_SF(4, 29), RG_SF(5, 15), RG_SF(6, 1)) \
+    X(2, RG_SCN_WAREHOUSE, 8, -1, RG_SF(1, 18), RG_SF(2, 5), -1, RG_SF(4, 29), RG_SF(5, 15), RG_SF(6, 1))                               \
+    X(3, RG_SCN_MATERIAL_TRANSPORT, 6, -1, RG_SF(1, 9), -1, RG_SF(3, 0), RG_SF(4, 74), RG_SF(5, 15), RG_SF(6, 1))
+inline int match_shape(const rg_scenario_params &p) {
+#define RG_X(id, scn, n, P, D, M, CA, U, PERIOD, PENALIZE)                                                                       \
+    if (p.scenario == (scn) && p.n_agents == (n) && ((P) < 0 || p.num_prey == (P)) && ((D) < 0 || p.obs_dim == (D)) &&            \
+        ((M) < 0 || p.num_neighbors == (M)) && ((CA) < 0 || (p.capability_aware != 0) == ((CA) != 0)) &&                          \
+        ((U) < 0 || p.update_frequency == (U)) && ((PERIOD) < 0 || p.controller_period == (PERIOD)) &&                           \
+        ((PENALIZE) < 0 || (p.penalize_violations != 0) == ((PENALIZE) != 0)))                                                   \
+        return id;
+    RG_REF_SHAPES(RG_X)
+#undef RG_X
+    return 0;
+}
+inline bool shape_row(int id, int32_t out[10]) {
+#define RG_X(i, scn, n, P, D, M, CA, U, PERIOD, PENALIZE)                          \
+    if (id == (i)) {                                                               \
+        const int32_t r[10] = {i, scn, n, P, D, M, CA, U, PERIOD, PENALIZE};       \
+        for (int c = 0; c < 10; ++c) out[c] = r[c];                                \
+        return true;                                                               \
+    }
+    RG_REF_SHAPES(RG_X)
+#undef RG_X
+    return false;
+}
 typedef hipError_t GroupLaunch(const KernelArgs &a, const GroupSide &side, hipStream_t stream);
 #define RG_X(entry, family, mode, kind) GroupLaunch entry;
 RG_GROUP_ENTRIES(RG_X)
diff --git a/marbler_amd/csrc/robogym_capi.hip b/marbler_amd/csrc/robogym_capi.hip
--- a/marbler_amd/csrc/robogym_capi.hip
+++ b/marbler_amd/csrc/robogym_capi.hip
@@ -31,6 +31,9 @@
     rg::KernelArgs *image_slots;
     int32_t images_used;
     const rg::KernelArgs *image;
+    bool shapes;
+    int32_t image_shape;
+    mutable int32_t last_form;
     bool image_stale;
 };
 constexpr int RG_IMAGE_SLOTS = 8;
@@ -39,6 +42,7 @@
 static void write_image(rg_handle *h);
 static void drop_image(rg_handle *h) {
     h->image = nullptr;
+    h->image_shape = 0;
     h->image_stale = true;
 }
 
@@ -235,6 +239,12 @@
         const char *res = getenv("RG_STEP_RESIDENT");
         h->resident = !(res && !strcmp(res, "0")) && rg::resident_image && rg::launch_step_resident;
     }
+    {
+        const char *shp = getenv("RG_STEP_SHAPE");
+        h->shapes = !(shp && !strcmp(shp, "0")) && rg::launch_step_shape;
+    }
+    h->image_shape = 0;
+    h->last_form = RG_FORM_NONE;
     h->image_slots = nullptr;
     h->images_used = 0;
     h->image = nullptr;
@@ -354,6 +364,7 @@
 
 static void write_image(rg_handle *h) {
     h->image = nullptr;
+    h->image_shape = 0;
     if (!h->resident || !h->bound || h->use_tpe || !h->span || h->teams.n_sets || h->lidar.rays || h->disturbed ||
         h->params.qp_mode != RG_QP_EXACT) {
         h->image_stale = false;
@@ -393,6 +404,7 @@
         return;
     }
     h->image = slot;
+    h->image_shape = h->shapes ? rg::match_shape(a.p) : 0;
 }
 
 static int fill_args(rg_handle *h, rg::KernelArgs &a) {
@@ -435,11 +447,17 @@
     return 0;
 }
 
+static int32_t step_form(const rg::KernelArgs *image, int shape) {
+    return !image ? RG_FORM_BY_VALUE : shape ? RG_FORM_SHAPE + shape : RG_FORM_RESIDENT;
+}
+
 static int launch_group_entry(const rg_handle *h, const rg::KernelArgs &a, int kind, const rg::KernelArgs *image = nullptr) {
     const int family = h->teams.n_sets ? rg::GROUP_TEAM : h->lidar.rays ? rg::GROUP_LIDAR
                        : (h->disturbed && kind != rg::GROUP_OBS) ? rg::GROUP_DISTURB : rg::GROUP_PLAIN;
     const int mode = kind == rg::GROUP_OBS ? RG_QP_EXACT : h->params.qp_mode;
-    const rg::GroupSide side = {&h->lidar, &h->teams, &h->disturb, family == rg::GROUP_PLAIN ? image : nullptr};
+    const bool res = family == rg::GROUP_PLAIN && image;
+    const rg::GroupSide side = {&h->lidar, &h->teams, &h->disturb, res ? image : nullptr, res ? h->image_shape : 0};
+    if (kind == rg::GROUP_STEP) h->last_form = step_form(side.image, side.shape);
     for (const GroupEntry &g : g_group)
         if (g.family == family && g.mode == mode && g.kind == kind && g.launch) return launched(g.launch(a, side, h->stream));
     return fail(-100, "this build has no lane-group step kernels");
@@ -470,7 +488,10 @@
     RG_ON_DEVICE(h);
     if (int rc = sync_seed(h, seed)) return rc;
     if (!h->span && !h->teams.n_sets && !h->lidar.rays && !h->disturbed) a.envs_per_wave = -1;
-    if (h->use_tpe) return launched(rg::launch_step_tpe(a, h->stream));
+    if (h->use_tpe) {
+        h->last_form = RG_FORM_BY_VALUE;
+        return launched(rg::launch_step_tpe(a, h->stream));
+    }
     if (h->image_stale) write_image(h);
     return launch_group_entry(h, a, rg::GROUP_STEP, io->elapsed ? nullptr : h->image);
 }
@@ -593,6 +614,21 @@
     return h->use_tpe ? 1 : 0;
 }
 
+int rg_step_form(const rg_handle *h) {
+    if (!h) return fail(-1, "handle is NULL");
+    return h->last_form;
+}
+
+int rg_shape_match(const rg_scenario_params *params) {
+    if (!params) return fail(-1, "params is NULL");
+    return rg::match_shape(*params);
+}
+
+int rg_shape_info(int32_t shape, int32_t *row) {
+    if (!row) return fail(-1, "row is NULL");
+    return rg::shape_row(shape, row) ? 0 : fail(-80, "rg_shape_info: no such reference shape");
+}
+
 int rg_get_obs(rg_handle *h, float *obs) {
     rg::KernelArgs a;
     if (int rc = fill_args(h, a)) return rc;
diff --git a/marbler_amd/csrc/robogym_resident_shapes.hip b/marbler_amd/csrc/robogym_resident_shapes.hip
--- /dev/null
+++ b/marbler_amd/csrc/robogym_resident_shapes.hip
@@ -0,0 +1,24 @@
+#include "step_group.h"
+
+namespace rg {
+
+hipError_t launch_step_shape(const KernelArgs &a, const GroupSide &side, hipStream_t stream) {
+    if constexpr (kStampsBuild) {
+        return hipErrorInvalidValue;
+    } else {
+        const int grid = wave_fill(a.E, 8).grid;
+        const dim3 g(grid), b(WAVE);
+#define RG_X(id, scn, n, P, D, M, CA, U, PERIOD, PENALIZE)                                                                            \
+    if (side.shape == (id)) {                                                                                                        \
+        if (a.p.scenario != (scn) || a.p.n_agents != (n)) return hipErrorInvalidValue;                                               \
+        hipLaunchKernelGGL((step_kernel<scn, 8, false, n, false, 16, true, Shape<P, D, M, CA, U, PERIOD, PENALIZE>>), g, b, 0, stream, \
+                           side.image, a.actions, a.seed, a.auto_reset, grid, a.io);                                                 \
+        return hipGetLastError();                                                                                                    \
+    }
+        RG_REF_SHAPES(RG_X)
+#undef RG_X
+        return hipErrorInvalidValue;
+    }
+}
+
+}
diff --git a/marbler_amd/csrc/step_group.h b/marbler_amd/csrc/step_group.h
--- a/marbler_amd/csrc/step_group.h
+++ b/marbler_amd/csrc/step_group.h
@@ -311,13 +311,14 @@
 }
 
 template <int SCN, int GW, bool OBS_ONLY, int NT, bool AHEAD, bool GYM, int QPM = 0, typename QpLds = void, typename Sync = WgSync,
-          bool LIDAR = false, bool TEAM = false, bool SPAN = false, bool NOISE = false, bool RES = false>
+          bool LIDAR = false, bool TEAM = false, bool SPAN = false, bool NOISE = false, bool RES = false, class SH = NoShape>
 __device__ __forceinline__ void step_once(const KernelArgs &a, Lds<GW> &lds, const StepView &sv, QpLds *qp_lds = nullptr,
                                           const rg_lidar_params *lid = nullptr, const rg_team_params *tm = nullptr,
                                           const DisturbScale *nz = nullptr) {
     static_assert(!SPAN || (GW == 8 && QPM == 0 && !GYM && !LIDAR && !TEAM && !NOISE), "the 16-lane rows: exact mode, GW = 8, no side blocks");
     static_assert(!NOISE || !OBS_ONLY, "an observation-only launch displaces nothing");
     static_assert(!RES || (SPAN && RG_ROW_ARG_REGS != 0), "the resident form: the 16-lane rows, arguments in vector registers");
+    static_assert(RES || std::is_same<SH, NoShape>::value, "shapes: the resident form only");
     constexpr int RW = SPAN ? 2 * GW : GW;
     constexpr int EPW = WAVE / RW;
     RG_STAMPS_BEGIN()
@@ -332,6 +333,7 @@
 #define RG_ARG(f) (ARGV ? arg_reg<std::decay_t<decltype(f)>>(av, RG_ARG_OFF(f)) : (f))
 #define RG_ARG_OR(f, q) (ARGV ? arg_reg<std::decay_t<decltype(q)>>(av, RG_ARG_OFF(f)) : (q))
 #define RG_OUT(m) (ARGV ? arg_reg<std::decay_t<decltype(sv.io.m)>>(av, RG_ARG_OFF(a.io.m)) : (sv.io.m))
+#define RG_SHAPED(F, x) (SH::F >= 0 ? SH::F : (x))
     auto arg_elem = [&](const auto &array, int i) {
         const unsigned off = static_cast<unsigned>(reinterpret_cast<const char *>(&array) - reinterpret_cast<const char *>(&a));
         return __builtin_amdgcn_readlane(av[off >> 8], static_cast<int>((off >> 2) & 63) + i);
@@ -347,9 +349,13 @@
     const int32_t *q_rc = RG_IMG(a.st.reset_count), *q_nep = AHEAD ? RG_IMG(a.st.next_episode) : nullptr;
     const float *q_nin = AHEAD ? RG_IMG(a.st.next_init) : nullptr;
     const int q_nst = AHEAD ? a.next_stride : 0;
-    const int q_E = a.E, q_epw = a.envs_per_wave, q_P = p.num_prey, q_N = p.n_agents, q_G = RES ? sv.grid : gridDim.x;
+    const int q_E = a.E, q_epw = a.envs_per_wave, q_P = RG_SHAPED(P, p.num_prey), q_N = p.n_agents, q_G = RES ? sv.grid : gridDim.x;
+    if constexpr (SH::P < 0)
     asm volatile("" ::"s"(q_poses), "s"(q_carry), "s"(q_ret), "s"(q_sum), "s"(q_steps), "s"(q_act), "s"(q_cnt), "s"(q_stp),
                  "s"(q_E), "s"(q_epw), "s"(q_P), "s"(q_N), "s"(q_G), "s"(q_rc));
+    else
+    asm volatile("" ::"s"(q_poses), "s"(q_carry), "s"(q_ret), "s"(q_sum), "s"(q_steps), "s"(q_act), "s"(q_cnt), "s"(q_stp),
+                 "s"(q_E), "s"(q_epw), "s"(q_N), "s"(q_G), "s"(q_rc));
     if constexpr (GYM) asm volatile("" ::"s"(q_el), "s"(q_tl));
     if constexpr (AHEAD) asm volatile("" ::"s"(q_nep), "s"(q_nin), "s"(q_nst));
     const float *q_prey = RG_IMG(a.st.prey_loc);
@@ -452,7 +458,7 @@
                 nx_pose[2] = nb[2 * N + ag];
             }
             if constexpr (SCN == RG_SCN_PREDATOR_CAPTURE_PREY || SCN == RG_SCN_SIMPLE) {
-                if (ag < RG_ARG_OR(p.num_prey, q_P)) {
+                if (ag < RG_SHAPED(P, RG_ARG_OR(p.num_prey, q_P))) {
                     nx_a = nb[3 * N + 2 * ag];
                     nx_b = nb[3 * N + 2 * ag + 1];
                 }
@@ -609,8 +615,8 @@
         bool dead = false;
         float fin_x = 0.0f, fin_y = 0.0f;
         float bx = x, by = y, ox = 0.0f, oy = 0.0f;
-        const bool penalize = p.penalize_violations != 0;
-        const int U = p.update_frequency, period = p.controller_period;
+        const bool penalize = RG_SHAPED(PENALIZE, p.penalize_violations) != 0;
+        const int U = RG_SHAPED(U, p.update_frequency), period = RG_SHAPED(PERIOD, p.controller_period);
         for (int it0 = 0; it0 < U; it0 += period) {
             const int n = (U - it0) < period ? (U - it0) : period;
             RG_HEADING_SINCOS(th, s, c);
@@ -802,7 +808,7 @@
         RG_CHUNK_REPORT()
     }
 
-    const int D = RG_ARG(p.obs_dim);
+    const int D = RG_SHAPED(D, RG_ARG(p.obs_dim));
     const auto obs_row = RG_OUT(obs) + (eN + ag) * D;
     const bool ahead_e = ARGV ? AHEAD && (!OBS_ONLY) && RG_ARG(a.next_stride) > 0 && RG_ARG(a.auto_reset) : ahead;
     const bool stats_e = ARGV ? (!OBS_ONLY) && RG_ARG(a.st.ep_return) != nullptr : stats;
@@ -818,7 +824,7 @@
     if constexpr (AHEAD) load_next(next_early & !helper);
 
     if constexpr (SCN == RG_SCN_PREDATOR_CAPTURE_PREY) {
-        const int P = RG_ARG_OR(p.num_prey, q_P);
+        const int P = RG_SHAPED(P, RG_ARG_OR(p.num_prey, q_P));
         if constexpr (TEAM) {
             RG_LATE(sr);
             RG_LATE(cr);
@@ -978,7 +984,7 @@
         }
         }
         RG_STAMP_E(0);
-        const int od = RG_ARG(p.capability_aware) ? 6 : 4;
+        const int od = RG_SHAPED(CA, RG_ARG(p.capability_aware)) ? 6 : 4;
         lds.own[lane][0] = x;
         lds.own[lane][1] = y;
         lds.own[lane][2] = qx;
@@ -991,10 +997,10 @@
 #pragma unroll
                 for (int cc = 0; cc < 6; ++cc) obs_row[cc] = lds.own[lane][cc];
             }
-            write_neighbour_obs<GW, 6, NT, SPAN>(lds, N, RG_ARG(p.num_neighbors), ag, gbase, lane_nb, x, y, obs_row);
+            write_neighbour_obs<GW, 6, NT, SPAN>(lds, N, RG_SHAPED(M, RG_ARG(p.num_neighbors)), ag, gbase, lane_nb, x, y, obs_row);
         } else {
             if (lane_st) out_store4(obs_row, x, y, qx, qy);
-            write_neighbour_obs<GW, 4, NT, SPAN>(lds, N, RG_ARG(p.num_neighbors), ag, gbase, lane_nb, x, y, obs_row);
+            write_neighbour_obs<GW, 4, NT, SPAN>(lds, N, RG_SHAPED(M, RG_ARG(p.num_neighbors)), ag, gbase, lane_nb, x, y, obs_row);
         }
         RG_STAMP_E(1);
         if constexpr (!OBS_ONLY) {
@@ -1026,7 +1032,7 @@
             obs_row[1] = y;
             obs_row[2] = loaded ? 1.0f : 0.0f;
         }
-        write_neighbour_obs<GW, 3, NT, SPAN>(lds, N, RG_ARG(p.num_neighbors), ag, gbase, lane_nb, x, y, obs_row);
+        write_neighbour_obs<GW, 3, NT, SPAN>(lds, N, RG_SHAPED(M, RG_ARG(p.num_neighbors)), ag, gbase, lane_nb, x, y, obs_row);
         if constexpr (!OBS_ONLY) {
             if (viol) {
                 reward = RG_ARG(p.violation_reward);
@@ -1167,7 +1173,7 @@
             obs_row[4] = static_cast<float>(zone1);
 #pragma unroll
             for (int i = 0; i < 4; ++i) obs_row[5 + i] = static_cast<float>(msg[i]);
-            if (RG_ARG(p.capability_aware)) {
+            if (RG_SHAPED(CA, RG_ARG(p.capability_aware))) {
                 if constexpr (TEAM) obs_row[9] = static_cast<float>(tq_raw);
                 else obs_row[9] = static_cast<float>(p.torque[ag]);
                 obs_row[10] = agent_step;
@@ -1323,7 +1329,7 @@
                     }
                 }
                 if constexpr (SCN == RG_SCN_PREDATOR_CAPTURE_PREY || SCN == RG_SCN_SIMPLE) {
-                    const int P = RG_ARG_OR(p.num_prey, q_P);
+                    const int P = RG_SHAPED(P, RG_ARG_OR(p.num_prey, q_P));
                     const auto nb = RG_ARG_OR(a.st.next_init, q_nin) + static_cast<size_t>(e) * RG_ARG_OR(a.next_stride, q_nst) + 3 * N;
                     for (int i = ag; i < P; i += GW) {
                         const auto pl = RG_ARG(a.st.prey_loc) + (static_cast<size_t>(e) * P + i) * 2;
@@ -1369,6 +1375,7 @@
 #undef RG_ARG_OFF
 #undef RG_ARG_OR
 #undef RG_OUT
+#undef RG_SHAPED
 
 struct PlainFamily {
     using Args = KernelArgs;
@@ -1463,6 +1470,18 @@
     const StepView sv = {actions, io, &auto_reset, &seed, grid};
     step_once<SCN, GW, false, NT, true, false, 0, void, WgSync, false, false, true, false, true>(a, lds, sv);
 }
+template <int SCN, int GW, bool OBS_ONLY, int NT, bool ROLLOUT, int ROW, bool RESIDENT, class SH, std::enable_if_t<ROW == 16 && RESIDENT, int> = 0>
+__global__ __launch_bounds__(WAVE) void step_kernel(const KernelArgs *image, const int32_t *actions, const uint64_t seed, const int32_t auto_reset,
+                                                    const int32_t grid, const rg_step_io io) {
+    static_assert(GW == 8 && !OBS_ONLY && !ROLLOUT, "the 16-lane rows: the single-step launch at GW 8");
+    typedef const __attribute__((address_space(4))) KernelArgs *ConstImage;
+    ConstImage ci = (ConstImage)image;
+    asm volatile("" : "+s"(ci));
+    const KernelArgs &a = *(const KernelArgs *)ci;
+    __shared__ Lds<GW> lds;
+    const StepView sv = {actions, io, &auto_reset, &seed, grid};
+    step_once<SCN, GW, false, NT, true, false, 0, void, WgSync, false, false, true, false, true, SH>(a, lds, sv);
+}
 #endif
 template <int SCN, int GW, bool OBS_ONLY, bool ROLLOUT, bool GYM, int QPM>
 __global__ __launch_bounds__(WAVE) void lidar_step_kernel(const LidarArgs la) {
@@ -1552,7 +1571,7 @@
             }
         };
         if constexpr (ROWS) {
-            if (rows && side.image) return launch_step_resident(args, side, stream);
+            if (rows && side.image) return side.shape ? launch_step_shape(args, side, stream) : launch_step_resident(args, side, stream);
         }
         if (ROWS && rows) by_n(std::integral_constant<bool, ROWS>());
         else by_n(std::false_type());
diff --git a/marbler_amd/vec_env.py b/marbler_amd/vec_env.py
--- a/marbler_amd/vec_env.py
+++ b/marbler_amd/vec_env.py
@@ -314,6 +314,13 @@
     def step_kernel(self):
         return "tpe" if self.lib.rg_step_kernel(self._h) == 1 else "group"
 
+    @property
+    def step_form(self):
+        form = self.lib.rg_step_form(self._h)
+        if form < 0:
+            _lib.check(form, "rg_step_form")
+        return form
+
     def step_raw(self, actions_ptr):
         return self.lib.rg_step(self._h, actions_ptr, self._io_ref, 1 if self.auto_reset else 0, self.seed)
 
```
